# rpng/open_vins

Hardware: NVIDIA H100
Metric: msckf_updates_per_sec (higher is better)
Workload: dtype f64

## Files before the change

open_vins_b200/csrc/chol_tiles.cuh:

```cuda
#pragma once
#include "chol.cuh"
#ifdef CQ_PROBE
#include <cstdio>
#endif

#define CT_XP 12

__device__ __forceinline__ void ct_dmma(double &d0, double &d1, double a, double b) {
  asm volatile("mma.sync.aligned.m8n8k4.row.col.f64.f64.f64.f64 {%0,%1}, {%2}, {%3}, {%0,%1};" : "+d"(d0), "+d"(d1) : "d"(a), "d"(b));
}
__device__ __forceinline__ int ct_tri(int b) { return (b * (b + 1)) >> 1; }
__device__ __forceinline__ void ct_bar_group(int id, int nthreads) { asm volatile("bar.sync %0, %1;" ::"r"(id), "r"(nthreads) : "memory"); }
__device__ __forceinline__ size_t ct_idx(int i, int j) { return (size_t)(ct_tri(i >> 3) + (j >> 3)) * 64 + (i & 7) * 8 + (j & 7); }

struct CtView {
  double *T, *Xp0, *Xp1, *invd, *Linv0, *Linv1, *dummyT, *dummyX;
  int *flag;
};
__host__ __device__ inline size_t ct_view_doubles(int NRB) {
  return (size_t)((NRB * (NRB + 1)) / 2) * 64 + 2 * (size_t)NRB * 8 * CT_XP + (size_t)NRB * 8 + 128 + 64 + 2 * CT_XP;
}
__device__ __forceinline__ CtView ct_view_carve(double *base, int NRB, int *flag_word) {
  CtView v;
  v.T = base;
  v.Xp0 = v.T + (size_t)((NRB * (NRB + 1)) / 2) * 64;
  v.Xp1 = v.Xp0 + (size_t)NRB * 8 * CT_XP;
  v.invd = v.Xp1 + (size_t)NRB * 8 * CT_XP;
  v.Linv0 = v.invd + (size_t)NRB * 8;
  v.Linv1 = v.Linv0 + 64;
  v.dummyT = v.Linv1 + 64;
  v.dummyX = v.dummyT + 64;
  v.flag = flag_word;
  return v;
}

__device__ __forceinline__ void ct_diag8_frag(double &d0, double &d1, int nbk, double *invd, bool strict, double floor_d, int *flag) {
  const unsigned full = 0xffffffffu;
  const int lane = threadIdx.x & 31, g = lane >> 2, q = lane & 3;
  bool bad = false;
  double myinv = 0.0;
  const double inv_floor = (floor_d > 0.0) ? fast_rsqrt(floor_d) : 0.0;
  double pj = __shfl_sync(full, d0, 0);
#pragma unroll
  for (int j = 0; j < 8; j++) {
    const int jq = j >> 1;
    const double cur = (j & 1) ? d1 : d0;
    const double ag = __shfl_sync(full, cur, 4 * g + jq);
    const double ac0 = __shfl_sync(full, cur, 8 * q + jq);
    const double ac1 = __shfl_sync(full, cur, 8 * q + 4 + jq);
    double an = 0.0, dn = 0.0;
    if (j < 7) {
      an = __shfl_sync(full, cur, 4 * (j + 1) + jq);
      dn = __shfl_sync(full, ((j + 1) & 1) ? d1 : d0, 4 * (j + 1) + ((j + 1) >> 1));
    }
    const double y = fast_rsqrt(pj);
    const bool in = j < nbk;
    double d, iv;
    if (strict) {
      const bool pos = pj > 0.0;
      bad = bad || (in && !pos);
      d = pj;
      iv = (in && pos) ? y : 0.0;
    } else {
      const bool above = pj > floor_d;
      d = above ? pj : floor_d;
      iv = in ? (above ? y : inv_floor) : 0.0;
    }
    if (j < 7) {
      const double ln = an * iv;
      pj = fma(-ln, ln, dn);
    }
    if (lane == j)
      myinv = iv;
    if (q == jq) {
      if (j & 1)
        d1 = (g == j) ? d * iv : d1 * iv;
      else
        d0 = (g == j) ? d * iv : d0 * iv;
    }
    const double lg = ag * iv, lc0 = ac0 * iv, lc1 = ac1 * iv;
    if (2 * q > j)
      d0 = fma(-lg, lc0, d0);
    if (2 * q + 1 > j)
      d1 = fma(-lg, lc1, d1);
  }
  if (lane < 8)
    invd[lane] = myinv;
  if (bad && lane == 0)
    *flag = 1;
}

__device__ __forceinline__ void ct_linv8(const double *Lt, const double *invd, double *Linv) {
  const int lane = threadIdx.x & 31, cc = lane & 7;
  double mc[8];
#pragma unroll
  for (int j = 0; j < 8; j++) {
    double s0 = (j == cc) ? 1.0 : 0.0, s1 = 0.0;
#pragma unroll
    for (int t = 0; t < j; t++) {
      if (t & 1)
        s1 = fma(-Lt[j * 8 + t], mc[t], s1);
      else
        s0 = fma(-Lt[j * 8 + t], mc[t], s0);
    }
    mc[j] = (s0 + s1) * invd[j];
  }
  if (lane < 8) {
#pragma unroll
    for (int i = 0; i < 8; i++)
      Linv[i * 8 + cc] = (i >= cc) ? mc[i] : 0.0;
  }
}

__device__ __forceinline__ void ct_panel_tile(const CtView &sm, int i, int k, const double *Linv, double *Xb) {
  const int lane = threadIdx.x & 31, g = lane >> 2, q = lane & 3;
  double *t = sm.T + (size_t)(ct_tri(i) + k) * 64;
  const double a0 = t[g * 8 + q], a1 = t[g * 8 + q + 4];
  const double b0 = Linv[g * 8 + q], b1 = Linv[g * 8 + q + 4];
  double2 d = make_double2(0.0, 0.0);
  ct_dmma(d.x, d.y, a0, b0);
  ct_dmma(d.x, d.y, a1, b1);
  *reinterpret_cast<double2 *>(t + 2 * lane) = d;
  *reinterpret_cast<double2 *>(Xb + (size_t)(8 * i + g) * CT_XP + 2 * q) = d;
}

__device__ __forceinline__ void ct_panel_rows(double *T, double *Xp, const double *invd, int i0, int stride, int nrows, int k, int nbk) {
  if (i0 >= nrows)
    return;
  const double *Lk = T + (size_t)(ct_tri(k) + k) * 64;
  double L[8][8], iv[8];
#pragma unroll
  for (int c = 0; c < 8; c++) {
    iv[c] = (c < nbk) ? invd[8 * k + c] : 0.0;
#pragma unroll
    for (int t2 = 0; t2 < 4; t2++) {
      if (2 * t2 < c) {
        const double2 v = *reinterpret_cast<const double2 *>(Lk + c * 8 + 2 * t2);
        L[c][2 * t2] = v.x;
        L[c][2 * t2 + 1] = v.y;
      }
    }
  }
  for (int i = i0; i < nrows; i += stride) {
    double *src = T + (size_t)(ct_tri(i >> 3) + k) * 64 + (i & 7) * 8;
    double v[8], x[8];
    {
      const double2 v01 = *reinterpret_cast<const double2 *>(src), v23 = *reinterpret_cast<const double2 *>(src + 2);
      const double2 v45 = *reinterpret_cast<const double2 *>(src + 4), v67 = *reinterpret_cast<const double2 *>(src + 6);
      v[0] = v01.x, v[1] = v01.y, v[2] = v23.x, v[3] = v23.y, v[4] = v45.x, v[5] = v45.y, v[6] = v67.x, v[7] = v67.y;
    }
#pragma unroll
    for (int c = 0; c < 8; c++) {
      x[c] = (c < nbk) ? v[c] * iv[c] : 0.0;
#pragma unroll
      for (int t = c + 1; t < 8; t++)
        v[t] = fma(-x[c], L[t][c], v[t]);
    }
    if (nbk == 8) {
      *reinterpret_cast<double2 *>(src) = make_double2(x[0], x[1]);
      *reinterpret_cast<double2 *>(src + 2) = make_double2(x[2], x[3]);
      *reinterpret_cast<double2 *>(src + 4) = make_double2(x[4], x[5]);
      *reinterpret_cast<double2 *>(src + 6) = make_double2(x[6], x[7]);
    } else {
#pragma unroll
      for (int c = 0; c < 8; c++)
        if (c < nbk)
          src[c] = x[c];
    }
    double *xp = Xp + (size_t)i * CT_XP;
    *reinterpret_cast<double2 *>(xp) = make_double2(x[0], x[1]);
    *reinterpret_cast<double2 *>(xp + 2) = make_double2(x[2], x[3]);
    *reinterpret_cast<double2 *>(xp + 4) = make_double2(x[4], x[5]);
    *reinterpret_cast<double2 *>(xp + 6) = make_double2(x[6], x[7]);
  }
}

struct CtTileOps {
  double a0, a1, b0, b1;
  double2 c;
  double2 *cp;
};
__device__ __forceinline__ void ct_tile_load(CtTileOps &o, const CtView &sm, const double *Xp, int bi, int bj, int lane, bool valid) {
  const int g = lane >> 2, q = lane & 3;
  const double *xa = valid ? Xp + (size_t)(8 * bi + g) * CT_XP + q : sm.dummyX + q;
  const double *xb = valid ? Xp + (size_t)(8 * bj + g) * CT_XP + q : sm.dummyX + q;
  o.cp = reinterpret_cast<double2 *>((valid ? sm.T + (size_t)(ct_tri(bi) + bj) * 64 : sm.dummyT) + 2 * lane);
  o.a0 = -xa[0];
  o.a1 = -xa[4];
  o.b0 = xb[0];
  o.b1 = xb[4];
  o.c = *o.cp;
}
__device__ __forceinline__ void ct_tile_mma(CtTileOps &o) {
  ct_dmma(o.c.x, o.c.y, o.a0, o.b0);
  ct_dmma(o.c.x, o.c.y, o.a1, o.b1);
}
__device__ __forceinline__ void ct_tile_mma_store(CtTileOps &o) {
  ct_tile_mma(o);
  *o.cp = o.c;
}

#ifdef CQ_PROBE
#define CT_PROBE_T(v) v = clock64()
#else
#define CT_PROBE_T(v) do { } while (0)
#endif

__device__ __forceinline__ void ct_trail_row(const CtView &sm, const double *Xk, int bi, int j0, int jmax, int lane) {
  const int g = lane >> 2, q = lane & 3;
  const double *xa = Xk + (size_t)(8 * bi + g) * CT_XP + q;
  const double a0 = -xa[0], a1 = -xa[4];
  double *trow = sm.T + (size_t)ct_tri(bi) * 64 + 2 * lane;
  for (int bj = j0; bj <= jmax; bj += 2) {
    const bool two = bj + 1 <= jmax;
    const double *xb0 = Xk + (size_t)(8 * bj + g) * CT_XP + q;
    const double *xb1 = two ? xb0 + 8 * CT_XP : sm.dummyX + q;
    double2 *c0p = reinterpret_cast<double2 *>(trow + (size_t)bj * 64);
    double2 *c1p = two ? c0p + 32 : reinterpret_cast<double2 *>(sm.dummyT + 2 * lane);
    const double b00 = xb0[0], b01 = xb0[4], b10 = xb1[0], b11 = xb1[4];
    double2 c0 = *c0p, c1 = *c1p;
    ct_dmma(c0.x, c0.y, a0, b00);
    ct_dmma(c1.x, c1.y, a0, b10);
    ct_dmma(c0.x, c0.y, a1, b01);
    ct_dmma(c1.x, c1.y, a1, b11);
    *c0p = c0;
    *c1p = c1;
  }
}

template <int THREADS>
__device__ __forceinline__ void ct_chol_tiles(const CtView &sm, int n, int nrows, bool strict, double floor_d) {
  const int tid = threadIdx.x, lane = tid & 31, wid = tid >> 5;
  constexpr int NW = THREADS / 32, NH = NW - (NW + 3) / 4;
  static_assert(NH >= 1, "need at least one helper warp");
  const bool helper = (wid & 3) != 0;
  const int hr = wid - 1 - (wid >> 2);
  constexpr bool LINV = NW >= 8;
#ifdef CQ_PROBE
  long long p0 = 0, p1 = 0, p2 = 0, p3 = 0, p4 = 0, p5 = 0, acc[6] = {0, 0, 0, 0, 0, 0};
#endif
  const int NB = (n + 7) >> 3, NRB = (nrows + 7) >> 3;
  if (wid == 0) {
    double2 c = *reinterpret_cast<const double2 *>(sm.T + 2 * lane);
    ct_diag8_frag(c.x, c.y, min(8, n), sm.invd, strict, floor_d, sm.flag);
    *reinterpret_cast<double2 *>(sm.T + 2 * lane) = c;
    __syncwarp();
    if (LINV)
      asm volatile("bar.arrive 3, 64;" ::: "memory");
    ct_panel_rows(sm.T, sm.Xp0, sm.invd, lane < 8 ? 8 + lane : nrows, 1 << 30, nrows, 0, min(8, n));
  } else if (LINV && wid == 4) {
    asm volatile("bar.sync 3, 64;" ::: "memory");
    ct_linv8(sm.T, sm.invd, sm.Linv0);
  }
  __syncthreads();
  for (int k = 0; k < NB; k++) {
    const int par = k & 1;
    double *Xk = par ? sm.Xp1 : sm.Xp0, *Xn = par ? sm.Xp0 : sm.Xp1;
    const bool more = k + 1 < NB;
    CT_PROBE_T(p0);
#ifdef CQ_PROBE
    p1 = p2 = p3 = p4 = p0;
#endif
    if (wid == 0) {
      if (more) {
        const int k1 = k + 1, nbk1 = min(8, n - 8 * k1);
        CtTileOps o;
        ct_tile_load(o, sm, Xk, k1, k1, lane, true);
        ct_tile_mma(o);
        CT_PROBE_T(p1);
        ct_diag8_frag(o.c.x, o.c.y, nbk1, sm.invd + 8 * k1, strict, floor_d, sm.flag);
        *o.cp = o.c;
        __syncwarp();
        if (LINV)
          asm volatile("bar.arrive 3, 64;" ::: "memory");
        CT_PROBE_T(p2);
        asm volatile("bar.sync 2, %0;" ::"r"((NH + 1) * 32) : "memory");
        CT_PROBE_T(p3);
        ct_panel_rows(sm.T, Xn, sm.invd, lane < 8 ? 8 * (k + 2) + lane : nrows, 1 << 30, nrows, k1, nbk1);
        CT_PROBE_T(p4);
      }
    } else if (LINV && wid == 4) {
      if (more) {
        asm volatile("bar.sync 3, 64;" ::: "memory");
        ct_linv8(sm.T + (size_t)(ct_tri(k + 1) + k + 1) * 64, sm.invd + 8 * (k + 1), par ? sm.Linv0 : sm.Linv1);
      }
    } else if (helper) {
      if (LINV) {
        const double *Lk = par ? sm.Linv1 : sm.Linv0;
        for (int i = k + 2 + hr; i < NRB; i += NH)
          ct_panel_tile(sm, i, k, Lk, Xk);
      } else {
        ct_panel_rows(sm.T, Xk, sm.invd, 8 * (k + 2) + hr * 32 + lane, NH * 32, nrows, k, min(8, n - 8 * k));
      }
      if (NH > 1)
        ct_bar_group(1, NH * 32);
      else
        __syncwarp();
      CT_PROBE_T(p1);
      if (more) {
        for (int i = k + 2 + hr; i < NRB; i += 2 * NH) {
          CtTileOps o0, o1;
          ct_tile_load(o0, sm, Xk, i, k + 1, lane, true);
          ct_tile_load(o1, sm, Xk, i + NH, k + 1, lane, i + NH < NRB);
          ct_tile_mma_store(o0);
          ct_tile_mma_store(o1);
        }
        asm volatile("bar.arrive 2, %0;" ::"r"((NH + 1) * 32) : "memory");
        CT_PROBE_T(p2);
        const int R = NRB - (k + 2), jmaxc = NB - 1;
        for (int pr = hr; 2 * pr < R; pr += NH) {
          const int rb = R - 1 - pr;
          ct_trail_row(sm, Xk, k + 2 + rb, k + 2, min(k + 2 + rb, jmaxc), lane);
          if (rb != pr)
            ct_trail_row(sm, Xk, k + 2 + pr, k + 2, min(k + 2 + pr, jmaxc), lane);
        }
      }
      CT_PROBE_T(p3);
    }
    __syncthreads();
    CT_PROBE_T(p5);
#ifdef CQ_PROBE
    if (wid == 0) {
      acc[0] += p1 - p0, acc[1] += p2 - p1, acc[2] += p3 - p2, acc[3] += p4 - p3, acc[4] += p5 - p4;
    } else {
      acc[0] += p1 - p0, acc[1] += p2 - p1, acc[2] += p3 - p2, acc[3] += p5 - p3;
    }
    acc[5] += p5 - p0;
#endif
  }
#ifdef CQ_PROBE
  if (tid == 0)
    printf("chol n=%d W0 (cycles over %d steps): diag update %lld pivots %lld wait %lld rows below %lld step tail %lld | %lld\n", n, NB, acc[0], acc[1], acc[2], acc[3],
           acc[4], acc[5]);
  if (tid == 32 || tid == THREADS - 32)
    printf("chol n=%d helper warp %d: panel rows %lld column k+1 %lld trailing %lld wait %lld | %lld\n", n, wid, acc[0], acc[1], acc[2], acc[3], acc[5]);
#endif
}
```

open_vins_b200/csrc/k_cholqr.cu:

```cuda
#include "chol.cuh"
#include "chol_tiles.cuh"
#include "ovb_internal.cuh"
#include <math.h>
#include <cstdio>

#define CQ_MAXN 160
#define CQ_MAXB 20
#define CQ_MAXRB 22
#define CQ_GRAM_T 512
#define CQ_KB 32
#ifndef CQ_CHOL_T
#define CQ_CHOL_T 384
#endif
#define CQ_XP CT_XP
#define CQ_TRSM_T 640

namespace {

__device__ __forceinline__ void dmma(double &d0, double &d1, double a, double b) {
  asm volatile("mma.sync.aligned.m8n8k4.row.col.f64.f64.f64.f64 {%0,%1}, {%2}, {%3}, {%0,%1};" : "+d"(d0), "+d"(d1) : "d"(a), "d"(b));
}
__device__ __forceinline__ unsigned s_u32(const void *p) { return (unsigned)__cvta_generic_to_shared(p); }
__device__ __forceinline__ void cpa16(unsigned dst, const void *src, unsigned bytes) {
  asm volatile("cp.async.cg.shared.global [%0], [%1], 16, %2;" ::"r"(dst), "l"(src), "r"(bytes) : "memory");
// ... 79 lines not shown

}

__global__ void __launch_bounds__(CQ_GRAM_T) k_cq_gram(const double *__restrict__ A, int ldA, int m, int nt, int slab_rows, int BW, int nblk_side,
                                                      double *__restrict__ Gpart, int cs) {
  OVB_PDL_ENTER();
  extern __shared__ __align__(16) double gsm[];
  const int tid = threadIdx.x, lane = tid & 31, wid = tid >> 5, g = lane >> 2, q = lane & 3;
  int ci, cj, offI, offJ;
  bool diag;
  const bool active = cq_tile_origin(blockIdx.x, wid, BW, nblk_side, ci, cj, offI, offJ, diag);
  int bI = 0, tt = blockIdx.x;
  while (tt >= nblk_side - bI) {
    tt -= nblk_side - bI;
    bI++;
  }
  const int bJ = bI + tt;
  const int WI = BW * 32;
  const int nrng = (bI == bJ) ? 1 : 2;
  const int pitch = nrng * WI + 4;
  const int cI0 = bI * WI, cJ0 = bJ * WI;
  const int r0 = blockIdx.y * slab_rows, r1 = min(m, r0 + slab_rows);
  const int nchunks = (r1 > r0) ? (r1 - r0 + CQ_KB - 1) / CQ_KB : 0;
  double acc[4][4][2];
#pragma unroll
  for (int a = 0; a < 4; a++)
#pragma unroll
    for (int b = 0; b < 4; b++)
      acc[a][b][0] = acc[a][b][1] = 0.0;

  auto issue = [&](int c) { cq_issue_rows<CQ_GRAM_T>(gsm + (size_t)(c & 1) * CQ_KB * pitch, pitch, A, ldA, r0 + c * CQ_KB, CQ_KB, r1, nt, cI0, cJ0, WI, nrng); };
  if (nchunks > 0)
    issue(0);
  for (int c = 0; c < nchunks; c++) {
    if (c + 1 < nchunks) {
      issue(c + 1);
      cpa_wait<1>();
    } else {
      cpa_wait<0>();
    }
    __syncthreads();
    if (active) {
      const double *buf = gsm + (size_t)(c & 1) * CQ_KB * pitch;
#pragma unroll
      for (int ks = 0; ks < CQ_KB / 4; ks++)
        cq_gram_kstep(acc, buf + (size_t)4 * ks * pitch, pitch, offI, offJ, diag && offI == offJ, g, q);
    }
    __syncthreads();
  }
  if (cs <= 1) {
    if (active) {
      double *dst = Gpart + (((size_t)blockIdx.y * gridDim.x + blockIdx.x) * 16 + wid) * 1024;
#pragma unroll
      for (int a = 0; a < 4; a++)
#pragma unroll
        for (int b = 0; b < 4; b++)
          *reinterpret_cast<double2 *>(dst + (8 * a + g) * 32 + 8 * b + 2 * q) = make_double2(acc[a][b][0], acc[a][b][1]);
    }
    return;
  }
  double *stage = gsm;
  if (active) {
    double *dst = stage + (size_t)wid * 1024;
#pragma unroll
    for (int a = 0; a < 4; a++)
#pragma unroll
      for (int b = 0; b < 4; b++)
        *reinterpret_cast<double2 *>(dst + (8 * a + g) * 32 + 8 * b + 2 * q) = make_double2(acc[a][b][0], acc[a][b][1]);
  }
  asm volatile("barrier.cluster.arrive.release.aligned;" ::: "memory");
  asm volatile("barrier.cluster.wait.acquire.aligned;" ::: "memory");
  unsigned rank;
  asm volatile("mov.u32 %0, %%cluster_ctarank;" : "=r"(rank));
  if (active) {
    const int per = 1024 / cs;
    double *dst = Gpart + ((((size_t)blockIdx.y / cs) * gridDim.x + blockIdx.x) * 16 + wid) * 1024 + (size_t)rank * per;
    const unsigned base = s_u32(stage + (size_t)wid * 1024 + (size_t)rank * per);
    for (int e = lane; e < per; e += 32) {
      double sum = 0.0;
      for (int r = 0; r < cs; r++) {
        unsigned ra;
        double v;
        asm volatile("mapa.shared::cluster.u32 %0, %1, %2;" : "=r"(ra) : "r"(base + 8u * (unsigned)e), "r"((unsigned)r));
        asm volatile("ld.shared::cluster.f64 %0, [%1];" : "=d"(v) : "r"(ra) : "memory");
        sum += v;
      }
      dst[e] = sum;
    }
  }
  asm volatile("barrier.cluster.arrive.release.aligned;" ::: "memory");
  asm volatile("barrier.cluster.wait.acquire.aligned;" ::: "memory");
}

#define CQ_RED_T 1024
#define CQ_RED_CH 8
#define CQ_RED_GX (16 * CQ_RED_CH)
__global__ void __launch_bounds__(CQ_RED_T) k_cq_reduce(const double *__restrict__ Gpart, int nslab, int nblk, int BW, int nblk_side, int nt,
                                                       double *__restrict__ G, int ldG, int tiled) {
  OVB_PDL_ENTER();
  __shared__ double red[8][128];
  int ci, cj, offI, offJ;
  bool diag;
  const int w = blockIdx.x / CQ_RED_CH, ch = blockIdx.x % CQ_RED_CH, blk = blockIdx.y;
  if (!cq_tile_origin(blk, w, BW, nblk_side, ci, cj, offI, offJ, diag))
    return;
  if (ci >= nt || cj >= nt)
    return;
  const int el = threadIdx.x & 127, sg = threadIdx.x >> 7;
  const int e = ch * 128 + el;
  const double *src = Gpart + ((size_t)blk * 16 + w) * 1024 + e;
  const size_t stride = (size_t)nblk * 16 * 1024;
  double s0 = 0.0, s1 = 0.0;
  int sl = sg;
  for (; sl + 8 < nslab; sl += 16) {
    s0 += src[(size_t)sl * stride];
    s1 += src[(size_t)(sl + 8) * stride];
  }
  if (sl < nslab)
    s0 += src[(size_t)sl * stride];
  red[sg][el] = s0 + s1;
  __syncthreads();
  if (sg == 0) {
    const int i = ci + (e >> 5), j = cj + (e & 31);
    if (i < nt && j < nt && i <= j) {
      const double s = ((red[0][el] + red[1][el]) + (red[2][el] + red[3][el])) + ((red[4][el] + red[5][el]) + (red[6][el] + red[7][el]));
      if (tiled) {
        G[ct_idx(j, i)] = s;
        if ((i >> 3) == (j >> 3))
          G[(size_t)(tri(j >> 3) + (j >> 3)) * 64 + (i & 7) * 8 + (j & 7)] = s;
      } else {
        G[(size_t)i * ldG + j] = s;
        G[(size_t)j * ldG + i] = s;
      }
    }
  }
}

struct CqCholSmem {
  double T[(CQ_MAXRB * (CQ_MAXRB + 1) / 2) * 64];
  double Xp[2][CQ_MAXRB * 8 * CQ_XP];
  double invd[CQ_MAXRB * 8];
  double Linv[2][64];
  double red[32];
  double dummyT[64];
  double dummyX[2 * CQ_XP];
  int flag;
};

#define CQ_PK_INV ((CQ_MAXB * (CQ_MAXB + 1) / 2) * 64)
#define CQ_PK_DOUBLES (CQ_PK_INV + CQ_MAXB * 8)

namespace {

__device__ __forceinline__ void cq_chol_tiles(CqCholSmem &sm, int n, int nrows, bool strict, double floor_d) {
  CtView v;
  v.T = sm.T;
  v.Xp0 = sm.Xp[0];
  v.Xp1 = sm.Xp[1];
  v.invd = sm.invd;
  v.Linv0 = sm.Linv[0];
  v.Linv1 = sm.Linv[1];
  v.dummyT = sm.dummyT;
  v.dummyX = sm.dummyX;
  v.flag = &sm.flag;
  ct_chol_tiles<CQ_CHOL_T>(v, n, nrows, strict, floor_d);
}

__device__ void cq_load_tiles(CqCholSmem &sm, const double *__restrict__ G, size_t ldG, int n, int nrows, const double *__restrict__ rhs, int ld_rhs) {
  const int tid = threadIdx.x, lane = tid & 31, wid = tid >> 5;
  const int NB = (n + 7) >> 3, NRB = (nrows + 7) >> 3;
  for (int i = wid; i < 8 * NRB; i += CQ_CHOL_T / 32) {
    const double *row = (i >= n && rhs != nullptr) ? rhs + (size_t)(i - n) * ld_rhs : G + (size_t)i * ldG;
    const int jmax = min(i | 7, 8 * NB - 1);
    double *dst = sm.T + (size_t)tri(i >> 3) * 64 + (i & 7) * 8;
    for (int j = 2 * lane; j <= jmax; j += 64) {
      unsigned bytes = 0;
      if (i < nrows)
        bytes = (j + 1 < n) ? 16u : (j < n ? 8u : 0u);
      cpa16(s_u32(dst + (size_t)(j >> 3) * 64 + (j & 7)), bytes ? (const void *)(row + j) : (const void *)G, bytes);
    }
  }
  cpa_commit();
  for (int e = tid; e < 2 * CQ_MAXRB * 8 * CQ_XP; e += CQ_CHOL_T)
    (&sm.Xp[0][0])[e] = 0.0;
  if (tid < 64)
    sm.dummyT[tid] = 0.0;
  if (tid < 2 * CQ_XP)
    sm.dummyX[tid] = 0.0;
  if (tid == 0)
    sm.flag = 0;
  cpa_wait<0>();
}

__device__ __forceinline__ double cq_el(const double *T, int i, int j) { return T[(size_t)(tri(i >> 3) + (j >> 3)) * 64 + (i & 7) * 8 + (j & 7)]; }

}

__global__ void __launch_bounds__(CQ_CHOL_T) k_cq_chol_gram(const double *__restrict__ G, int ldG, int n, double shift_rel, double *__restrict__ Lpk, int tiled) {
  OVB_PDL_ENTER();
  extern __shared__ __align__(16) unsigned char cq_raw[];
  CqCholSmem &sm = *reinterpret_cast<CqCholSmem *>(cq_raw);
  const int tid = threadIdx.x, lane = tid & 31, wid = tid >> 5;
#ifdef CQ_PROBE
  const long long q0 = clock64();
#endif
  if (tiled) {
    __shared__ __align__(8) unsigned long long g_bar;
    const unsigned bar = s_u32(&g_bar);
    const int NB = (n + 7) >> 3;
    if (tid == 0) {
      asm volatile("mbarrier.init.shared::cta.b64 [%0], 1;" ::"r"(bar) : "memory");
      asm volatile("fence.mbarrier_init.release.cluster;" ::: "memory");
    }
    __syncthreads();
    if (tid == 0) {
      const unsigned bytes = (unsigned)(tri(NB) * 64 * sizeof(double));
      asm volatile("mbarrier.arrive.expect_tx.shared::cta.b64 _, [%0], %1;" ::"r"(bar), "r"(bytes) : "memory");
      asm volatile("cp.async.bulk.shared::cluster.global.mbarrier::complete_tx::bytes [%0], [%1], %2, [%3];" ::"r"(s_u32(sm.T)), "l"(G), "r"(bytes), "r"(bar)
                   : "memory");
    }
    for (int e = tid; e < 2 * CQ_MAXRB * 8 * CQ_XP; e += CQ_CHOL_T)
      (&sm.Xp[0][0])[e] = 0.0;
    if (tid < 64)
      sm.dummyT[tid] = 0.0;
    if (tid < 2 * CQ_XP)
      sm.dummyX[tid] = 0.0;
    if (tid == 0)
      sm.flag = 0;
    asm volatile("{\n\t.reg .pred p;\n\tCQ_GWAIT:\n\tmbarrier.try_wait.parity.shared::cta.b64 p, [%0], 0;\n\t@p bra CQ_GDONE;\n\tbra CQ_GWAIT;\n\tCQ_GDONE:\n\t}" ::"r"(bar)
                 : "memory");
    const int r0 = n - 8 * (NB - 1);
    if (r0 < 8) {
      double *last = sm.T + (size_t)tri(NB - 1) * 64;
      for (int e = tid; e < NB * 64; e += CQ_CHOL_T)
        if (((e >> 3) & 7) >= r0)
          last[e] = 0.0;
    }
  } else {
    cq_load_tiles(sm, G, (size_t)ldG, n, n, nullptr, 0);
  }
  __syncthreads();
  double mx = 0.0;
  for (int i = tid; i < n; i += CQ_CHOL_T) {
    const double d = sm.T[(size_t)(tri(i >> 3) + (i >> 3)) * 64 + (i & 7) * 9];
    mx = (d > mx) ? d : mx;
  }
#pragma unroll
  for (int o = 16; o > 0; o >>= 1) {
    const double y = __shfl_xor_sync(0xffffffffu, mx, o);
    mx = (y > mx) ? y : mx;
  }
  if (lane == 0)
    sm.red[wid] = mx;
  __syncthreads();
  mx = 0.0;
  for (int w = 0; w < CQ_CHOL_T / 32; w++)
    mx = (sm.red[w] > mx) ? sm.red[w] : mx;
  const double shift = shift_rel * mx;
  for (int i = tid; i < n; i += CQ_CHOL_T)
    sm.T[(size_t)(tri(i >> 3) + (i >> 3)) * 64 + (i & 7) * 9] += shift;
  __syncthreads();
#ifdef CQ_PROBE
  const long long q1 = clock64();
#endif
  cq_chol_tiles(sm, n, n, false, 0.25 * shift);
#ifdef CQ_PROBE
  const long long q2 = clock64();
#endif
  const int NB = (n + 7) >> 3;
  for (int e = 2 * tid; e < tri(NB) * 64; e += 2 * CQ_CHOL_T)
    *reinterpret_cast<double2 *>(Lpk + e) = *reinterpret_cast<const double2 *>(sm.T + e);
  for (int e = tid; e < CQ_MAXB * 8; e += CQ_CHOL_T)
    Lpk[CQ_PK_INV + e] = (e < n) ? sm.invd[e] : 1.0;
#ifdef CQ_PROBE
  if (tid == 0)
    printf("chol_gram n=%d: load %lld factor %lld store %lld cycles\n", n, q1 - q0, q2 - q1, clock64() - q2);
#endif
}

__global__ void __launch_bounds__(CQ_CHOL_T) k_cq_chol_ekf(double *__restrict__ S, int ldS, int r, const double *__restrict__ res, double *__restrict__ w,
                                                          double *__restrict__ invdiag, DevUpdateInfo *__restrict__ info, double *__restrict__ Lpk,
                                                          const double *__restrict__ floor_dev) {
  OVB_PDL_ENTER();
  extern __shared__ __align__(16) unsigned char cq_raw[];
  CqCholSmem &sm = *reinterpret_cast<CqCholSmem *>(cq_raw);
  const int tid = threadIdx.x, lane = tid & 31, wid = tid >> 5;
  const int nrows = r + (res != nullptr ? 1 : 0);
  cq_load_tiles(sm, S, (size_t)ldS, r, nrows, res, 0);
  __syncthreads();
  if (floor_dev != nullptr)
    cq_chol_tiles(sm, r, nrows, false, *floor_dev);
  else
    cq_chol_tiles(sm, r, nrows, true, 0.0);
  for (int i = wid; i < r; i += CQ_CHOL_T / 32)
    for (int j = lane; j <= i; j += 32)
      S[(size_t)i * ldS + j] = cq_el(sm.T, i, j);
  if (res != nullptr)
    for (int j = tid; j < r; j += CQ_CHOL_T)
      w[j] = cq_el(sm.T, r, j);
  if (invdiag != nullptr)
    for (int j = tid; j < r; j += CQ_CHOL_T)
      invdiag[j] = sm.invd[j];
  if (Lpk != nullptr) {
    const int NB = (r + 7) >> 3;
    for (int e = 2 * tid; e < tri(NB) * 64; e += 2 * CQ_CHOL_T)
      *reinterpret_cast<double2 *>(Lpk + e) = *reinterpret_cast<const double2 *>(sm.T + e);
    for (int e = tid; e < CQ_MAXB * 8; e += CQ_CHOL_T)
      Lpk[CQ_PK_INV + e] = (e < r) ? sm.invd[e] : 1.0;
  }
  if (tid == 0 && sm.flag && info != nullptr)
    info->not_spd = 1;
}

#define CQ_TRSM_NH 10
#define CQ_TRSM_SMEM (sizeof(double) * ((size_t)CQ_PK_DOUBLES + (size_t)(CQ_TRSM_T / 32) * CQ_TRSM_NH * 2 * 32))
template <int NH>
__device__ __forceinline__ void cq_trsm_half(double (&acc)[NH][2], int b0, const double *Lt, const double *Ri, double *xs, int lane) {
  const int g = lane >> 2, q = lane & 3;
#pragma unroll
  for (int jb = 0; jb < NH; jb++) {
    const int B = b0 + jb;
    const double *Ld = Lt + (size_t)(tri(B) + B) * 64;
    const double *ri = Ri + B * 8;
    double x[8];
#pragma unroll
    for (int qq = 0; qq < 4; qq++) {
      x[2 * qq] = __shfl_sync(0xffffffffu, acc[jb][0], (lane & ~3) | qq);
      x[2 * qq + 1] = __shfl_sync(0xffffffffu, acc[jb][1], (lane & ~3) | qq);
    }
#pragma unroll
    for (int c = 0; c < 8; c++) {
      x[c] *= ri[c];
#pragma unroll
      for (int c2 = c + 1; c2 < 8; c2++)
        x[c2] -= x[c] * Ld[c2 * 8 + c];
    }
    acc[jb][0] = (q == 0) ? x[0] : (q == 1) ? x[2] : (q == 2) ? x[4] : x[6];
    acc[jb][1] = (q == 0) ? x[1] : (q == 1) ? x[3] : (q == 2) ? x[5] : x[7];
    const double af0 = -((q == 0) ? x[0] : (q == 1) ? x[1] : (q == 2) ? x[2] : x[3]);
    const double af1 = -((q == 0) ? x[4] : (q == 1) ? x[5] : (q == 2) ? x[6] : x[7]);
    if (xs != nullptr) {
      xs[(2 * jb) * 32 + lane] = af0;
      xs[(2 * jb + 1) * 32 + lane] = af1;
    }
#pragma unroll
    for (int j = jb + 1; j < NH; j++) {
      const double *lf = Lt + (size_t)(tri(b0 + j) + B) * 64 + g * 8 + q;
      dmma(acc[j][0], acc[j][1], af0, lf[0]);
      dmma(acc[j][0], acc[j][1], af1, lf[4]);
    }
  }
}

template <int NH>
__device__ __forceinline__ void cq_trsm_load(double (&acc)[NH][2], const double *arow, bool row_ok, int b0, int nt, int q) {
#pragma unroll
  for (int jb = 0; jb < NH; jb++) {
    const int col = 8 * (b0 + jb) + 2 * q;
    acc[jb][0] = acc[jb][1] = 0.0;
    if (row_ok) {
      if (col + 1 < nt) {
        const double2 v = *reinterpret_cast<const double2 *>(arow + col);
        acc[jb][0] = v.x;
        acc[jb][1] = v.y;
      } else if (col < nt) {
        acc[jb][0] = arow[col];
      }
    }
  }
}
template <int NH>
__device__ __forceinline__ void cq_trsm_store(const double (&acc)[NH][2], double *arow, bool row_ok, int b0, int nt, int q) {
  if (!row_ok)
    return;
#pragma unroll
  for (int jb = 0; jb < NH; jb++) {
    const int col = 8 * (b0 + jb) + 2 * q;
    if (col + 1 < nt)
      *reinterpret_cast<double2 *>(arow + col) = make_double2(acc[jb][0], acc[jb][1]);
    else if (col < nt)
      arow[col] = acc[jb][0];
  }
}

template <int NBP, int NT>
__device__ __forceinline__ void cq_fetch_factor(double *Lt, double *Ri, const double *__restrict__ Lpk, int NB) {
  const int tid = threadIdx.x;
  __shared__ __align__(8) unsigned long long l_bar;
  const unsigned bar = s_u32(&l_bar);
  if (tid == 0) {
    asm volatile("mbarrier.init.shared::cta.b64 [%0], 1;" ::"r"(bar) : "memory");
    asm volatile("fence.mbarrier_init.release.cluster;" ::: "memory");
  }
  __syncthreads();
  if (tid == 0) {
    const unsigned bytesL = (unsigned)(tri(NB) * 64 * sizeof(double)), bytesR = (unsigned)(NB * 8 * sizeof(double));
    asm volatile("mbarrier.arrive.expect_tx.shared::cta.b64 _, [%0], %1;" ::"r"(bar), "r"(bytesL + bytesR) : "memory");
    asm volatile("cp.async.bulk.shared::cluster.global.mbarrier::complete_tx::bytes [%0], [%1], %2, [%3];" ::"r"(s_u32(Lt)), "l"(Lpk), "r"(bytesL), "r"(bar)
                 : "memory");
    asm volatile("cp.async.bulk.shared::cluster.global.mbarrier::complete_tx::bytes [%0], [%1], %2, [%3];" ::"r"(s_u32(Ri)), "l"(Lpk + CQ_PK_INV), "r"(bytesR),
                 "r"(bar)
                 : "memory");
  }
  for (int e = tri(NB) * 64 + tid; e < tri(NBP) * 64; e += NT)
    Lt[e] = 0.0;
  for (int e = NB * 8 + tid; e < NBP * 8; e += NT)
    Ri[e] = 1.0;
  asm volatile("{\n\t.reg .pred p;\n\tCQ_LWAIT:\n\tmbarrier.try_wait.parity.shared::cta.b64 p, [%0], 0;\n\t@p bra CQ_LDONE;\n\tbra CQ_LWAIT;\n\tCQ_LDONE:\n\t}" ::"r"(bar)
               : "memory");
  __syncthreads();
}

template <int NH1, int NH2>
__global__ void __launch_bounds__(CQ_TRSM_T) k_cq_trsm(double *__restrict__ A, int ldA, int m, int nt, const double *__restrict__ Lpk) {
  OVB_PDL_ENTER();
  extern __shared__ __align__(16) double tsm[];
  double *Lt = tsm;
  double *Ri = tsm + CQ_PK_INV;
  double *Xs = tsm + CQ_PK_DOUBLES;
  const int tid = threadIdx.x, lane = tid & 31, wid = tid >> 5, g = lane >> 2, q = lane & 3;
  cq_fetch_factor<NH1 + NH2, CQ_TRSM_T>(Lt, Ri, Lpk, (nt + 7) >> 3);
  double *xs = Xs + (size_t)wid * (CQ_TRSM_NH * 2 * 32);
  const int ngroups = (m + 7) >> 3;
  for (int rg = blockIdx.x + gridDim.x * wid; rg < ngroups; rg += gridDim.x * (CQ_TRSM_T / 32)) {
    const int row = 8 * rg + g;
    const bool row_ok = row < m;
    double *arow = A + (size_t)row * ldA;
#ifdef CQ_PROBE
    long long t0 = clock64(), t1, t2, t3 = 0, t4 = 0;
#endif
    {
      double acc[NH1][2];
      cq_trsm_load<NH1>(acc, arow, row_ok, 0, nt, q);
#ifdef CQ_PROBE
      t1 = clock64();
#endif
      cq_trsm_half<NH1>(acc, 0, Lt, Ri, NH2 > 0 ? xs : nullptr, lane);
#ifdef CQ_PROBE
      t2 = clock64();
#endif
      cq_trsm_store<NH1>(acc, arow, row_ok, 0, nt, q);
    }
    if constexpr (NH2 > 0) {
      double acc[NH2][2];
      cq_trsm_load<NH2>(acc, arow, row_ok, NH1, nt, q);
      __syncwarp();
#pragma unroll 2
      for (int jb = 0; jb < NH1; jb++) {
        const double af0 = xs[(2 * jb) * 32 + lane], af1 = xs[(2 * jb + 1) * 32 + lane];
#pragma unroll
        for (int j = 0; j < NH2; j++) {
          const double *lf = Lt + (size_t)(tri(NH1 + j) + jb) * 64 + g * 8 + q;
          dmma(acc[j][0], acc[j][1], af0, lf[0]);
          dmma(acc[j][0], acc[j][1], af1, lf[4]);
        }
      }
#ifdef CQ_PROBE
      t3 = clock64();
#endif
      cq_trsm_half<NH2>(acc, NH1, Lt, Ri, nullptr, lane);
#ifdef CQ_PROBE
      t4 = clock64();
#endif
      cq_trsm_store<NH2>(acc, arow, row_ok, NH1, nt, q);
      __syncwarp();
    }
// ... 210 lines not shown
      acc[a][b][0] = acc[a][b][1] = 0.0;
  for (int k0 = 0; k0 < K; k0 += 32) {
    for (int e = tid; e < 64 * 16; e += CQ_GN_T) {
      const int r = e >> 4, u = e & 15, k = k0 + 2 * u;
      unsigned ba = 0, bb = 0;
      if (m0 + r < M)
        ba = (k + 1 < K) ? 16u : (k < K ? 8u : 0u);
      if (n0 + r < N)
        bb = (k + 1 < K) ? 16u : (k < K ? 8u : 0u);
      cpa16(s_u32(&As[r][2 * u]), ba ? (const void *)(A + (size_t)(m0 + r) * lda + k) : (const void *)A, ba);
      cpa16(s_u32(&Bs[r][2 * u]), bb ? (const void *)(B + (size_t)(n0 + r) * ldb + k) : (const void *)B, bb);
    }
    cpa_commit();
    cpa_wait<0>();
    __syncthreads();
#pragma unroll
    for (int ks = 0; ks < 8; ks++) {
      double fa[4], fb[2];
#pragma unroll
      for (int a = 0; a < 4; a++)
        fa[a] = As[wm + 8 * a + g][4 * ks + q];
#pragma unroll
      for (int b = 0; b < 2; b++)
        fb[b] = Bs[wn + 8 * b + g][4 * ks + q];
#pragma unroll
      for (int a = 0; a < 4; a++)
#pragma unroll
        for (int b = 0; b < 2; b++)
          dmma(acc[a][b][0], acc[a][b][1], fa[a], fb[b]);
    }
    __syncthreads();
  }
#pragma unroll
  for (int a = 0; a < 4; a++)
#pragma unroll
    for (int b = 0; b < 2; b++) {
      const int i = m0 + wm + 8 * a + g, j = n0 + wn + 8 * b + 2 * q;
      if (i < M) {
        double *c = C + (size_t)i * ldc + j;
        if (j + 1 < N) {
          double2 v = *reinterpret_cast<double2 *>(c);
          v.x -= acc[a][b][0];
          v.y -= acc[a][b][1];
          *reinterpret_cast<double2 *>(c) = v;
        } else if (j < N) {
          c[0] -= acc[a][b][0];
        }
      }
    }
}

__global__ void __launch_bounds__(256) k_cq_shift(double *__restrict__ G, int ldG, int n, double shift_rel, double *__restrict__ floor_out) {
  OVB_PDL_ENTER();
  __shared__ double red[8];
  double mx = 0.0;
  for (int i = threadIdx.x; i < n; i += 256) {
    const double d = G[(size_t)i * ldG + i];
    mx = (d > mx) ? d : mx;
  }
#pragma unroll
  for (int o = 16; o > 0; o >>= 1) {
    const double y = __shfl_xor_sync(0xffffffffu, mx, o);
    mx = (y > mx) ? y : mx;
  }
  if ((threadIdx.x & 31) == 0)
    red[threadIdx.x >> 5] = mx;
  __syncthreads();
  mx = 0.0;
  for (int w = 0; w < 8; w++)
    mx = (red[w] > mx) ? red[w] : mx;
  const double shift = shift_rel * mx;
  for (int i = threadIdx.x; i < n; i += 256)
    G[(size_t)i * ldG + i] += shift;
  if (threadIdx.x == 0)
    *floor_out = 0.25 * shift;
}

__global__ void __launch_bounds__(256) k_cq_trmm_wide(const double *__restrict__ L2, const double *__restrict__ L1, int ldL, int nt, double *__restrict__ Rout,
                                                     int ldR) {
  OVB_PDL_ENTER();
  __shared__ double As[32][33];
  __shared__ double Bs[32][33];
  const int ti = blockIdx.y, tj = blockIdx.x;
  const int tid = threadIdx.x, tx = tid & 31, ty = tid >> 5;
  const int n = nt - 1;
  double acc[4] = {0, 0, 0, 0};
  if (tj >= ti) {
    for (int tk = ti; tk <= tj; tk++) {
      for (int e = tid; e < 1024; e += 256) {
        const int a = e >> 5, b = e & 31;
        const int k = tk * 32 + a, i = ti * 32 + b;
        As[a][b] = (k < nt && i < nt && k >= i) ? L2[(size_t)k * ldL + i] : 0.0;
        const int j = tj * 32 + a, k2 = tk * 32 + b;
        Bs[a][b] = (j < nt && k2 < nt && j >= k2) ? L1[(size_t)j * ldL + k2] : 0.0;
      }
      __syncthreads();
#pragma unroll 8
      for (int kk = 0; kk < 32; kk++) {
        const double b = Bs[tx][kk];
#pragma unroll
        for (int u = 0; u < 4; u++)
          acc[u] += As[kk][ty + 8 * u] * b;
      }
      __syncthreads();
    }
  }
#pragma unroll
  for (int u = 0; u < 4; u++) {
    const int i = ti * 32 + ty + 8 * u, j = tj * 32 + tx;
    if (i < n && j < nt)
      Rout[(size_t)i * ldR + j] = (j >= i) ? acc[u] : 0.0;
  }
}

#define CQ_GRAM_CS 4
static void cq_launch_gram(ovb_ctx *ctx, int nblk, int nslab_padded, size_t smem, const double *A, int ldA, int m, int nt, int slab_rows, int BW, int nblk_side,
                           double *Gpart, int cs) {
  cudaLaunchConfig_t cfg = {};
  cfg.gridDim = dim3(nblk, nslab_padded);
  cfg.blockDim = dim3(CQ_GRAM_T);
  cfg.dynamicSmemBytes = smem;
  cfg.stream = ctx->stream;
  cudaLaunchAttribute at[2];
  int na = 0;
  if (ctx->tsqr_pdl && !ctx->prof_on) {
    at[na].id = cudaLaunchAttributeProgrammaticStreamSerialization;
    at[na].val.programmaticStreamSerializationAllowed = 1;
    na++;
  }
  if (cs > 1) {
    at[na].id = cudaLaunchAttributeClusterDimension;
    at[na].val.clusterDim.x = 1;
    at[na].val.clusterDim.y = cs;
    at[na].val.clusterDim.z = 1;
    na++;
  }
  cfg.attrs = at;
  cfg.numAttrs = na;
  const bool prof = ctx->prof_on && ctx->prof_n < 96 && ctx->prof_ev[0] != nullptr;
  if (prof)
    cudaEventRecord(ctx->prof_ev[2 * ctx->prof_n], ctx->stream);
  cudaLaunchKernelEx(&cfg, k_cq_gram, A, ldA, m, nt, slab_rows, BW, nblk_side, Gpart, cs);
  if (prof) {
    cudaEventRecord(ctx->prof_ev[2 * ctx->prof_n + 1], ctx->stream);
    ctx->prof_fn[ctx->prof_n++] = (const void *)k_cq_gram;
  }
}

static bool cq_attrs(ovb_ctx *ctx) {
  if (!ctx->attr_done[4]) {
    cudaFuncSetAttribute(k_cq_gram, cudaFuncAttributeMaxDynamicSharedMemorySize, 160 * 1024);
    cudaFuncSetAttribute(k_cq_chol_gram, cudaFuncAttributeMaxDynamicSharedMemorySize, (int)sizeof(CqCholSmem));
    cudaFuncSetAttribute(k_cq_chol_ekf, cudaFuncAttributeMaxDynamicSharedMemorySize, (int)sizeof(CqCholSmem));
    cudaFuncSetAttribute(k_cq_trsm<5, 0>, cudaFuncAttributeMaxDynamicSharedMemorySize, (int)CQ_TRSM_SMEM);
    cudaFuncSetAttribute(k_cq_trsm<10, 0>, cudaFuncAttributeMaxDynamicSharedMemorySize, (int)CQ_TRSM_SMEM);
    cudaFuncSetAttribute(k_cq_trsm<10, 5>, cudaFuncAttributeMaxDynamicSharedMemorySize, (int)CQ_TRSM_SMEM);
    cudaFuncSetAttribute(k_cq_trsm<10, 10>, cudaFuncAttributeMaxDynamicSharedMemorySize, (int)CQ_TRSM_SMEM);
    cudaFuncSetAttribute(k_cq_solve_gram<5, 0>, cudaFuncAttributeMaxDynamicSharedMemorySize, CQ_SG_SMEM);
    cudaFuncSetAttribute(k_cq_solve_gram<10, 0>, cudaFuncAttributeMaxDynamicSharedMemorySize, CQ_SG_SMEM);
    cudaFuncSetAttribute(k_cq_solve_gram<10, 5>, cudaFuncAttributeMaxDynamicSharedMemorySize, CQ_SG_SMEM);
    cudaFuncSetAttribute(k_cq_solve_gram<10, 10>, cudaFuncAttributeMaxDynamicSharedMemorySize, CQ_SG_SMEM);
    ctx->attr_done[4] = 1;
  }
  return true;
}

int ovb_cholqr_max_cols(void) { return CQ_MAXN; }

static bool cq_ensure_G(ovb_ctx *ctx) {
  const int ldW = CQ_MAXN + 8;
  const size_t need_G = (size_t)4 * ldW * ldW;
  if (need_G > ctx->G_cap) {
    if (ctx->d_G)
      cudaFree(ctx->d_G);
    ctx->d_G = nullptr;
    if (cudaMalloc(&ctx->d_G, sizeof(double) * need_G) != cudaSuccess)
      return false;
    cudaMemsetAsync(ctx->d_G, 0, sizeof(double) * need_G, ctx->stream);
    ctx->G_cap = need_G;
  }
  return true;
}

bool launch_chol_ekf_dmma(ovb_ctx *ctx, double *S, int ldS, int r, const double *res, double *w, double *invdiag, double **Lpk_out) {
  if (Lpk_out)
    *Lpk_out = nullptr;
  if (r + 1 > CQ_MAXRB * 8 || r > CQ_MAXN || (ldS & 1))
    return false;
  cq_attrs(ctx);
  double *Lpk = nullptr;
  if (cq_ensure_G(ctx)) {
    const int ldW = CQ_MAXN + 8;
    Lpk = ctx->d_G + (size_t)3 * ldW * ldW;
  }
  ovb_launch(ctx, k_cq_chol_ekf, dim3(1), dim3(CQ_CHOL_T), sizeof(CqCholSmem), S, ldS, r, res, w, invdiag, ctx->d_info, Lpk, (const double *)nullptr);
  if (Lpk_out)
    *Lpk_out = Lpk;
  return true;
}

bool launch_trsm_rows(ovb_ctx *ctx, double *A, int ldA, int m, int nt, const double *Lpk) {
  if (nt > CQ_MAXN || (ldA & 1) || m < 1 || Lpk == nullptr)
    return false;
  cq_attrs(ctx);
  const int ngroups = (m + 7) / 8;
  int ctas = ngroups;
  if (ctas > ctx->sm_count)
    ctas = ctx->sm_count;
  cq_launch_trsm(ctx, ctas, A, ldA, m, nt, Lpk);
  return true;
}

#define CQ_WB 128
#define CQ_WMAX 520
#define CQ_WBLOCKS ((CQ_WMAX + CQ_WB - 1) / CQ_WB)
static bool cq_ensure_wide(ovb_ctx *ctx) {
  const size_t need = (size_t)2 * CQ_WMAX * CQ_WMAX + (size_t)2 * CQ_WBLOCKS * CQ_PK_DOUBLES + 64;
  if (need > ctx->cqw_cap) {
    if (ctx->d_cqw)
      cudaFree(ctx->d_cqw);
    ctx->d_cqw = nullptr;
    if (cudaMalloc(&ctx->d_cqw, sizeof(double) * need) != cudaSuccess)
      return false;
    ctx->cqw_cap = need;
  }
  return true;
}
static void cq_gemm_nt(ovb_ctx *ctx, double *C, int ldc, const double *A, int lda, const double *B, int ldb, int M, int N, int K, int lower_only) {
  if (M <= 0 || N <= 0 || K <= 0)
    return;
  ovb_launch(ctx, k_cq_gemm_nt, dim3((N + 63) / 64, (M + 63) / 64), dim3(CQ_GN_T), (size_t)0, C, ldc, A, lda, B, ldb, M, N, K, lower_only);
}
static void cq_trsm_any(ovb_ctx *ctx, double *A, int ldA, int m, int nt, const double *Lpk) {
  const int ngroups = (m + 7) / 8;
  int ctas = (ngroups + CQ_TRSM_T / 32 - 1) / (CQ_TRSM_T / 32);
  if (ngroups <= ctx->sm_count)
    ctas = ngroups;
  if (ctas > ctx->sm_count)
    ctas = ctx->sm_count;
  cq_launch_trsm(ctx, ctas, A, ldA, m, nt, Lpk);
}
static void cq_chol_blocked(ovb_ctx *ctx, double *S, int ld, int n, int extra, double *Lpk, const double *floor_dev, DevUpdateInfo *info) {
  for (int J = 0, b = 0; J < n; J += CQ_WB, b++) {
    const int nb = (n - J < CQ_WB) ? n - J : CQ_WB;
    double *Lb = Lpk + (size_t)b * CQ_PK_DOUBLES;
    ovb_launch(ctx, k_cq_chol_ekf, dim3(1), dim3(CQ_CHOL_T), sizeof(CqCholSmem), S + (size_t)J * ld + J, ld, nb, (const double *)nullptr, (double *)nullptr,
               (double *)nullptr, info, Lb, floor_dev);
    const int mrem = n + extra - (J + nb);
    if (mrem > 0) {
      double *panel = S + (size_t)(J + nb) * ld + J;
      cq_trsm_any(ctx, panel, ld, mrem, nb, Lb);
      const int ncols = n - (J + nb);
      cq_gemm_nt(ctx, S + (size_t)(J + nb) * ld + (J + nb), ld, panel, ld, panel, ld, mrem, ncols, nb, 1);
    }
  }
}
static void cq_trsm_blocked(ovb_ctx *ctx, double *X, int ldx, int m, int n, const double *S, int ld, const double *Lpk) {
  for (int J = 0, b = 0; J < n; J += CQ_WB, b++) {
    const int nb = (n - J < CQ_WB) ? n - J : CQ_WB;
    if (J > 0)
      cq_gemm_nt(ctx, X + J, ldx, X, ldx, S + (size_t)J * ld, ld, m, nb, J, 0);
    cq_trsm_any(ctx, X + J, ldx, m, nb, Lpk + (size_t)b * CQ_PK_DOUBLES);
  }
}

__global__ void k_cq_copy_row(const double *__restrict__ src, double *__restrict__ dst, int n) {
  OVB_PDL_ENTER();
  const int i = blockIdx.x * blockDim.x + threadIdx.x;
  if (i < n)
    dst[i] = src[i];
}
__global__ void k_cq_inv_diag(const double *__restrict__ S, int ld, int n, double *__restrict__ inv) {
  OVB_PDL_ENTER();
  const int i = blockIdx.x * blockDim.x + threadIdx.x;
  if (i < n) {
    const double d = S[(size_t)i * ld + i];
    inv[i] = d != 0.0 ? 1.0 / d : 0.0;
  }
}

bool launch_chol_solve_wide(ovb_ctx *ctx, double *S, int ldS, int r, double *w, double *invdiag, double *M, int ldM, int N, bool gate_only) {
  if (r > CQ_WMAX - 8 || (ldS & 1) || (ldM & 1) || r + 1 > ctx->cfg.max_state + 1)
    return false;
  cq_attrs(ctx);
  if (!cq_ensure_wide(ctx))
    return false;
  double *Lpk = ctx->d_cqw + (size_t)2 * CQ_WMAX * CQ_WMAX;
  ovb_launch(ctx, k_cq_copy_row, dim3((r + 127) / 128), dim3(128), (size_t)0, (const double *)w, S + (size_t)r * ldS, r);
  cq_chol_blocked(ctx, S, ldS, r, 1, Lpk, nullptr, ctx->d_info);
  ovb_launch(ctx, k_cq_copy_row, dim3((r + 127) / 128), dim3(128), (size_t)0, (const double *)(S + (size_t)r * ldS), w, r);
  ovb_launch(ctx, k_cq_inv_diag, dim3((r + 127) / 128), dim3(128), (size_t)0, (const double *)S, ldS, r, invdiag);
  if (!gate_only)
    cq_trsm_blocked(ctx, M, ldM, N, r, S, ldS, Lpk);
  return true;
}

static int cq_compress_wide(ovb_ctx *ctx, double *A, int m, int n, int ldA, double *Rout, int ldR) {
  const int nt = n + 1;
  if (nt > CQ_WMAX - 7 || !cq_ensure_wide(ctx))
    return -1;
  const int nT = (nt + 31) / 32, BW = 4, nblk_side = (nT + BW - 1) / BW, nblk = nblk_side * (nblk_side + 1) / 2;
  int nslab = ctx->sm_count / nblk;
  if (nslab < 1)
    nslab = 1;
  const int max_slabs = (m + CQ_KB - 1) / CQ_KB;
  if (nslab > max_slabs)
    nslab = max_slabs;
  int slab_rows = (((m + nslab - 1) / nslab) + 3) & ~3;
  nslab = (m + slab_rows - 1) / slab_rows;
  const size_t need_part = (size_t)nslab * nblk * 16 * 1024;
  if (need_part > ctx->Gpart_cap) {
    if (ctx->d_Gpart)
      cudaFree(ctx->d_Gpart);
    ctx->d_Gpart = nullptr;
    if (cudaMalloc(&ctx->d_Gpart, sizeof(double) * need_part) != cudaSuccess)
      return -1;
    ctx->Gpart_cap = need_part;
  }
  double *G1 = ctx->d_cqw, *G2 = G1 + (size_t)CQ_WMAX * CQ_WMAX, *Lpk1 = G2 + (size_t)CQ_WMAX * CQ_WMAX, *Lpk2 = Lpk1 + (size_t)CQ_WBLOCKS * CQ_PK_DOUBLES;
  double *floor_dev = Lpk2 + (size_t)CQ_WBLOCKS * CQ_PK_DOUBLES;
  const size_t gram_smem = sizeof(double) * 2 * CQ_KB * (size_t)(2 * BW * 32 + 4);
  int launches = 0;
  for (int pass = 0; pass < 2; pass++) {
    double *G = pass == 0 ? G1 : G2;
    cq_launch_gram(ctx, nblk, nslab, gram_smem, (const double *)A, ldA, m, nt, slab_rows, BW, nblk_side, ctx->d_Gpart, 1);
    ovb_launch(ctx, k_cq_reduce, dim3(CQ_RED_GX, nblk), dim3(CQ_RED_T), (size_t)0, (const double *)ctx->d_Gpart, nslab, nblk, BW, nblk_side, nt, G, (int)CQ_WMAX, 0);
    ovb_launch(ctx, k_cq_shift, dim3(1), dim3(256), (size_t)0, G, (int)CQ_WMAX, nt, pass == 0 ? 1e-11 : 1e-13, floor_dev + pass);
    cq_chol_blocked(ctx, G, CQ_WMAX, nt, 0, pass == 0 ? Lpk1 : Lpk2, floor_dev + pass, (DevUpdateInfo *)nullptr);
    if (pass == 0)
      cq_trsm_blocked(ctx, A, ldA, m, nt, G1, CQ_WMAX, Lpk1);
    launches += 3 + 3 * ((nt + CQ_WB - 1) / CQ_WB);
  }
  const int nT32 = (nt + 31) / 32;
  ovb_launch(ctx, k_cq_trmm_wide, dim3(nT32, nT32), dim3(256), (size_t)0, (const double *)G2, (const double *)G1, (int)CQ_WMAX, nt, Rout, ldR);
  ctx->n_launch += launches + 1;
  return launches + 1;
}

int launch_compress_cholqr2(ovb_ctx *ctx, double *A, int m, int n, int ldA, double *Rout, int ldR) {
  const int nt = n + 1;
  if ((ldA & 1) || m < 1)
    return -1;
  cq_attrs(ctx);
  if (nt > CQ_MAXN)
    return cq_compress_wide(ctx, A, m, n, ldA, Rout, ldR);
  const int nT = (nt + 31) / 32;
  const int BW = nT, nblk_side = 1, nblk = 1;
  int nslab = ctx->sm_count;
  const int max_slabs = (m + CQ_KB - 1) / CQ_KB;
  if (nslab > max_slabs)
    nslab = max_slabs;
  int slab_rows = (m + nslab - 1) / nslab;
  slab_rows = (slab_rows + 3) & ~3;
  nslab = (m + slab_rows - 1) / slab_rows;
  const int cs = (ctx->gram_cluster && nslab >= 2 * CQ_GRAM_CS) ? CQ_GRAM_CS : 1;
  const int nslab_pad = (nslab + cs - 1) / cs * cs, npart = nslab_pad / cs;
  const size_t part_doubles = (size_t)nslab_pad * nblk * 16 * 1024;
  const size_t need_part = part_doubles + cq_solve_gram_scratch(nslab, nt, BW, slab_rows);
  const int ldW = CQ_MAXN + 8;
  if (!cq_ensure_G(ctx))
    return -1;
  if (need_part > ctx->Gpart_cap) {
    if (ctx->d_Gpart)
// ... 23 lines not shown
```

open_vins_b200/csrc/k_ekf.cu:

```cuda
#include "chol.cuh"
#include "ovb_internal.cuh"

#define EK_T 32

__global__ void __launch_bounds__(256) k_ekf_gemm(int mode, const double *__restrict__ P, int ldP, const double *__restrict__ H, int ldH,
                                                  const double *__restrict__ Min, int ldM, const DevUpdateInfo *__restrict__ info, int X, int Y,
                                                  int K, double *__restrict__ Cout, int ldC, double sigma2, const double *__restrict__ Rdiag) {
  OVB_PDL_ENTER();
  __shared__ double As[EK_T][EK_T + 1];
  __shared__ double Bs[EK_T][EK_T + 1];
  const int x0 = blockIdx.x * EK_T, y0 = blockIdx.y * EK_T;
  if (mode == 1 && y0 > x0 + EK_T - 1)
    return;
  const int tid = threadIdx.x, tx = tid & 31, ty = tid >> 5;
  double acc[4] = {0, 0, 0, 0};
  const int *cs = info->col_state;
  for (int j0 = 0; j0 < K; j0 += EK_T) {
    for (int e = tid; e < EK_T * EK_T; e += 256) {
      int jj = e >> 5, q = e & 31;
      int j = j0 + jj;
      double av = 0.0, bv = 0.0;
      if (j < K) {
        if (mode == 0) {
          int a = x0 + q;
// ... 58 lines not shown
    ld = r | 1;
    W = chol_sm;
    stage_lower_async<EKC_THREADS>(W, ld, S, (size_t)ldS, r + 1, r);
  }
  chol_lower_block<EKC_THREADS, 4>(W, ld, r, 1, &flag, invd_sh, nullptr, 0.0, invdiag);
  __syncthreads();
  if (use_smem) {
    for (int i = wid; i < r; i += EKC_THREADS / 32) {
      for (int j = lane; j <= i; j += 32)
        S[(size_t)i * ldS + j] = W[i * ld + j];
    }
  }
  for (int j = tid; j < r; j += EKC_THREADS)
    w[j] = W[(size_t)r * ld + j];
  if (tid == 0 && flag)
    info->not_spd = 1;
}

#define TR_ROWS 8
__global__ void __launch_bounds__(32 * TR_ROWS) k_ekf_trsm(const double *__restrict__ M, int ldM, const double *__restrict__ L, int ldL,
                                                           const double *__restrict__ invdiag, int N, int r, double *__restrict__ Yout, int ldY,
                                                           int L_in_smem, const DevUpdateInfo *__restrict__ info) {
  OVB_PDL_ENTER();
  extern __shared__ __align__(16) double tsm[];
  const int lane = threadIdx.x & 31, wid = threadIdx.x >> 5;
  if (info->not_spd)
    return;
  const int ldl = r | 1;
  double *inv_s = tsm + (size_t)TR_ROWS * r;
  double *Ls = inv_s + r;
  for (int e = threadIdx.x; e < r; e += 32 * TR_ROWS)
    inv_s[e] = invdiag[e];
  if (L_in_smem)
    stage_lower_async<32 * TR_ROWS>(Ls, ldl, L, (size_t)ldL, r, r);
  else
    __syncthreads();
  const double *Lp = L_in_smem ? Ls : L;
  const int lp = L_in_smem ? ldl : ldL;
  const int a = blockIdx.x * TR_ROWS + wid;
  if (a >= N)
    return;
  double *y = tsm + (size_t)wid * r;
  for (int t = lane; t < r; t += 32)
    y[t] = M[(size_t)a * ldM + t];
  __syncwarp();
  for (int kb = 0; kb < r; kb += 8) {
    const int nbk = min(8, r - kb);
    double s[8];
#pragma unroll
    for (int c = 0; c < 8; c++)
      s[c] = 0.0;
    for (int t = lane; t < kb; t += 32) {
      const double yt = y[t];
#pragma unroll
      for (int c = 0; c < 8; c++)
        if (c < nbk)
          s[c] += Lp[(size_t)(kb + c) * lp + t] * yt;
    }
#pragma unroll
    for (int o = 16; o > 0; o >>= 1) {
#pragma unroll
      for (int c = 0; c < 8; c++)
        s[c] += __shfl_xor_sync(0xffffffffu, s[c], o);
    }
    double yn[8];
#pragma unroll
    for (int c = 0; c < 8; c++) {
      if (c < nbk) {
        const double *Lr = Lp + (size_t)(kb + c) * lp + kb;
        double v = y[kb + c] - s[c];
#pragma unroll
        for (int t = 0; t < 8; t++)
          if (t + 1 < c)
            v -= Lr[t] * yn[t];
        if (c > 0)
          v -= Lr[c - 1] * yn[c - 1];
        yn[c] = v * inv_s[kb + c];
      }
    }
    __syncwarp();
    if (lane < nbk) {
      double v = yn[0];
#pragma unroll
      for (int c = 1; c < 8; c++)
        v = (lane == c) ? yn[c] : v;
      y[kb + lane] = v;
    }
    __syncwarp();
  }
  for (int t = lane; t < r; t += 32)
    Yout[(size_t)a * ldY + t] = y[t];
}

__global__ void __launch_bounds__(256) k_ekf_downdate(double *__restrict__ P, int ldP, const double *__restrict__ Yin, int ldY, int N, int r,
                                                      const double *__restrict__ w, double *__restrict__ dx, DevUpdateInfo *__restrict__ info) {
  OVB_PDL_ENTER();
  __shared__ double As[EK_T][EK_T + 1];
  __shared__ double Bs[EK_T][EK_T + 1];
  const int a0 = blockIdx.x * EK_T, b0 = blockIdx.y * EK_T;
  if (b0 < a0)
    return;
  const int tid = threadIdx.x, tx = tid & 31, ty = tid >> 5;
  if (info->not_spd) {
    if (a0 == b0 && tid < EK_T && a0 + tid < N)
      dx[a0 + tid] = 0.0;
    return;
  }
  double acc[4] = {0, 0, 0, 0};
  double dxa = 0.0;
  for (int k0 = 0; k0 < r; k0 += EK_T) {
    for (int e = tid; e < EK_T * EK_T; e += 256) {
      int q = e >> 5, kk = e & 31;
      int k = k0 + kk;
      As[kk][q] = (k < r && a0 + q < N) ? Yin[(size_t)(a0 + q) * ldY + k] : 0.0;
      Bs[kk][q] = (k < r && b0 + q < N) ? Yin[(size_t)(b0 + q) * ldY + k] : 0.0;
    }
    __syncthreads();
#pragma unroll 8
    for (int kk = 0; kk < EK_T; kk++) {
      double b = Bs[kk][tx];
#pragma unroll
      for (int u = 0; u < 4; u++)
        acc[u] += As[kk][ty + 8 * u] * b;
    }
    if (a0 == b0 && tid < EK_T) {
      for (int kk = 0; kk < EK_T; kk++)
        if (k0 + kk < r)
          dxa += As[kk][tid] * w[k0 + kk];
    }
    __syncthreads();
  }
#pragma unroll
  for (int u = 0; u < 4; u++) {
    int a = a0 + ty + 8 * u, b = b0 + tx;
    if (a < N && b < N && b >= a) {
      double v = P[(size_t)a * ldP + b] - acc[u];
      P[(size_t)a * ldP + b] = v;
      P[(size_t)b * ldP + a] = v;
      if (a == b && v < 0.0)
        atomicMin(&info->neg_diag_index, a);
      if (!isfinite(v))
        info->nonfinite = 1;
    }
  }
  if (a0 == b0 && tid < EK_T && a0 + tid < N)
    dx[a0 + tid] = dxa;
}

#define EK1_KMAX 160
__device__ __forceinline__ void ek_cpa8(double *dst_smem, const double *src) {
  asm volatile("cp.async.ca.shared.global [%0], [%1], 8;" ::"r"((unsigned)__cvta_generic_to_shared(dst_smem)), "l"(src) : "memory");
}
__global__ void __launch_bounds__(256) k_ekf_gemm1(int mode, const double *__restrict__ P, int ldP, const double *__restrict__ H, int ldH,
                                                   const double *__restrict__ Min, int ldM, const DevUpdateInfo *__restrict__ info, int X, int Y,
                                                   int K, double *__restrict__ Cout, int ldC, double sigma2, const double *__restrict__ Rdiag) {
  OVB_PDL_ENTER();
  extern __shared__ __align__(16) double g1[];
  const int x0 = blockIdx.x * EK_T, y0 = blockIdx.y * EK_T;
  if (mode == 1 && y0 > x0 + EK_T - 1)
    return;
  const int tid = threadIdx.x, tx = tid & 31, ty = tid >> 5;
  const int *cs = info->col_state;
  const int pk = K | 1;
  double *Gs = g1, *Hs = g1 + (size_t)K * 33;
  const double *Gsrc = (mode == 0) ? P : Min;
  const int ldG = (mode == 0) ? ldP : ldM;
  const int g0 = (mode == 0) ? x0 : y0, gmax = (mode == 0) ? X : Y;
  const int h0 = (mode == 0) ? y0 : x0, hmax = (mode == 0) ? Y : X;
  __shared__ int cs_s[EK1_KMAX];
  for (int j = tid; j < K; j += 256)
    cs_s[j] = cs[j];
  __syncthreads();
  for (int e = tid; e < K * 32; e += 256) {
    const int j = e >> 5, a = e & 31;
    if (g0 + a < gmax)
      ek_cpa8(&Gs[j * 33 + a], &Gsrc[(size_t)cs_s[j] * ldG + g0 + a]);
    else
      Gs[j * 33 + a] = 0.0;
  }
  for (int i = ty; i < 32; i += 8)
    for (int j = tx; j < K; j += 32) {
      if (h0 + i < hmax)
        ek_cpa8(&Hs[i * pk + j], &H[(size_t)(h0 + i) * ldH + j]);
      else
        Hs[i * pk + j] = 0.0;
    }
  asm volatile("cp.async.commit_group;" ::: "memory");
  asm volatile("cp.async.wait_group 0;" ::: "memory");
  __syncthreads();
  double acc[4] = {0, 0, 0, 0};
  if (mode == 0) {
    for (int j = 0; j < K; j++) {
      const double gv = Gs[j * 33 + tx];
#pragma unroll
      for (int u = 0; u < 4; u++)
        acc[u] += gv * Hs[(ty + 8 * u) * pk + j];
    }
#pragma unroll
    for (int u = 0; u < 4; u++) {
      const int a = x0 + tx, i = y0 + ty + 8 * u;
      if (a < X && i < Y)
        Cout[(size_t)a * ldC + i] = acc[u];
    }
  } else {
    for (int j = 0; j < K; j++) {
      const double gv = Gs[j * 33 + tx];
#pragma unroll
      for (int u = 0; u < 4; u++)
        acc[u] += Hs[(ty + 8 * u) * pk + j] * gv;
    }
#pragma unroll
    for (int u = 0; u < 4; u++) {
      const int i = x0 + ty + 8 * u, k = y0 + tx;
      if (i < X && k < Y) {
        double v = acc[u];
        if (i == k)
          v += Rdiag ? Rdiag[i] : sigma2;
        Cout[(size_t)i * ldC + k] = v;
      }
    }
  }
}

__global__ void __launch_bounds__(256) k_ekf_downdate1(double *__restrict__ P, int ldP, const double *__restrict__ Yin, int ldY, int N, int r,
                                                       const double *__restrict__ w, double *__restrict__ dx, DevUpdateInfo *__restrict__ info) {
  OVB_PDL_ENTER();
  extern __shared__ __align__(16) double d1[];
  const int a0 = blockIdx.x * EK_T, b0 = blockIdx.y * EK_T;
  if (b0 < a0)
    return;
  const int tid = threadIdx.x, tx = tid & 31, ty = tid >> 5;
  if (info->not_spd) {
    if (a0 == b0 && tid < EK_T && a0 + tid < N)
      dx[a0 + tid] = 0.0;
    return;
  }
  const int pk = r | 1;
  double *As = d1, *Bs = d1 + (size_t)32 * pk, *ws = Bs + (size_t)32 * pk;
  for (int i = ty; i < 32; i += 8)
    for (int k = tx; k < r; k += 32) {
      if (a0 + i < N)
        ek_cpa8(&As[i * pk + k], &Yin[(size_t)(a0 + i) * ldY + k]);
      else
        As[i * pk + k] = 0.0;
      if (b0 + i < N)
        ek_cpa8(&Bs[i * pk + k], &Yin[(size_t)(b0 + i) * ldY + k]);
      else
        Bs[i * pk + k] = 0.0;
    }
  for (int k = tid; k < r; k += 256)
    ek_cpa8(&ws[k], &w[k]);
  asm volatile("cp.async.commit_group;" ::: "memory");
  asm volatile("cp.async.wait_group 0;" ::: "memory");
  __syncthreads();
  double acc[4] = {0, 0, 0, 0};
  for (int k = 0; k < r; k++) {
    const double bv = Bs[tx * pk + k];
#pragma unroll
    for (int u = 0; u < 4; u++)
      acc[u] += As[(ty + 8 * u) * pk + k] * bv;
  }
#pragma unroll
  for (int u = 0; u < 4; u++) {
    const int a = a0 + ty + 8 * u, b = b0 + tx;
    if (a < N && b < N && b >= a) {
      const double v = P[(size_t)a * ldP + b] - acc[u];
      P[(size_t)a * ldP + b] = v;
      P[(size_t)b * ldP + a] = v;
      if (a == b && v < 0.0)
        atomicMin(&info->neg_diag_index, a);
      if (!isfinite(v))
        info->nonfinite = 1;
    }
  }
  if (a0 == b0 && tid < EK_T && a0 + tid < N) {
    double s0 = 0.0, s1 = 0.0;
    int k = 0;
    for (; k + 1 < r; k += 2) {
      s0 += As[tid * pk + k] * ws[k];
      s1 += As[tid * pk + k + 1] * ws[k + 1];
    }
    if (k < r)
      s0 += As[tid * pk + k] * ws[k];
    dx[a0 + tid] = s0 + s1;
  }
}

__global__ void k_ekf_prep(DevUpdateInfo *info) {
  OVB_PDL_ENTER();
  info->neg_diag_index = 0x7fffffff;
  info->not_spd = 0;
  info->nonfinite = 0;
}

void launch_ekf_update(ovb_ctx *ctx, const double *H, int ldHm, int r, int n, bool gate_only, double sigma2, const double *Rdiag_dev) {
  const int N = ctx->N;
  const int ld = ctx->ldP;
  double *P = ctx->P[ctx->cur];
  ovb_launch(ctx, k_ekf_prep, dim3(1), dim3(1), (size_t)(0), ctx->d_info);
  if (r <= 0 || n <= 0)
    return;
  if (!ctx->attr_done[2]) {
    cudaFuncSetAttribute(k_ekf_chol, cudaFuncAttributeMaxDynamicSharedMemorySize, 200 * 1024);
    cudaFuncSetAttribute(k_ekf_trsm, cudaFuncAttributeMaxDynamicSharedMemorySize, 200 * 1024);
    cudaFuncSetAttribute(k_ekf_gemm1, cudaFuncAttributeMaxDynamicSharedMemorySize, 100 * 1024);
    cudaFuncSetAttribute(k_ekf_downdate1, cudaFuncAttributeMaxDynamicSharedMemorySize, 100 * 1024);
    ctx->attr_done[2] = 1;
  }
  const bool one_shot = ctx->ekf_chol_dmma && n <= EK1_KMAX && r <= EK1_KMAX;
  dim3 g0((N + EK_T - 1) / EK_T, (r + EK_T - 1) / EK_T);
  dim3 g1((r + EK_T - 1) / EK_T, (r + EK_T - 1) / EK_T);
  if (one_shot) {
    const size_t sm01 = sizeof(double) * ((size_t)n * 33 + (size_t)32 * (n | 1));
    ovb_launch(ctx, k_ekf_gemm1, dim3(g0), dim3(256), sm01, 0, P, ld, H, ldHm, nullptr, 0, ctx->d_info, N, r, n, ctx->d_M, ld, 0.0, nullptr);
    ovb_launch(ctx, k_ekf_gemm1, dim3(g1), dim3(256), sm01, 1, P, ld, H, ldHm, ctx->d_M, ld, ctx->d_info, r, r, n, ctx->d_S, ld, sigma2, Rdiag_dev);
  } else {
    ovb_launch(ctx, k_ekf_gemm, dim3(g0), dim3(256), (size_t)(0), 0, P, ld, H, ldHm, nullptr, 0, ctx->d_info, N, r, n, ctx->d_M, ld, 0.0, nullptr);
    ovb_launch(ctx, k_ekf_gemm, dim3(g1), dim3(256), (size_t)(0), 1, P, ld, H, ldHm, ctx->d_M, ld, ctx->d_info, r, r, n, ctx->d_S, ld, sigma2, Rdiag_dev);
  }
  size_t chol_bytes = sizeof(double) * (size_t)(r + 1) * (size_t)(r | 1);
  int use_smem = chol_bytes <= 200 * 1024;
  double *invdiag = ctx->d_w + ctx->cfg.max_state;
  double *Lpk = nullptr;
  const bool dmma_chol = ctx->ekf_chol_dmma && launch_chol_ekf_dmma(ctx, ctx->d_S, ld, r, ctx->d_w, ctx->d_w, invdiag, &Lpk);
  const bool wide = !dmma_chol && ctx->ekf_chol_dmma && r < ld && launch_chol_solve_wide(ctx, ctx->d_S, ld, r, ctx->d_w, invdiag, ctx->d_M, ld, N, gate_only);
  if (wide) {
    if (gate_only)
      return;
    dim3 g2w((N + EK_T - 1) / EK_T, (N + EK_T - 1) / EK_T);
    ovb_launch(ctx, k_ekf_downdate, dim3(g2w), dim3(256), (size_t)(0), P, ld, (const double *)ctx->d_M, ld, N, r, ctx->d_w, ctx->d_dx, ctx->d_info);
    return;
  }
  if (!dmma_chol)
    ovb_launch(ctx, k_ekf_chol, dim3(1), dim3(EKC_THREADS), (size_t)(use_smem ? chol_bytes : 0), ctx->d_S, ld, r, ctx->d_w, ctx->d_w, invdiag, ctx->d_info, use_smem);
  if (gate_only)
    return;
  const double *Yd = ctx->d_Y;
  if (dmma_chol && Lpk != nullptr && launch_trsm_rows(ctx, ctx->d_M, ld, N, r, Lpk)) {
    Yd = ctx->d_M;
  } else {
    size_t trsm_small = sizeof(double) * ((size_t)TR_ROWS * r + r);
    size_t trsm_full = trsm_small + sizeof(double) * (size_t)r * (size_t)(r | 1);
    int L_in_smem = trsm_full <= 200 * 1024;
    ovb_launch(ctx, k_ekf_trsm, dim3((N + TR_ROWS - 1) / TR_ROWS), dim3(32 * TR_ROWS), (size_t)(L_in_smem ? trsm_full : trsm_small), ctx->d_M, ld, ctx->d_S, ld, invdiag, N,
               r, ctx->d_Y, ld, L_in_smem, ctx->d_info);
  }
  dim3 g2((N + EK_T - 1) / EK_T, (N + EK_T - 1) / EK_T);
  if (one_shot) {
    const size_t smd = sizeof(double) * ((size_t)64 * (r | 1) + r);
    ovb_launch(ctx, k_ekf_downdate1, dim3(g2), dim3(256), smd, P, ld, Yd, ld, N, r, ctx->d_w, ctx->d_dx, ctx->d_info);
  } else {
    ovb_launch(ctx, k_ekf_downdate, dim3(g2), dim3(256), (size_t)(0), P, ld, Yd, ld, N, r, ctx->d_w, ctx->d_dx, ctx->d_info);
  }
}


__global__ void k_cov_init_augment(double *__restrict__ P, int ld, int N, int k, int n, const DevUpdateInfo *__restrict__ info,
                                   const double *__restrict__ Hx, const double *__restrict__ Hinv, double sigma2) {
  extern __shared__ double ism[];
  double *m = ism, *M = ism + (size_t)N * k;
  const int tid = threadIdx.x;
  for (int a = tid; a < N; a += blockDim.x) {
    for (int i = 0; i < k; i++) {
      double acc = 0.0;
      for (int j = 0; j < n; j++)
        acc += P[(size_t)a * ld + info->col_state[j]] * Hx[i * n + j];
      m[a * k + i] = acc;
    }
  }
  __syncthreads();
  if (tid < k * k) {
    const int i = tid / k, i2 = tid % k;
    double acc = 0.0;
    for (int j = 0; j < n; j++)
      acc += Hx[i * n + j] * m[info->col_state[j] * k + i2];
    M[i * k + i2] = acc + (i == i2 ? sigma2 : 0.0);
  }
  __syncthreads();
  if (tid < k * k) {
    const int i = tid / k, i2 = tid % k;
    if (i2 < i)
      M[i * k + i2] = M[i2 * k + i];
  }
  __syncthreads();
  for (int a = tid; a < N; a += blockDim.x) {
    for (int q = 0; q < k; q++) {
      double acc = 0.0;
      for (int i = 0; i < k; i++)
        acc += m[a * k + i] * Hinv[q * k + i];
      P[(size_t)a * ld + N + q] = -acc;
      P[(size_t)(N + q) * ld + a] = -acc;
    }
  }
  if (tid < k * k) {
    const int q = tid / k, q2 = tid % k;
    double acc = 0.0;
    for (int i = 0; i < k; i++)
      for (int i2 = 0; i2 < k; i2++)
        acc += Hinv[q * k + i] * M[i * k + i2] * Hinv[q2 * k + i2];
    if (q <= q2) {
      P[(size_t)(N + q) * ld + N + q2] = acc;
      P[(size_t)(N + q2) * ld + N + q] = acc;
    }
  }
}

bool launch_cov_init_augment(ovb_ctx *ctx, int k, int n, const double *Hx_dev, const double *Hinv_dev, double sigma2) {
  const int N = ctx->N;
  size_t smem = sizeof(double) * ((size_t)N * k + (size_t)k * k);
  if (smem > 200 * 1024)
    return false;
  if (!ctx->attr_done[5]) {
    cudaFuncSetAttribute(k_cov_init_augment, cudaFuncAttributeMaxDynamicSharedMemorySize, 200 * 1024);
    ctx->attr_done[5] = 1;
  }
  k_cov_init_augment<<<1, 256, smem, ctx->stream>>>(ctx->P[ctx->cur], ctx->ldP, N, k, n, ctx->d_info, Hx_dev, Hinv_dev, sigma2);
  return cudaGetLastError() == cudaSuccess;
}

__global__ void k_cov_clone(double *P, int ld, int N, int old_off, int size) {
  int idx = blockIdx.x * blockDim.x + threadIdx.x;
  int N2 = N + size;
  if (idx >= N2 * size)
    return;
  int i = idx / size, j = idx % size;
  double v;
  if (i < N)
    v = P[(size_t)i * ld + old_off + j];
  else
    v = P[(size_t)(old_off + (i - N)) * ld + old_off + j];
  double vr = (i < N) ? P[(size_t)(old_off + j) * ld + i] : v;
  P[(size_t)i * ld + N + j] = v;
  if (i < N)
    P[(size_t)(N + j) * ld + i] = vr;
}
__global__ void k_cov_dt_cols(double *P, int ld, int N2, int new_off, int size, int dt_off, const double *dnc) {
  int idx = blockIdx.x * blockDim.x + threadIdx.x;
  if (idx >= N2 * size)
    return;
  int i = idx / size, j = idx % size;
  P[(size_t)i * ld + new_off + j] += P[(size_t)i * ld + dt_off] * dnc[j];
}
__global__ void k_cov_dt_rows(double *P, int ld, int N2, int new_off, int size, int dt_off, const double *dnc) {
  int idx = blockIdx.x * blockDim.x + threadIdx.x;
  if (idx >= N2 * size)
    return;
  int i = idx / N2, j = idx % N2;
  P[(size_t)(new_off + i) * ld + j] += dnc[i] * P[(size_t)dt_off * ld + j];
}

void launch_cov_clone(ovb_ctx *ctx, int old_off, int size, const double *dnc_dt_dev, int dt_off) {
  double *P = ctx->P[ctx->cur];
  int N = ctx->N, N2 = N + size;
  int tot = N2 * size;
  k_cov_clone<<<(tot + 255) / 256, 256, 0, ctx->stream>>>(P, ctx->ldP, N, old_off, size);
  if (dnc_dt_dev) {
    k_cov_dt_cols<<<(tot + 255) / 256, 256, 0, ctx->stream>>>(P, ctx->ldP, N2, N, size, dt_off, dnc_dt_dev);
    k_cov_dt_rows<<<(tot + 255) / 256, 256, 0, ctx->stream>>>(P, ctx->ldP, N2, N, size, dt_off, dnc_dt_dev);
  }
}

__global__ void k_cov_marg(const double *Pin, double *Pout, int ld, int N, int off, int size) {
  int N2 = N - size;
  int i = blockIdx.y * blockDim.y + threadIdx.y, j = blockIdx.x * blockDim.x + threadIdx.x;
  if (i >= N2 || j >= N2)
    return;
  int si = i < off ? i : i + size, sj = j < off ? j : j + size;
  double v = (i >= off && j < off) ? Pin[(size_t)sj * ld + si] : Pin[(size_t)si * ld + sj];
  Pout[(size_t)i * ld + j] = v;
}

void launch_cov_marginalize(ovb_ctx *ctx, int off, int size) {
  int N2 = ctx->N - size;
  dim3 b(32, 8), g((N2 + 31) / 32, (N2 + 7) / 8);
  k_cov_marg<<<g, b, 0, ctx->stream>>>(ctx->P[ctx->cur], ctx->P[ctx->cur ^ 1], ctx->ldP, ctx->N, off, size);
}

__global__ void k_prop_C(const double *P, int ld, int N, int p, int q, const int *old_idx, const double *Phi, double *Cbuf, int ldC) {
  int idx = blockIdx.x * blockDim.x + threadIdx.x;
  if (idx >= N * p)
    return;
  int a = idx / p, j = idx % p;
  double acc = 0.0;
  for (int k = 0; k < q; k++)
    acc += P[(size_t)a * ld + old_idx[k]] * Phi[(size_t)j * q + k];
  Cbuf[(size_t)a * ldC + j] = acc;
}
__global__ void k_prop_PCP(const double *Cbuf, int ldC, int p, int q, const int *old_idx, const double *Phi, const double *Q, double *Sbuf,
                           int ldS) {
  int idx = blockIdx.x * blockDim.x + threadIdx.x;
  if (idx >= p * p)
    return;
  int i = idx / p, j = idx % p;
  double acc = (i <= j) ? Q[(size_t)i * p + j] : Q[(size_t)j * p + i];
  for (int k = 0; k < q; k++)
    acc += Phi[(size_t)i * q + k] * Cbuf[(size_t)old_idx[k] * ldC + j];
  Sbuf[(size_t)i * ldS + j] = acc;
}
__global__ void k_prop_write(double *P, int ld, int N, int new_off, int p, const double *Cbuf, int ldC, const double *Sbuf, int ldS,
                             DevUpdateInfo *info) {
  int idx = blockIdx.x * blockDim.x + threadIdx.x;
  if (idx >= N * p)
    return;
  int a = idx / p, j = idx % p;
  if (a >= new_off && a < new_off + p) {
    double v = Sbuf[(size_t)(a - new_off) * ldS + j];
// ... 19 lines not shown
```

open_vins_b200/csrc/ovb_api.cu:

```cuda
#include "ovb_internal.cuh"
#include <chrono>
#include <algorithm>
#include <cmath>
#include <cstdio>
#include <cstdlib>
#include <cstring>
#include <new>
#include <vector>

static const double g_chi2_table[OVB_CHI2_TABLE_LEN] = {
#include "chi2_table.inc"
};

unsigned char *ovb_feat_order_ptr(ovb_ctx *ctx) { return ctx->d_feat_order; }

static size_t align_up(size_t v, size_t a) { return (v + a - 1) / a * a; }

extern "C" {

static ovb_status ensure_stage(ovb_ctx *ctx, size_t doubles);

int ovb_abi_version(void) { return OVB_ABI_VERSION; }

double ovb_chi2_quantile95(int dof) {
  if (dof < 1)
    return 0.0;
  if (dof >= OVB_CHI2_TABLE_LEN)
    dof = OVB_CHI2_TABLE_LEN - 1;
  return g_chi2_table[dof];
}

void ovb_opts_default(ovb_opts *o) {
  memset(o, 0, sizeof(*o));
  o->triangulate_1d = 0;
  o->refine_features = 1;
  o->max_runs = 5;
  o->init_lamda = 1e-3;
  o->max_lamda = 1e10;
  o->min_dx = 1e-6;
  o->min_dcost = 1e-6;
  o->lam_mult = 10;
  o->min_dist = 0.10;
  o->max_dist = 60;
  o->max_baseline = 40;
  o->max_cond_number = 10000;
  o->sigma_pix = 1;
  o->chi2_multipler = 5;
  o->do_fej = 1;
  o->feat_rep = OVB_REP_GLOBAL_3D;
  o->do_calib_camera_pose = 0;
  o->do_calib_camera_intrinsics = 0;
  o->col_order = OVB_COLS_CANONICAL;
  o->compress = OVB_COMPRESS_CHOLQR2;
}

const char *ovb_last_error(const ovb_ctx *ctx) { return ctx ? ctx->err : "null context"; }

ovb_status ovb_create(const ovb_config *cfg, ovb_ctx **out) {
  if (!cfg || !out)
    return OVB_ERR_ARG;
  *out = nullptr;
  ovb_ctx *ctx = new (std::nothrow) ovb_ctx();
  if (!ctx)
    return OVB_ERR_CAPACITY;
  memset(ctx, 0, sizeof(*ctx));
  ctx->cfg = *cfg;
  if (ctx->cfg.max_state < 32)
    ctx->cfg.max_state = 32;
  if (ctx->cfg.max_feats < 1)
    ctx->cfg.max_feats = 1;
  if (ctx->cfg.max_meas < 2)
    ctx->cfg.max_meas = 2;
  ctx->device = cfg->device;
  int ndev = 0;
  if (cudaGetDeviceCount(&ndev) != cudaSuccess || ndev <= 0 || cfg->device >= ndev) {
    delete ctx;
    return OVB_ERR_CUDA;
  }
#define CK(call)                                                                                                      \
  do {                                                                                                                \
    cudaError_t e_ = (call);                                                                                          \
    if (e_ != cudaSuccess) {                                                                                          \
      fprintf(stderr, "ovb_create: %s failed: %s\n", #call, cudaGetErrorString(e_));                                  \
      ovb_destroy(ctx);                                                                                               \
      return OVB_ERR_CUDA;                                                                                            \
    }                                                                                                                 \
  } while (0)
  CK(cudaSetDevice(ctx->device));
  cudaDeviceProp prop;
  CK(cudaGetDeviceProperties(&prop, ctx->device));
  ctx->sm_count = prop.multiProcessorCount;
  {
    const char *e = getenv("OVB_TSQR_CLUSTER");
    ctx->tsqr_cluster = e ? atoi(e) : 1;
    const char *e2 = getenv("OVB_TSQR_PDL");
    ctx->tsqr_pdl = e2 ? atoi(e2) : 1;
    const char *e3 = getenv("OVB_FEAT_CLASSES");
    ctx->feat_classes = e3 ? atoi(e3) : 1;
    const char *e4 = getenv("OVB_EKF_CHOL_DMMA");
    ctx->ekf_chol_dmma = e4 ? atoi(e4) : 1;
    const char *e5 = getenv("OVB_GRAM_CLUSTER");
    ctx->gram_cluster = e5 ? atoi(e5) : 0;
  }
  CK(cudaStreamCreateWithFlags(&ctx->stream, cudaStreamNonBlocking));
  ctx->own_stream = 1;
  CK(cudaStreamCreateWithFlags(&ctx->side_stream, cudaStreamNonBlocking));
  CK(cudaStreamCreateWithFlags(&ctx->side_stream2, cudaStreamNonBlocking));
  CK(cudaEventCreateWithFlags(&ctx->ev_join2, cudaEventDisableTiming));
  CK(cudaEventCreateWithFlags(&ctx->ev_fork, cudaEventDisableTiming));
  CK(cudaEventCreateWithFlags(&ctx->ev_join, cudaEventDisableTiming));
  for (int i = 0; i < 8; i++)
    CK(cudaEventCreate(&ctx->ev[i]));
  const int ms = ctx->cfg.max_state;
  ctx->ldP = ms;
  ctx->N = 0;
  ctx->cur = 0;
  CK(cudaMalloc(&ctx->P[0], sizeof(double) * (size_t)ms * ms));
  CK(cudaMalloc(&ctx->P[1], sizeof(double) * (size_t)ms * ms));
  CK(cudaMemset(ctx->P[0], 0, sizeof(double) * (size_t)ms * ms));
  CK(cudaMemset(ctx->P[1], 0, sizeof(double) * (size_t)ms * ms));
  ctx->off_opts = align_up(sizeof(DevFrame), 256);
  ctx->off_feat = ctx->off_opts + align_up(sizeof(DevOpts), 256);
  ctx->off_blob = ctx->off_feat + align_up(sizeof(DevFeat) * (size_t)ctx->cfg.max_feats, 256);
  ctx->blob_cap = align_up((size_t)ctx->cfg.max_meas * (1 + 2 + 8 + 8) + (size_t)ctx->cfg.max_feats * OVB_MAX_CAMS + 64, 256);
  ctx->arena_bytes = ctx->off_blob + ctx->blob_cap;
  CK(cudaMalloc(&ctx->d_arena, ctx->arena_bytes));
  CK(cudaMallocHost(&ctx->h_arena, ctx->arena_bytes));
  ctx->d_frame = (DevFrame *)ctx->d_arena;
  ctx->d_opts = (DevOpts *)(ctx->d_arena + ctx->off_opts);
  ctx->d_feat = (DevFeat *)(ctx->d_arena + ctx->off_feat);
  ctx->d_blob = ctx->d_arena + ctx->off_blob;
  ctx->h_frame = (DevFrame *)ctx->h_arena;
  ctx->h_opts = (DevOpts *)(ctx->h_arena + ctx->off_opts);
  ctx->h_feat = (DevFeat *)(ctx->h_arena + ctx->off_feat);
  ctx->h_blob = ctx->h_arena + ctx->off_blob;
  CK(cudaMalloc(&ctx->d_cc, sizeof(DevCamPoses)));
  CK(cudaMalloc(&ctx->d_feat_order, (size_t)ctx->cfg.max_feats * (OVB_MAX_VARS + 1)));
  ctx->info_bytes = align_up(sizeof(DevUpdateInfo), 256);
  CK(cudaMalloc(&ctx->d_info, ctx->info_bytes + sizeof(double) * (size_t)ms));
  ctx->d_dx = (double *)((char *)ctx->d_info + ctx->info_bytes);
  CK(cudaMallocHost(&ctx->h_info, ctx->info_bytes + sizeof(double) * (size_t)ms));
  ctx->h_dx = (double *)((char *)ctx->h_info + ctx->info_bytes);
  CK(cudaMalloc(&ctx->d_chi2_table, sizeof(g_chi2_table)));
  CK(cudaMemcpy(ctx->d_chi2_table, g_chi2_table, sizeof(g_chi2_table), cudaMemcpyHostToDevice));
  ctx->max_rows = ctx->cfg.max_rows > 0 ? ctx->cfg.max_rows : 2 * ctx->cfg.max_meas;
  if (ctx->max_rows < 2 * ctx->cfg.max_meas)
    ctx->max_rows = 2 * ctx->cfg.max_meas;
  int ldcap = std::min(OVB_MAX_COLS, ms) + 8;
  ctx->Hs_cap = (size_t)ctx->max_rows * ldcap;
  CK(cudaMalloc(&ctx->d_Hs, sizeof(double) * ctx->Hs_cap));
  ctx->h_stage = nullptr;
  ctx->stage_cap = 0;
  ctx->W_cap = ((size_t)ctx->max_rows / OVB_CR + 2 + (size_t)ctx->sm_count) * OVB_NB * OVB_NB + 4096;
  CK(cudaMalloc(&ctx->d_W[0], sizeof(double) * ctx->W_cap));
  CK(cudaMalloc(&ctx->d_W[1], sizeof(double) * ctx->W_cap));
  size_t rsz = (size_t)(ms + 8) * (ms + 8);
  CK(cudaMalloc(&ctx->d_R, sizeof(double) * rsz));
  CK(cudaMalloc(&ctx->d_R2, sizeof(double) * rsz));
  CK(cudaMalloc(&ctx->d_M, sizeof(double) * (size_t)ms * ms));
  CK(cudaMalloc(&ctx->d_S, sizeof(double) * (size_t)(ms + 1) * ms));
  CK(cudaMalloc(&ctx->d_Y, sizeof(double) * (size_t)ms * ms));
  CK(cudaMalloc(&ctx->d_w, sizeof(double) * (size_t)ms * 4));
  ctx->scratch_per_cta = (size_t)(2 * OVB_BIG_MAX_MEAS + 1) * (2 * OVB_BIG_MAX_MEAS + 1);
  ctx->scratch_ctas = 2 * ctx->sm_count;
  CK(cudaMalloc(&ctx->d_scratch, sizeof(double) * ctx->scratch_per_cta * ctx->scratch_ctas));
  ctx->dump_cap = 0;
  ctx->d_dump = nullptr;
#undef CK
  *out = ctx;
  return OVB_OK;
}

void ovb_destroy(ovb_ctx *ctx) {
  if (ctx)
    for (int i = 0; i < 2 * 96; i++)
      if (ctx->prof_ev[i])
        cudaEventDestroy(ctx->prof_ev[i]);
  if (!ctx)
    return;
  cudaSetDevice(ctx->device);
  if (ctx->stream)
    cudaStreamSynchronize(ctx->stream);
  void *dev[] = {ctx->P[0],   ctx->P[1], ctx->d_arena, ctx->d_cc, ctx->d_feat_order, ctx->d_info, ctx->d_chi2_table, ctx->d_Hs, ctx->d_W[0],
                 ctx->d_W[1], ctx->d_R,  ctx->d_R2,    ctx->d_M,  ctx->d_S,          ctx->d_Y,    ctx->d_w,          ctx->d_scratch,
                 ctx->d_long, ctx->d_dump, ctx->P_snap, ctx->d_flush, ctx->d_Gpart, ctx->d_G, ctx->d_cqw, ctx->d_grp, ctx->d_grp_acc};
  for (void *p : dev)
    if (p)
      cudaFree(p);
  void *host[] = {ctx->h_arena, ctx->h_info, ctx->h_stage, ctx->h_grp};
  for (void *p : host)
    if (p)
      cudaFreeHost(p);
  for (int i = 0; i < 8; i++)
    if (ctx->ev[i])
      cudaEventDestroy(ctx->ev[i]);
  if (ctx->ev_fork)
    cudaEventDestroy(ctx->ev_fork);
  if (ctx->ev_join)
    cudaEventDestroy(ctx->ev_join);
  if (ctx->ev_join2)
    cudaEventDestroy(ctx->ev_join2);
  if (ctx->side_stream2)
    cudaStreamDestroy(ctx->side_stream2);
  if (ctx->side_stream)
    cudaStreamDestroy(ctx->side_stream);
  if (ctx->stream && ctx->own_stream)
    cudaStreamDestroy(ctx->stream);
  delete ctx;
}

int ovb_cov_dim(const ovb_ctx *ctx) { return ctx ? ctx->N : 0; }

ovb_status ovb_cov_set(ovb_ctx *ctx, const double *P, int N) {
  if (!ctx || !P || N < 1)
    return OVB_ERR_ARG;
  if (N > ctx->cfg.max_state) {
    snprintf(ctx->err, sizeof(ctx->err), "ovb_cov_set: N=%d exceeds max_state=%d", N, ctx->cfg.max_state);
    return OVB_ERR_CAPACITY;
  }
  OVB_CUDA_CHECK(ctx, cudaSetDevice(ctx->device));
  OVB_CUDA_CHECK(ctx, cudaMemcpy2DAsync(ctx->P[ctx->cur], sizeof(double) * ctx->ldP, P, sizeof(double) * N, sizeof(double) * N, N,
                                        cudaMemcpyHostToDevice, ctx->stream));
  OVB_CUDA_CHECK(ctx, cudaStreamSynchronize(ctx->stream));
  ctx->N = N;
  return OVB_OK;
}

ovb_status ovb_cov_get(ovb_ctx *ctx, double *P, int N) {
  if (!ctx || !P || N != ctx->N)
    return OVB_ERR_ARG;
  OVB_CUDA_CHECK(ctx, cudaSetDevice(ctx->device));
  OVB_CUDA_CHECK(ctx, cudaMemcpy2DAsync(P, sizeof(double) * N, ctx->P[ctx->cur], sizeof(double) * ctx->ldP, sizeof(double) * N, N,
                                        cudaMemcpyDeviceToHost, ctx->stream));
  OVB_CUDA_CHECK(ctx, cudaStreamSynchronize(ctx->stream));
  return OVB_OK;
}

ovb_status ovb_cov_get_marginal(ovb_ctx *ctx, const int *off, const int *sz, int nvar, double *out) {
  if (!ctx || !off || !sz || !out || nvar < 1)
    return OVB_ERR_ARG;
  int n = 0;
  for (int i = 0; i < nvar; i++) {
    if (off[i] < 0 || sz[i] < 1 || off[i] + sz[i] > ctx->N)
      return OVB_ERR_ARG;
    n += sz[i];
  }
  OVB_CUDA_CHECK(ctx, cudaSetDevice(ctx->device));
  int ii = 0;
  for (int i = 0; i < nvar; i++) {
    int kk = 0;
    for (int k = 0; k < nvar; k++) {
      OVB_CUDA_CHECK(ctx, cudaMemcpy2DAsync(out + (size_t)ii * n + kk, sizeof(double) * n,
                                            ctx->P[ctx->cur] + (size_t)off[i] * ctx->ldP + off[k], sizeof(double) * ctx->ldP,
// ... 610 lines not shown
}

static void nullspace_project_host(double *Hf, int nf, double *X, int w, int rows) {
  for (int n = 0; n < nf; ++n)
    for (int m = rows - 1; m > n; m--) {
      double gc, gs;
      make_givens(Hf[(size_t)(m - 1) * nf + n], Hf[(size_t)m * nf + n], gc, gs);
      auto rot = [&](double &x, double &y) {
        const double x0 = x, y0 = y;
        x = gc * x0 - gs * y0;
        y = gs * x0 + gc * y0;
      };
      for (int k = n; k < nf; k++)
        rot(Hf[(size_t)(m - 1) * nf + k], Hf[(size_t)m * nf + k]);
      for (int k = 0; k < w; k++)
        rot(X[(size_t)(m - 1) * w + k], X[(size_t)m * w + k]);
    }
}

ovb_status ovb_slam_delayed_init(ovb_ctx *ctx, const ovb_frame *frame, const ovb_feat_batch *feats, const ovb_opts *opts, const double *sigma_pix,
                                 const double *chi2_multipler, ovb_init_callback on_init, void *user, ovb_feat_out *out, int32_t *lm_off_out) {
  return ovb_slam_delayed_init_reps(ctx, frame, feats, opts, nullptr, sigma_pix, chi2_multipler, on_init, user, out, lm_off_out);
}

ovb_status ovb_slam_delayed_init_reps(ovb_ctx *ctx, const ovb_frame *frame, const ovb_feat_batch *feats, const ovb_opts *opts,
                                      const int32_t *feat_rep, const double *sigma_pix, const double *chi2_multipler, ovb_init_callback on_init,
                                      void *user, ovb_feat_out *out, int32_t *lm_off_out) {
  if (!ctx || !frame || !feats || !opts || !out || !out->status || !out->p_FinA || !out->p_FinG || !out->anchor_cam || !out->anchor_clone || !lm_off_out)
    return OVB_ERR_ARG;
  const int F = feats->n_feats;
  auto rep_of = [&](int f) { return feat_rep ? feat_rep[f] : opts->feat_rep; };
  int n_single = 0;
  for (int f = 0; f < F; f++) {
    if (rep_of(f) < OVB_REP_GLOBAL_3D || rep_of(f) > OVB_REP_ANCHORED_INVERSE_DEPTH_SINGLE) {
      snprintf(ctx->err, sizeof(ctx->err), "feature %d: representation %d is not an ovb_feat_rep", f, rep_of(f));
      return OVB_ERR_ARG;
    }
    n_single += rep_of(f) == OVB_REP_ANCHORED_INVERSE_DEPTH_SINGLE ? 1 : 0;
  }
  if (n_single > 0 && n_single < F) {
    snprintf(ctx->err, sizeof(ctx->err), "ovb_slam_delayed_init: ANCHORED_INVERSE_DEPTH_SINGLE mixed with a 3-wide representation in one call");
    return OVB_ERR_ARG;
  }
  for (int f = 0; f < F; f++)
    lm_off_out[f] = -1;
  if (F <= 0)
    return OVB_OK;
  ovb_status st = ovb_triangulate(ctx, frame, feats, opts, out);
  if (st != OVB_OK)
    return st;
  std::vector<double> Hf, Hx, res, HR, dx;
  std::vector<int32_t> colidx(OVB_MAX_COLS);
  for (int f = 0; f < F; f++) {
    if (out->status[f] != OVB_FEAT_OK)
      continue;
    const int m0 = feats->meas_off[f], m1 = feats->meas_off[f + 1], rows = 2 * (m1 - m0);
    int32_t moff[2] = {0, m1 - m0}, koff[2] = {0, 0};
    ovb_feat_batch v = *feats;
    v.n_feats = 1;
    v.n_meas = m1 - m0;
    v.meas_off = moff;
    v.cam = feats->cam + m0;
    v.clone = feats->clone + m0;
    v.uv = feats->uv + 2 * (size_t)m0;
    v.uvn = feats->uvn + 2 * (size_t)m0;
    if (feats->cam_keys_off && feats->cam_keys) {
      koff[1] = feats->cam_keys_off[f + 1] - feats->cam_keys_off[f];
      v.cam_keys_off = koff;
      v.cam_keys = feats->cam_keys + feats->cam_keys_off[f];
    }
    int32_t st1 = OVB_FEAT_OK, ac = out->anchor_cam[f], acl = out->anchor_clone[f];
    double pA[3] = {out->p_FinA[3 * f], out->p_FinA[3 * f + 1], out->p_FinA[3 * f + 2]};
    double pG[3] = {out->p_FinG[3 * f], out->p_FinG[3 * f + 1], out->p_FinG[3 * f + 2]}, c2 = 0;
    ovb_feat_out o1{&st1, pA, pG, &ac, &acl, &c2};
    Hf.assign((size_t)rows * 3, 0.0);
    Hx.assign((size_t)rows * OVB_MAX_COLS, 0.0);
    res.assign((size_t)rows, 0.0);
    int32_t row_off[2], ncols = 0;
    ovb_opts o_f = *opts;
    o_f.feat_rep = rep_of(f);
    const bool single = o_f.feat_rep == OVB_REP_ANCHORED_INVERSE_DEPTH_SINGLE;
    const int lm_size = single ? 1 : 3;
    st = ovb_feature_jacobians(ctx, frame, &v, &o_f, &o1, 0, Hf.data(), Hx.data(), res.data(), row_off, &ncols, colidx.data(), OVB_MAX_COLS);
    if (st != OVB_OK)
      return st;
    std::vector<int> used;
    for (int j = 0; j < ncols; j++) {
      bool nz = false;
      for (int i = 0; i < rows && !nz; i++)
        nz = Hx[(size_t)i * OVB_MAX_COLS + j] != 0.0;
      if (nz)
        used.push_back(j);
    }
    std::vector<int> off, sz;
    for (size_t a = 0; a < used.size();) {
      size_t b = a + 1;
      while (b < used.size() && colidx[(size_t)used[b]] == colidx[(size_t)used[b - 1]] + 1)
        b++;
      off.push_back(colidx[(size_t)used[a]]);
      sz.push_back((int)(b - a));
      a = b;
    }
    const int n = (int)used.size();
    HR.assign((size_t)rows * n, 0.0);
    for (int i = 0; i < rows; i++)
      for (int j = 0; j < n; j++)
        HR[(size_t)i * n + j] = Hx[(size_t)i * OVB_MAX_COLS + used[(size_t)j]];
    const double *HL = Hf.data(), *rs = res.data();
    int r = rows;
    if (single) {
      std::vector<double> Hb((size_t)rows * 2), X((size_t)rows * (n + 2));
      for (int i = 0; i < rows; i++) {
        Hb[(size_t)i * 2] = Hf[(size_t)i * 3];
        Hb[(size_t)i * 2 + 1] = Hf[(size_t)i * 3 + 1];
        for (int j = 0; j < n; j++)
          X[(size_t)i * (n + 2) + j] = HR[(size_t)i * n + j];
        X[(size_t)i * (n + 2) + n] = Hf[(size_t)i * 3 + 2];
        X[(size_t)i * (n + 2) + n + 1] = res[i];
      }
      nullspace_project_host(Hb.data(), 2, X.data(), n + 2, rows);
      r = rows - 2;
      HR.assign((size_t)r * n, 0.0);
      Hf.assign((size_t)r, 0.0);
      res.assign((size_t)r, 0.0);
      for (int i = 0; i < r; i++) {
        const double *xi = X.data() + (size_t)(i + 2) * (n + 2);
        for (int j = 0; j < n; j++)
          HR[(size_t)i * n + j] = xi[j];
        Hf[i] = xi[n];
        res[i] = xi[n + 1];
      }
      HL = Hf.data();
      rs = res.data();
    }
    const double sp = sigma_pix ? sigma_pix[f] : opts->sigma_pix, cm = chi2_multipler ? chi2_multipler[f] : opts->chi2_multipler;
    const int N0 = ctx->N;
    int accepted = 0;
    double dx_new[3] = {0, 0, 0};
    dx.assign((size_t)N0 + lm_size, 0.0);
    st = ovb_cov_initialize(ctx, off.data(), sz.data(), (int)off.size(), HR.data(), HL, rs, r, lm_size, sp * sp, cm, &accepted, dx_new, dx.data());
    if (st != OVB_OK)
      return st;
    if (!accepted) {
      out->status[f] = OVB_FEAT_CHI2;
      continue;
    }
    lm_off_out[f] = N0;
    if (on_init)
      on_init(user, f, N0, lm_size, dx_new, dx.data(), N0 + lm_size);
  }
  return OVB_OK;
}

__global__ void k_take_z(const double *R, int ldR, int rows, int col, double *w) {
  OVB_PDL_ENTER();
  int i = blockIdx.x * blockDim.x + threadIdx.x;
  if (i < rows)
    w[i] = R[(size_t)i * ldR + col];
}
__global__ void k_fill_zero_dx(double *dx, int N) {
  int i = blockIdx.x * blockDim.x + threadIdx.x;
  if (i < N)
    dx[i] = 0.0;
}

__global__ void k_group_take_z(const double *__restrict__ R, int ldR, int rows, int n, const int *__restrict__ col_state,
                               const double *__restrict__ dx_acc, double *__restrict__ w, DevUpdateInfo *__restrict__ info) {
  OVB_PDL_ENTER();
  const int i = blockIdx.x * blockDim.x + threadIdx.x;
  if (i < n)
    info->col_state[i] = col_state[i];
  if (i < rows) {
    const double *Ri = R + (size_t)i * ldR;
    double z = Ri[n];
    for (int j = 0; j < n; j++)
      z -= Ri[j] * dx_acc[col_state[j]];
    w[i] = z;
  }
}
__global__ void k_group_accumulate(const double *__restrict__ dx, double *__restrict__ dx_acc, int N, const DevUpdateInfo *__restrict__ info,
                                   int *__restrict__ flags) {
  OVB_PDL_ENTER();
  const int i = blockIdx.x * blockDim.x + threadIdx.x;
  if (i < N)
    dx_acc[i] += dx[i];
  if (i == 0) {
    if (info->not_spd)
      flags[0] = 1;
    if (info->nonfinite)
      flags[1] = 1;
  }
}
__global__ void k_group_finish(double *__restrict__ P, int ldP, int N, const double *__restrict__ P_prior, const double *__restrict__ dx_acc,
                               double *__restrict__ dx, DevUpdateInfo *__restrict__ info, const int *__restrict__ flags) {
  OVB_PDL_ENTER();
  const bool failed = flags[0] || flags[1] || info->neg_diag_index != 0x7fffffff;
  const int j = blockIdx.x * blockDim.x + threadIdx.x, i = blockIdx.y * blockDim.y + threadIdx.y;
  if (i == 0 && j < N)
    dx[j] = failed ? 0.0 : dx_acc[j];
  if (i == 0 && j == 0) {
    info->not_spd = flags[0];
    info->nonfinite = flags[1];
  }
  if (failed && i < N && j < N)
    P[(size_t)i * ldP + j] = P_prior[(size_t)i * ldP + j];
}

static int compress_system(ovb_ctx *ctx, int mode, double *A, int m, int n, int ldA, double *Rout, int ldR) {
  if (mode == OVB_COMPRESS_CHOLQR2 && launch_compress_cholqr2(ctx, A, m, n, ldA, Rout, ldR) >= 0)
    return n;
  if (mode == OVB_COMPRESS_NORMAL_EQUATIONS && launch_compress_gram(ctx, A, m, n, ldA, Rout, ldR) >= 0)
    return n;
  launch_tsqr(ctx, A, m, n, ldA, Rout, ldR);
  return std::min(m, n);
}

static int enqueue_slam_groups(ovb_ctx *ctx, int n_groups, int ldH);
static int enqueue_update(ovb_ctx *ctx, int F, BlobView bv, int ldH, int m_total, int n_all, int col_order, cudaEvent_t *ev,
                          bool slam = false, int n_groups = 1) {
  const int N = ctx->N;
  ctx->n_launch = 0;
  ctx->n_launch_tsqr_level = 0;
  ctx->prof_n = 0;
  if (!slam) {
    launch_cam_poses(ctx);
    launch_triangulate(ctx, F, bv);
    ctx->n_launch += 2;
  }
  ctx->n_launch += 1;
  if (ev)
    cudaEventRecord(ev[1], ctx->stream);
  launch_feature_system(ctx, F, bv, ldH, slam ? 2 : 0);
  if (ev)
    cudaEventRecord(ev[2], ctx->stream);
  {
    cudaEventRecord(ctx->ev_fork, ctx->stream);
    cudaStreamWaitEvent(ctx->side_stream, ctx->ev_fork, 0);
    cudaStream_t main_stream = ctx->stream;
    ctx->stream = ctx->side_stream;
    if (slam) {
      launch_column_map_slam(ctx, F, n_groups == 1);
    } else {
      launch_column_map(ctx, F, bv, 3);
    }
    ctx->stream = main_stream;
    cudaEventRecord(ctx->ev_join, ctx->side_stream);
  }
  if (ev)
    cudaEventRecord(ev[3], ctx->stream);
  if (slam && n_groups > 1) {
    cudaStreamWaitEvent(ctx->stream, ctx->ev_join, 0);
    if (ev)
      cudaEventRecord(ev[4], ctx->stream);
    const int r = enqueue_slam_groups(ctx, n_groups, ldH);
    if (ev)
      cudaEventRecord(ev[5], ctx->stream);
    return r;
  }
  const int ldR = ldH;
  const double *Rfinal = ctx->d_R;
  int r = 0;
  if (m_total > 0) {
    r = compress_system(ctx, ctx->h_opts->o.compress, ctx->d_Hs, m_total, n_all, ldH, ctx->d_R, ldR);
    cudaStreamWaitEvent(ctx->stream, ctx->ev_join, 0);
    if (col_order == OVB_COLS_REFERENCE_FIRST_SEEN) {
      launch_reorder_R(ctx, ctx->d_R, n_all, ldR, ctx->d_R2, ldR);
      Rfinal = ctx->d_R2;
    }
  }
  else
    cudaStreamWaitEvent(ctx->stream, ctx->ev_join, 0);
  if (ev)
    cudaEventRecord(ev[4], ctx->stream);
  if (r > 0) {
    ovb_launch(ctx, k_take_z, dim3((r + 127) / 128), dim3(128), (size_t)(0), Rfinal, ldR, r, n_all, ctx->d_w);
    launch_ekf_update(ctx, Rfinal, ldR, r, n_all, false, slam ? 1.0 : ctx->h_opts->sigma_pix_sq, nullptr);
    ctx->n_launch += 7;
  } else {
    k_fill_zero_dx<<<(N + 127) / 128, 128, 0, ctx->stream>>>(ctx->d_dx, N);
    ctx->n_launch += 1;
  }
  if (ev)
    cudaEventRecord(ev[5], ctx->stream);
  return r;
}

static int enqueue_slam_groups(ovb_ctx *ctx, int n_groups, int ldH) {
  const int N = ctx->N, ld = ctx->ldP;
  double *P = ctx->P[ctx->cur];
  double *acc = ctx->d_grp_acc;
  int *flags = (int *)(acc + ctx->cfg.max_state);
  cudaMemcpyAsync(ctx->P_snap, P, sizeof(double) * (size_t)ld * N, cudaMemcpyDeviceToDevice, ctx->stream);
  cudaMemsetAsync(acc, 0, sizeof(double) * ((size_t)ctx->cfg.max_state + 4), ctx->stream);
  int r_total = 0;
  for (int g = 0; g < n_groups; g++) {
    const DevGroup &G = ctx->h_grp[g];
    if (G.rows == 0)
      continue;
    const int n = G.n_cols;
    const int r = compress_system(ctx, ctx->h_opts->o.compress, ctx->d_Hs + (size_t)G.row0 * ldH, G.rows, n, ldH, ctx->d_R, ldH);
    ovb_launch(ctx, k_group_take_z, dim3((n + 127) / 128), dim3(128), (size_t)0, (const double *)ctx->d_R, ldH, r, n,
               (const int *)ctx->d_grp[g].col_state, (const double *)acc, ctx->d_w, ctx->d_info);
    launch_ekf_update(ctx, ctx->d_R, ldH, r, n, false, 1.0, nullptr);
    ovb_launch(ctx, k_group_accumulate, dim3((N + 255) / 256), dim3(256), (size_t)0, (const double *)ctx->d_dx, acc, N,
               (const DevUpdateInfo *)ctx->d_info, flags);
    ctx->n_launch += 8;
    r_total += r;
  }
  if (r_total > 0) {
    ovb_launch(ctx, k_group_finish, dim3((N + 31) / 32, (N + 7) / 8), dim3(32, 8), (size_t)0, P, ld, N, (const double *)ctx->P_snap,
               (const double *)acc, ctx->d_dx, ctx->d_info, (const int *)flags);
  } else {
    k_fill_zero_dx<<<(N + 127) / 128, 128, 0, ctx->stream>>>(ctx->d_dx, N);
  }
  ctx->n_launch += 1;
  return r_total;
}

ovb_status ovb_set_profile(ovb_ctx *ctx, int enabled) {
  if (!ctx)
    return OVB_ERR_ARG;
  OVB_CUDA_CHECK(ctx, cudaSetDevice(ctx->device));
  if (enabled && ctx->prof_ev[0] == nullptr)
    for (int i = 0; i < 2 * 96; i++)
      OVB_CUDA_CHECK(ctx, cudaEventCreate(&ctx->prof_ev[i]));
  ctx->prof_on = enabled ? 1 : 0;
  ctx->prof_n = 0;
  return OVB_OK;
}

ovb_status ovb_profile_read(ovb_ctx *ctx, char *names, int name_cap, float *us, int cap, int *n) {
  if (!ctx || !names || !us || !n || name_cap < 1)
    return OVB_ERR_ARG;
  OVB_CUDA_CHECK(ctx, cudaSetDevice(ctx->device));
  int w = 0, k = 0;
  for (; k < ctx->prof_n && k < cap; k++) {
    float ms = 0.f;
    if (cudaEventElapsedTime(&ms, ctx->prof_ev[2 * k], ctx->prof_ev[2 * k + 1]) != cudaSuccess)
      cudaGetLastError();
    us[k] = 1e3f * ms;
    const char *nm = nullptr;
    if (cudaFuncGetName(&nm, ctx->prof_fn[k]) != cudaSuccess || !nm) {
      cudaGetLastError();
      nm = "?";
    }
    for (const char *c = nm; *c && w < name_cap - 2; c++)
      names[w++] = *c;
    names[w++] = 0;
  }
  if (w < name_cap)
    names[w] = 0;
  *n = k;
  return OVB_OK;
}

ovb_status ovb_last_host_us(const ovb_ctx *ctx, double out[4]) {
  if (!ctx || !out)
    return OVB_ERR_ARG;
  for (int i = 0; i < 4; i++)
    out[i] = ctx->host_us[i];
  return OVB_OK;
}

ovb_status ovb_last_counters(const ovb_ctx *ctx, int64_t out[4]) {
  if (!ctx || !out)
    return OVB_ERR_ARG;
  out[0] = ctx->n_launch;
  out[1] = ctx->n_launch_tsqr_level;
  out[2] = (int64_t)ctx->last_h2d_bytes;
  out[3] = (int64_t)ctx->last_d2h_bytes;
  return OVB_OK;
}

ovb_status ovb_set_slam_unbounded(ovb_ctx *ctx, int enabled) {
  if (!ctx)
    return OVB_ERR_ARG;
  ctx->slam_unbounded = enabled ? 1 : 0;
  return OVB_OK;
}

ovb_status ovb_set_replay(ovb_ctx *ctx, int enabled) {
  if (!ctx)
    return OVB_ERR_ARG;
  OVB_CUDA_CHECK(ctx, cudaSetDevice(ctx->device));
  if (enabled && !ctx->P_snap)
    OVB_CUDA_CHECK(ctx, cudaMalloc(&ctx->P_snap, sizeof(double) * (size_t)ctx->ldP * ctx->ldP));
  ctx->replay_enabled = enabled ? 1 : 0;
  ctx->last_pk_valid = 0;
  return OVB_OK;
}

ovb_status ovb_msckf_replay(ovb_ctx *ctx, int steps, int flush_l2, float *ms_per_step, float stage_ms_sum[5]) {
  if (!ctx || steps < 1 || !ms_per_step)
    return OVB_ERR_ARG;
  if (!ctx->replay_enabled || !ctx->last_pk_valid) {
    snprintf(ctx->err, sizeof(ctx->err), "ovb_msckf_replay: call ovb_set_replay(ctx,1) and ovb_msckf_update first");
    return OVB_ERR_ARG;
  }
  OVB_CUDA_CHECK(ctx, cudaSetDevice(ctx->device));
  const size_t flush_bytes = (size_t)256 << 20;
  if (flush_l2 && !ctx->d_flush)
    OVB_CUDA_CHECK(ctx, cudaMalloc(&ctx->d_flush, flush_bytes));
  std::vector<cudaEvent_t> evs((size_t)steps * 6);
  for (auto &e : evs)
    OVB_CUDA_CHECK(ctx, cudaEventCreate(&e));
  const size_t Pbytes = sizeof(double) * (size_t)ctx->ldP * ctx->N;
  for (int s = 0; s < steps; s++) {
    if (flush_l2)
      cudaMemsetAsync(ctx->d_flush, s & 0xff, flush_bytes, ctx->stream);
    cudaMemcpyAsync(ctx->P[ctx->cur], ctx->P_snap, Pbytes, cudaMemcpyDeviceToDevice, ctx->stream);
    cudaEvent_t *ev = &evs[(size_t)s * 6];
    cudaEventRecord(ev[0], ctx->stream);
    enqueue_update(ctx, ctx->last_n_feats, ctx->last_bv, ctx->last_ldH, ctx->last_m_total, ctx->last_n_all, ctx->last_col_order,
                   ev);
  }
  OVB_CUDA_CHECK(ctx, cudaGetLastError());
  OVB_CUDA_CHECK(ctx, cudaStreamSynchronize(ctx->stream));
  if (stage_ms_sum)
    for (int k = 0; k < 5; k++)
      stage_ms_sum[k] = 0.f;
  for (int s = 0; s < steps; s++) {
    cudaEvent_t *ev = &evs[(size_t)s * 6];
    cudaEventElapsedTime(&ms_per_step[s], ev[0], ev[5]);
    if (stage_ms_sum)
      for (int k = 0; k < 5; k++) {
        float t;
        cudaEventElapsedTime(&t, ev[k], ev[k + 1]);
        stage_ms_sum[k] += t;
      }
  }
  for (auto &e : evs)
    cudaEventDestroy(e);
  return OVB_OK;
}

ovb_status ovb_msckf_update(ovb_ctx *ctx, const ovb_frame *frame, const ovb_feat_batch *feats, const ovb_opts *opts, ovb_feat_out *out,
                            double *dx, ovb_stats *stats) {
  if (!ctx || !dx)
    return OVB_ERR_ARG;
  if (ctx->N < 1) {
    snprintf(ctx->err, sizeof(ctx->err), "ovb_msckf_update: no covariance loaded (ovb_cov_set)");
    return OVB_ERR_ARG;
  }
  OVB_CUDA_CHECK(ctx, cudaSetDevice(ctx->device));
  const int N = ctx->N;
  if (stats) {
    memset(stats, 0, sizeof(*stats));
    stats->neg_diag_index = -1;
  }
  for (int i = 0; i < N; i++)
    dx[i] = 0.0;
  if (!feats || feats->n_feats <= 0)
    return OVB_OK;
  cudaEventRecord(ctx->ev[0], ctx->stream);
  const auto h0 = std::chrono::steady_clock::now();
  Packed pk;
  ovb_status st = pack_inputs(ctx, frame, feats, opts, nullptr, &pk);
  if (st != OVB_OK)
    return st;
// ... 109 lines not shown
    dx[i] = ctx->h_dx[i];
  ctx->stage_pending = 1;
  cudaEventElapsedTime(&ctx->stage_ms[5], ctx->ev[0], ctx->ev[6]);
  const DevUpdateInfo *inf = ctx->h_info;
  if (stats) {
    stats->n_feats_in = F;
    stats->n_feats_used = inf->n_feats_used;
    stats->rows_stacked = inf->rows_stacked;
    stats->cols_stacked = inf->n_used;
    stats->rows_update = inf->rows_stacked;
    stats->neg_diag_index = (r > 0 && inf->neg_diag_index != 0x7fffffff) ? inf->neg_diag_index : -1;
    stats->ms_total = ctx->stage_ms[5];
  }
  if (r > 0) {
    if (inf->not_spd) {
      snprintf(ctx->err, sizeof(ctx->err), "EKFUpdate: innovation covariance not positive definite");
      return OVB_ERR_NOT_SPD;
    }
    if (inf->nonfinite) {
      snprintf(ctx->err, sizeof(ctx->err), "EKFUpdate: non-finite covariance entry");
      return OVB_ERR_NONFINITE;
    }
    if (inf->neg_diag_index != 0x7fffffff) {
      snprintf(ctx->err, sizeof(ctx->err), "EKFUpdate: diagonal at %d is negative", inf->neg_diag_index);
      return OVB_ERR_NEG_DIAG;
    }
  }
  return OVB_OK;
}

ovb_status ovb_last_stage_ms(const ovb_ctx *ctx, float ms[6]) {
  if (!ctx || !ms)
    return OVB_ERR_ARG;
  if (ctx->stage_pending) {
    for (int s = 0; s < 5; s++)
      cudaEventElapsedTime(&ctx->stage_ms[s], ctx->ev[s], ctx->ev[s + 1]);
    ctx->stage_pending = 0;
  }
  for (int i = 0; i < 6; i++)
    ms[i] = ctx->stage_ms[i];
  return OVB_OK;
}

ovb_status ovb_set_stream(ovb_ctx *ctx, void *cuda_stream) {
  if (!ctx)
    return OVB_ERR_ARG;
  if (!cuda_stream) {
    snprintf(ctx->err, sizeof(ctx->err), "ovb_set_stream: pass an explicit (non-default) CUDA stream handle");
    return OVB_ERR_ARG;
  }
  OVB_CUDA_CHECK(ctx, cudaSetDevice(ctx->device));
  OVB_CUDA_CHECK(ctx, cudaStreamSynchronize(ctx->stream));
  if (ctx->own_stream && ctx->stream)
    cudaStreamDestroy(ctx->stream);
  ctx->stream = (cudaStream_t)cuda_stream;
  ctx->own_stream = 0;
  return OVB_OK;
}

ovb_status ovb_shard_partition(const int32_t *meas_off, int n_feats, int world, int32_t *bounds) {
  if (!meas_off || !bounds || n_feats < 0 || world < 1)
    return OVB_ERR_ARG;
  long long total = 0;
  for (int f = 0; f < n_feats; f++)
    total += std::max(2 * (meas_off[f + 1] - meas_off[f]) - 3, 0);
  bounds[0] = 0;
  long long cum = 0;
  int f = 0;
  for (int r = 1; r < world; r++) {
    const double target = (double)total * r / world;
    while (f < n_feats && (double)cum < target) {
      cum += std::max(2 * (meas_off[f + 1] - meas_off[f]) - 3, 0);
      f++;
    }
    bounds[r] = f;
  }
  bounds[world] = n_feats;
  return OVB_OK;
}

ovb_status ovb_msckf_shard_compress_range(ovb_ctx *ctx, const ovb_frame *frame, const ovb_feat_batch *feats, int f0, int f1, const ovb_opts *opts,
                                          double *R_dev, int R_cap_doubles, int *n_cols, int *ld) {
  if (!ctx || !feats || f0 < 0 || f1 < f0 || f1 > feats->n_feats)
    return OVB_ERR_ARG;
  const int F = f1 - f0, m0 = feats->meas_off[f0], m1 = feats->meas_off[f1];
  std::vector<int32_t> moff((size_t)F + 1), koff;
  for (int f = 0; f <= F; f++)
    moff[(size_t)f] = feats->meas_off[f0 + f] - m0;
  ovb_feat_batch v = *feats;
  v.n_feats = F;
  v.n_meas = m1 - m0;
  v.meas_off = moff.data();
  v.cam = feats->cam + m0;
  v.clone = feats->clone + m0;
  v.uv = feats->uv + 2 * (size_t)m0;
  v.uvn = feats->uvn + 2 * (size_t)m0;
  if (feats->cam_keys_off && feats->cam_keys) {
    const int k0 = feats->cam_keys_off[f0];
    koff.resize((size_t)F + 1);
    for (int f = 0; f <= F; f++)
      koff[(size_t)f] = feats->cam_keys_off[f0 + f] - k0;
    v.cam_keys_off = koff.data();
    v.cam_keys = feats->cam_keys + k0;
  }
  return ovb_msckf_shard_compress(ctx, frame, &v, opts, R_dev, R_cap_doubles, n_cols, ld);
}

ovb_status ovb_msckf_shard_compress(ovb_ctx *ctx, const ovb_frame *frame, const ovb_feat_batch *feats, const ovb_opts *opts, double *R_dev,
                                    int R_cap_doubles, int *n_cols, int *ld) {
  if (!ctx || !frame || !feats || !opts || !R_dev || !n_cols || !ld || ctx->N < 1)
    return OVB_ERR_ARG;
  OVB_CUDA_CHECK(ctx, cudaSetDevice(ctx->device));
  cudaEventRecord(ctx->ev[0], ctx->stream);
  Packed pk;
  ovb_opts o2 = *opts;
  o2.col_order = OVB_COLS_CANONICAL;
  ovb_status st = pack_inputs(ctx, frame, feats, &o2, nullptr, &pk);
  if (st != OVB_OK)
    return st;
  cudaEventRecord(ctx->ev[1], ctx->stream);
  *n_cols = pk.n_all;
  *ld = pk.ldH;
  if ((size_t)pk.n_all * pk.ldH > (size_t)R_cap_doubles)
    return OVB_ERR_CAPACITY;
  ctx->last_n_feats = pk.n_feats;
  ctx->last_n_all = pk.n_all;
  ctx->last_ldH = pk.ldH;
  ctx->n_launch = 0;
  ctx->n_launch_tsqr_level = 0;
  launch_cam_poses(ctx);
  launch_triangulate(ctx, pk.n_feats, pk.bv);
  launch_feature_system(ctx, pk.n_feats, pk.bv, pk.ldH, 0);
  launch_column_map(ctx, pk.n_feats, pk.bv);
  ctx->n_launch += 3;
  if (pk.m_total > 0)
    compress_system(ctx, o2.compress, ctx->d_Hs, pk.m_total, pk.n_all, pk.ldH, R_dev, pk.ldH);
  else
    OVB_CUDA_CHECK(ctx, cudaMemsetAsync(R_dev, 0, sizeof(double) * (size_t)pk.n_all * pk.ldH, ctx->stream));
  cudaEventRecord(ctx->ev[4], ctx->stream);
  OVB_CUDA_CHECK(ctx, cudaGetLastError());
  return OVB_OK;
}

ovb_status ovb_msckf_shard_finish(ovb_ctx *ctx, double *stacked_dev, int n_blocks, ovb_feat_out *out, double *dx, ovb_stats *stats) {
  if (!ctx || !stacked_dev || n_blocks < 1 || !dx || ctx->N < 1)
    return OVB_ERR_ARG;
  OVB_CUDA_CHECK(ctx, cudaSetDevice(ctx->device));
  const int N = ctx->N, n_all = ctx->last_n_all, ld = ctx->last_ldH, F = ctx->last_n_feats;
  const double *Rfinal = stacked_dev;
  if (n_blocks > 1) {
    compress_system(ctx, ctx->h_opts->o.compress, stacked_dev, n_blocks * n_all, n_all, ld, ctx->d_R, ld);
    Rfinal = ctx->d_R;
  }
  ovb_launch(ctx, k_take_z, dim3((n_all + 127) / 128), dim3(128), (size_t)(0), Rfinal, ld, n_all, n_all, ctx->d_w);
  launch_ekf_update(ctx, Rfinal, ld, n_all, n_all, false, ctx->h_opts->sigma_pix_sq, nullptr);
  ctx->n_launch += 7;
  cudaEventRecord(ctx->ev[5], ctx->stream);
  OVB_CUDA_CHECK(ctx, cudaGetLastError());
  OVB_CUDA_CHECK(ctx, cudaMemcpyAsync(ctx->h_feat, ctx->d_feat, sizeof(DevFeat) * (size_t)F, cudaMemcpyDeviceToHost, ctx->stream));
  OVB_CUDA_CHECK(ctx, cudaMemcpyAsync(ctx->h_info, ctx->d_info, ctx->info_bytes + sizeof(double) * (size_t)N, cudaMemcpyDeviceToHost,
                                      ctx->stream));
  ctx->last_d2h_bytes = sizeof(DevFeat) * (size_t)F + ctx->info_bytes + sizeof(double) * (size_t)N;
  cudaEventRecord(ctx->ev[6], ctx->stream);
  OVB_CUDA_CHECK(ctx, cudaStreamSynchronize(ctx->stream));
  unpack_feats(ctx, F, out);
  for (int i = 0; i < N; i++)
    dx[i] = ctx->h_dx[i];
  ctx->stage_pending = 0;
  cudaEventElapsedTime(&ctx->stage_ms[5], ctx->ev[0], ctx->ev[6]);
  cudaEventElapsedTime(&ctx->stage_ms[3], ctx->ev[0], ctx->ev[4]);
  cudaEventElapsedTime(&ctx->stage_ms[4], ctx->ev[4], ctx->ev[5]);
  cudaEventElapsedTime(&ctx->stage_ms[0], ctx->ev[1], ctx->ev[5]);
  const DevUpdateInfo *inf = ctx->h_info;
  if (stats) {
    memset(stats, 0, sizeof(*stats));
    stats->n_feats_in = F;
    int used = 0, rows = 0;
    for (int f = 0; f < F; f++)
      if (ctx->h_feat[f].status == OVB_FEAT_OK) {
        used++;
        rows += 2 * (ctx->h_feat[f].m1 - ctx->h_feat[f].m0) - 3;
      }
    stats->n_feats_used = used;
    stats->rows_stacked = rows;
    stats->cols_stacked = n_all;
    stats->rows_update = n_all;
    stats->neg_diag_index = inf->neg_diag_index != 0x7fffffff ? inf->neg_diag_index : -1;
    stats->ms_total = ctx->stage_ms[5];
  }
  if (inf->not_spd)
    return OVB_ERR_NOT_SPD;
  if (inf->nonfinite)
    return OVB_ERR_NONFINITE;
  if (inf->neg_diag_index != 0x7fffffff)
    return OVB_ERR_NEG_DIAG;
  return OVB_OK;
}

__global__ void k_whiten_rows(double *A, int ld, int m, int ncols) {
  int i = blockIdx.x;
  double s = 1.0 / sqrt(A[(size_t)i * ld + ncols]);
  __syncthreads();
  for (int j = threadIdx.x; j < ncols; j += blockDim.x)
    A[(size_t)i * ld + j] *= s;
}

static ovb_status ensure_stage(ovb_ctx *ctx, size_t doubles) {
  if (doubles <= ctx->stage_cap && ctx->h_stage)
    return OVB_OK;
  if (ctx->h_stage)
    cudaFreeHost(ctx->h_stage);
  ctx->h_stage = nullptr;
  ctx->stage_cap = 0;
  OVB_CUDA_CHECK(ctx, cudaMallocHost(&ctx->h_stage, sizeof(double) * doubles));
  ctx->stage_cap = doubles;
  return OVB_OK;
}

static ovb_status stage_dense(ovb_ctx *ctx, const double *H, int m, int n, const double *res, const double *extra, int *ld_out) {
  int ld = (int)align_up((size_t)n + 2, 4);
  if ((size_t)std::max(m, n) * ld > ctx->Hs_cap) {
    snprintf(ctx->err, sizeof(ctx->err), "dense system %d x %d exceeds the reserved staging matrix (max_rows/max_state)", m, n);
    return OVB_ERR_CAPACITY;
  }
  ovb_status st = ensure_stage(ctx, (size_t)std::max(m, n) * ld);
  if (st != OVB_OK)
    return st;
  double *hs = ctx->h_stage;
  for (int i = 0; i < m; i++) {
    memcpy(hs + (size_t)i * ld, H + (size_t)i * n, sizeof(double) * n);
    hs[(size_t)i * ld + n] = res[i];
    for (int j = n + 1; j < ld; j++)
      hs[(size_t)i * ld + j] = 0.0;
    if (extra)
      hs[(size_t)i * ld + n + 1] = extra[i];
  }
  OVB_CUDA_CHECK(ctx, cudaMemcpyAsync(ctx->d_Hs, hs, sizeof(double) * (size_t)m * ld, cudaMemcpyHostToDevice, ctx->stream));
  *ld_out = ld;
  return OVB_OK;
}

ovb_status ovb_compress(ovb_ctx *ctx, const double *H, int m, int n, const double *res, double *R_out, double *z_out) {
  if (!ctx || !H || !res || !R_out || !z_out || m < 1 || n < 1)
    return OVB_ERR_ARG;
  if (n + 8 > ctx->cfg.max_state + 8)
    return OVB_ERR_CAPACITY;
  OVB_CUDA_CHECK(ctx, cudaSetDevice(ctx->device));
  int ld;
  ovb_status st = stage_dense(ctx, H, m, n, res, nullptr, &ld);
  if (st != OVB_OK)
    return st;
  launch_tsqr(ctx, ctx->d_Hs, m, n, ld, ctx->d_R, ld);
  OVB_CUDA_CHECK(ctx, cudaGetLastError());
  double *hs = ctx->h_stage;
  OVB_CUDA_CHECK(ctx, cudaMemcpyAsync(hs, ctx->d_R, sizeof(double) * (size_t)n * ld, cudaMemcpyDeviceToHost, ctx->stream));
  OVB_CUDA_CHECK(ctx, cudaStreamSynchronize(ctx->stream));
  for (int i = 0; i < n; i++) {
    for (int j = 0; j < n; j++)
      R_out[(size_t)i * n + j] = hs[(size_t)i * ld + j];
    z_out[i] = hs[(size_t)i * ld + n];
  }
  return OVB_OK;
}

ovb_status ovb_compress_gram(ovb_ctx *ctx, const double *H, int m, int n, const double *res, double *R_out, double *z_out) {
  if (!ctx || !H || !res || !R_out || !z_out || m < 1 || n < 1)
    return OVB_ERR_ARG;
  if (n > ctx->cfg.max_state)
    return OVB_ERR_CAPACITY;
  OVB_CUDA_CHECK(ctx, cudaSetDevice(ctx->device));
  int ld;
  ovb_status st = stage_dense(ctx, H, m, n, res, nullptr, &ld);
  if (st != OVB_OK)
    return st;
  if (launch_compress_gram(ctx, ctx->d_Hs, m, n, ld, ctx->d_R, ld) < 0)
    return OVB_ERR_CUDA;
  OVB_CUDA_CHECK(ctx, cudaGetLastError());
  double *hs = ctx->h_stage;
  OVB_CUDA_CHECK(ctx, cudaMemcpyAsync(hs, ctx->d_R, sizeof(double) * (size_t)n * ld, cudaMemcpyDeviceToHost, ctx->stream));
  OVB_CUDA_CHECK(ctx, cudaStreamSynchronize(ctx->stream));
  for (int i = 0; i < n; i++) {
    for (int j = 0; j < n; j++)
      R_out[(size_t)i * n + j] = hs[(size_t)i * ld + j];
    z_out[i] = hs[(size_t)i * ld + n];
  }
  return OVB_OK;
}

ovb_status ovb_compress_cholqr2(ovb_ctx *ctx, const double *H, int m, int n, const double *res, double *R_out, double *z_out) {
  if (!ctx || !H || !res || !R_out || !z_out || m < 1 || n < 1)
    return OVB_ERR_ARG;
  if (n > ctx->cfg.max_state)
    return OVB_ERR_CAPACITY;
  OVB_CUDA_CHECK(ctx, cudaSetDevice(ctx->device));
  int ld;
  ovb_status st = stage_dense(ctx, H, m, n, res, nullptr, &ld);
  if (st != OVB_OK)
    return st;
  if (launch_compress_cholqr2(ctx, ctx->d_Hs, m, n, ld, ctx->d_R, ld) < 0) {
    snprintf(ctx->err, sizeof(ctx->err), "ovb_compress_cholqr2: %d columns exceed what this path takes", n);
    return OVB_ERR_CAPACITY;
  }
  OVB_CUDA_CHECK(ctx, cudaGetLastError());
  double *hs = ctx->h_stage;
  OVB_CUDA_CHECK(ctx, cudaMemcpyAsync(hs, ctx->d_R, sizeof(double) * (size_t)n * ld, cudaMemcpyDeviceToHost, ctx->stream));
  OVB_CUDA_CHECK(ctx, cudaStreamSynchronize(ctx->stream));
  for (int i = 0; i < n; i++) {
    for (int j = 0; j < n; j++)
      R_out[(size_t)i * n + j] = hs[(size_t)i * ld + j];
    z_out[i] = hs[(size_t)i * ld + n];
  }
  return OVB_OK;
}

ovb_status ovb_ekf_update(ovb_ctx *ctx, const int *off, const int *sz, int nvar, const double *H, int r, const double *res, double sigma2,
                          const double *Rdiag, double *dx) {
  if (!ctx || !off || !sz || !H || !res || !dx || nvar < 1 || r < 1)
    return OVB_ERR_ARG;
  if (ctx->N < 1)
    return OVB_ERR_ARG;
  const int N = ctx->N;
  int n = 0;
  for (int i = 0; i < nvar; i++) {
    if (off[i] < 0 || sz[i] < 1 || off[i] + sz[i] > N)
      return OVB_ERR_ARG;
    n += sz[i];
  }
  if (n > OVB_MAX_COLS || n > ctx->cfg.max_state)
    return OVB_ERR_CAPACITY;
  OVB_CUDA_CHECK(ctx, cudaSetDevice(ctx->device));
  if (Rdiag)
    for (int i = 0; i < r; i++)
      if (!(Rdiag[i] > 0.0))
        return OVB_ERR_ARG;
  int ld;
  ovb_status st = stage_dense(ctx, H, r, n, res, Rdiag, &ld);
  if (st != OVB_OK)
    return st;
  DevUpdateInfo *hi = ctx->h_info;
  memset(hi, 0, sizeof(*hi));
  int c = 0;
  for (int i = 0; i < nvar; i++)
    for (int k = 0; k < sz[i]; k++)
      hi->col_state[c++] = off[i] + k;
  OVB_CUDA_CHECK(ctx, cudaMemcpyAsync(ctx->d_info, hi, sizeof(DevUpdateInfo), cudaMemcpyHostToDevice, ctx->stream));
  const double *Hdev = ctx->d_Hs;
  int rr = r;
  double s2 = sigma2;
  if (Rdiag) {
    k_whiten_rows<<<r, 128, 0, ctx->stream>>>(ctx->d_Hs, ld, r, n + 1);
    s2 = 1.0;
  }
  if (r > n) {
    rr = compress_system(ctx, OVB_COMPRESS_CHOLQR2, ctx->d_Hs, r, n, ld, ctx->d_R, ld);
    Hdev = ctx->d_R;
  }
  ovb_launch(ctx, k_take_z, dim3((rr + 127) / 128), dim3(128), (size_t)(0), Hdev, ld, rr, n, ctx->d_w);
  launch_ekf_update(ctx, Hdev, ld, rr, n, false, s2, nullptr);
  OVB_CUDA_CHECK(ctx, cudaGetLastError());
  OVB_CUDA_CHECK(ctx, cudaMemcpyAsync(ctx->h_info, ctx->d_info, sizeof(DevUpdateInfo), cudaMemcpyDeviceToHost, ctx->stream));
  OVB_CUDA_CHECK(ctx, cudaMemcpyAsync(ctx->h_dx, ctx->d_dx, sizeof(double) * (size_t)N, cudaMemcpyDeviceToHost, ctx->stream));
  OVB_CUDA_CHECK(ctx, cudaStreamSynchronize(ctx->stream));
  for (int i = 0; i < N; i++)
    dx[i] = ctx->h_dx[i];
  if (ctx->h_info->not_spd) {
    snprintf(ctx->err, sizeof(ctx->err), "EKFUpdate: innovation covariance not positive definite");
    return OVB_ERR_NOT_SPD;
  }
  if (ctx->h_info->nonfinite)
    return OVB_ERR_NONFINITE;
  if (ctx->h_info->neg_diag_index != 0x7fffffff) {
    snprintf(ctx->err, sizeof(ctx->err), "EKFUpdate: diagonal at %d is negative", ctx->h_info->neg_diag_index);
    return OVB_ERR_NEG_DIAG;
  }
  return OVB_OK;
}

ovb_status ovb_cov_initialize(ovb_ctx *ctx, const int *off, const int *sz, int nvar, const double *H_R_in, const double *H_L_in,
                              const double *res_in, int r, int k, double sigma2, double chi2_mult, int *accepted, double *dx_new, double *dx) {
  if (!ctx || !off || !sz || !H_R_in || !H_L_in || !res_in || !accepted || !dx_new || !dx || nvar < 1 || k < 1 || k > 3 || r < k)
    return OVB_ERR_ARG;
  if (ctx->N < 1 || !(sigma2 > 0.0))
    return OVB_ERR_ARG;
  const int N = ctx->N;
  int n = 0;
  for (int i = 0; i < nvar; i++) {
    if (off[i] < 0 || sz[i] < 1 || off[i] + sz[i] > N)
      return OVB_ERR_ARG;
    n += sz[i];
  }
  if (n > OVB_MAX_COLS || n > ctx->cfg.max_state)
    return OVB_ERR_CAPACITY;
  if (N + k > ctx->ldP) {
    snprintf(ctx->err, sizeof(ctx->err), "initialize: covariance would grow to %d (max_state %d)", N + k, ctx->ldP);
    return OVB_ERR_CAPACITY;
  }
  OVB_CUDA_CHECK(ctx, cudaSetDevice(ctx->device));
  *accepted = 0;
  std::vector<double> HR(H_R_in, H_R_in + (size_t)r * n), HL(H_L_in, H_L_in + (size_t)r * k), res(res_in, res_in + r);
  auto rot = [](double c, double s, double &x, double &y) {
    const double x0 = x, y0 = y;
    x = c * x0 - s * y0;
    y = s * x0 + c * y0;
  };
  for (int c0 = 0; c0 < k; ++c0) {
    for (int m = r - 1; m > c0; m--) {
      double gc, gs;
      make_givens(HL[(size_t)(m - 1) * k + c0], HL[(size_t)m * k + c0], gc, gs);
      for (int j = c0; j < k; j++)
        rot(gc, gs, HL[(size_t)(m - 1) * k + j], HL[(size_t)m * k + j]);
      rot(gc, gs, res[m - 1], res[m]);
      for (int j = 0; j < n; j++)
        rot(gc, gs, HR[(size_t)(m - 1) * n + j], HR[(size_t)m * n + j]);
    }
  }
  double A[9], Inv[9];
  for (int i = 0; i < k; i++)
    for (int j = 0; j < k; j++) {
      A[i * k + j] = HL[(size_t)i * k + j];
      Inv[i * k + j] = (i == j) ? 1.0 : 0.0;
    }
  for (int c0 = 0; c0 < k; c0++) {
    int piv = c0;
    for (int i = c0 + 1; i < k; i++)
      if (std::fabs(A[i * k + c0]) > std::fabs(A[piv * k + c0]))
        piv = i;
    if (!(std::fabs(A[piv * k + c0]) > 0.0)) {
      snprintf(ctx->err, sizeof(ctx->err), "initialize: H_L is rank deficient");
      return OVB_ERR_ARG;
    }
    if (piv != c0)
      for (int j = 0; j < k; j++) {
        std::swap(A[c0 * k + j], A[piv * k + j]);
        std::swap(Inv[c0 * k + j], Inv[piv * k + j]);
      }
    const double d = A[c0 * k + c0];
    for (int j = 0; j < k; j++) {
      A[c0 * k + j] /= d;
      Inv[c0 * k + j] /= d;
    }
    for (int i = 0; i < k; i++) {
      if (i == c0)
        continue;
      const double f = A[i * k + c0];
      for (int j = 0; j < k; j++) {
        A[i * k + j] -= f * A[c0 * k + j];
        Inv[i * k + j] -= f * Inv[c0 * k + j];
      }
    }
  }
  DevUpdateInfo *hi = ctx->h_info;
  memset(hi, 0, sizeof(*hi));
  {
    int c = 0;
    for (int i = 0; i < nvar; i++)
      for (int q = 0; q < sz[i]; q++)
        hi->col_state[c++] = off[i] + q;
  }
  const int rup = r - k;
  const double *Hdev = nullptr;
  int ld = 0, rr = 0;
  if (rup > 0) {
    ovb_status st = stage_dense(ctx, HR.data() + (size_t)k * n, rup, n, res.data() + k, nullptr, &ld);
    if (st != OVB_OK)
      return st;
    OVB_CUDA_CHECK(ctx, cudaMemcpyAsync(ctx->d_info, hi, sizeof(DevUpdateInfo), cudaMemcpyHostToDevice, ctx->stream));
    Hdev = ctx->d_Hs;
    rr = rup;
    double res2 = 0.0;
    for (int i = k; i < r; i++)
      res2 += res[i] * res[i];
    const bool compressed = rup > n;
    if (compressed) {
      launch_tsqr(ctx, ctx->d_Hs, rup, n, ld, ctx->d_R, ld);
      Hdev = ctx->d_R;
      rr = n;
    }
    ovb_launch(ctx, k_take_z, dim3((rr + 127) / 128), dim3(128), (size_t)(0), Hdev, ld, rr, n, ctx->d_w);
    std::vector<double> zh((size_t)rr), wh((size_t)rr);
    OVB_CUDA_CHECK(ctx, cudaMemcpyAsync(zh.data(), ctx->d_w, sizeof(double) * (size_t)rr, cudaMemcpyDeviceToHost, ctx->stream));
    launch_ekf_update(ctx, Hdev, ld, rr, n, true, sigma2, nullptr);
    OVB_CUDA_CHECK(ctx, cudaGetLastError());
    OVB_CUDA_CHECK(ctx, cudaMemcpyAsync(wh.data(), ctx->d_w, sizeof(double) * (size_t)rr, cudaMemcpyDeviceToHost, ctx->stream));
    OVB_CUDA_CHECK(ctx, cudaMemcpyAsync(ctx->h_info, ctx->d_info, sizeof(DevUpdateInfo), cudaMemcpyDeviceToHost, ctx->stream));
    OVB_CUDA_CHECK(ctx, cudaStreamSynchronize(ctx->stream));
    double chi2 = 0.0, z2 = 0.0;
    for (int i = 0; i < rr; i++) {
      chi2 += wh[(size_t)i] * wh[(size_t)i];
      z2 += zh[(size_t)i] * zh[(size_t)i];
    }
    if (compressed)
      chi2 += std::max(0.0, res2 - z2) / sigma2;
    if (ctx->h_info->not_spd)
      chi2 = NAN;
    const double chi2_check = g_chi2_table[std::min(r, OVB_CHI2_TABLE_LEN - 1)];
    if (!(chi2 <= chi2_mult * chi2_check))
      return OVB_OK;
  } else {
    OVB_CUDA_CHECK(ctx, cudaMemcpyAsync(ctx->d_info, hi, sizeof(DevUpdateInfo), cudaMemcpyHostToDevice, ctx->stream));
  }
  {
    std::vector<double> stage((size_t)k * n + (size_t)k * k);
    for (int i = 0; i < k; i++)
      for (int j = 0; j < n; j++)
        stage[(size_t)i * n + j] = HR[(size_t)i * n + j];
    for (int i = 0; i < k * k; i++)
      stage[(size_t)k * n + i] = Inv[i];
    OVB_CUDA_CHECK(ctx, cudaMemcpyAsync(ctx->d_Y, stage.data(), sizeof(double) * stage.size(), cudaMemcpyHostToDevice, ctx->stream));
    const bool launched = launch_cov_init_augment(ctx, k, n, ctx->d_Y, ctx->d_Y + (size_t)k * n, sigma2);
    OVB_CUDA_CHECK(ctx, cudaStreamSynchronize(ctx->stream));
    if (!launched) {
      snprintf(ctx->err, sizeof(ctx->err), "ovb_cov_initialize: covariance augmentation kernel could not be launched (N=%d, k=%d)", N, k);
      return OVB_ERR_CAPACITY;
    }
  }
  ctx->N = N + k;
  for (int q = 0; q < k; q++) {
    double acc = 0.0;
    for (int i = 0; i < k; i++)
      acc += Inv[q * k + i] * res[i];
    dx_new[q] = acc;
  }
  *accepted = 1;
  for (int i = 0; i < N + k; i++)
    dx[i] = 0.0;
  if (rup > 0) {
    ovb_launch(ctx, k_take_z, dim3((rr + 127) / 128), dim3(128), (size_t)(0), Hdev, ld, rr, n, ctx->d_w);
    launch_ekf_update(ctx, Hdev, ld, rr, n, false, sigma2, nullptr);
    OVB_CUDA_CHECK(ctx, cudaGetLastError());
    OVB_CUDA_CHECK(ctx, cudaMemcpyAsync(ctx->h_info, ctx->d_info, sizeof(DevUpdateInfo), cudaMemcpyDeviceToHost, ctx->stream));
    OVB_CUDA_CHECK(ctx, cudaMemcpyAsync(ctx->h_dx, ctx->d_dx, sizeof(double) * (size_t)(N + k), cudaMemcpyDeviceToHost, ctx->stream));
    OVB_CUDA_CHECK(ctx, cudaStreamSynchronize(ctx->stream));
    for (int i = 0; i < N + k; i++)
      dx[i] = ctx->h_dx[i];
    if (ctx->h_info->not_spd) {
      snprintf(ctx->err, sizeof(ctx->err), "EKFUpdate: innovation covariance not positive definite");
      return OVB_ERR_NOT_SPD;
    }
    if (ctx->h_info->nonfinite)
      return OVB_ERR_NONFINITE;
    if (ctx->h_info->neg_diag_index != 0x7fffffff) {
      snprintf(ctx->err, sizeof(ctx->err), "EKFUpdate: diagonal at %d is negative", ctx->h_info->neg_diag_index);
      return OVB_ERR_NEG_DIAG;
    }
  }
  return OVB_OK;
}

}
```

open_vins_b200/csrc/ovb_internal.cuh:

```cuda
#pragma once
#include "../../include/ovb200.h"
#include <cuda_runtime.h>
#include <stdint.h>

#define OVB_BIG_MAX_MEAS 128
#define OVB_MAX_COLS 512
#define OVB_NB 16
#define OVB_CR 256

struct DevFrame {
  int n_clones, n_cams;
  int n_slots;
  int n_all;
  double clone_R[OVB_MAX_CLONES][9];
  double clone_p[OVB_MAX_CLONES][3];
  double clone_R_fej[OVB_MAX_CLONES][9];
  double clone_p_fej[OVB_MAX_CLONES][3];
  double cam_R[OVB_MAX_CAMS][9];
  double cam_p[OVB_MAX_CAMS][3];
  double cam_intr[OVB_MAX_CAMS][8];
  int cam_model[OVB_MAX_CAMS];
  int slot_off[OVB_MAX_VARS];
  int slot_size[OVB_MAX_VARS];
  int slot_col[OVB_MAX_VARS];
  int clone_slot[OVB_MAX_CLONES];
  int cam_ext_slot[OVB_MAX_CAMS];
  int cam_intr_slot[OVB_MAX_CAMS];
  const struct DevGroup *groups;
  int lm_w;
};

struct DevGroup {
  int f0, f1;
  int row0, rows;
  int n_cols;
  int n_ent;
  int ent[OVB_MAX_VARS + OVB_MAX_COLS];
  int col_state[OVB_MAX_COLS];
  short col_frame[OVB_MAX_COLS];
};

struct DevCamPoses {
  double cc_R[OVB_MAX_CAMS][OVB_MAX_CLONES][9];
  double cc_p[OVB_MAX_CAMS][OVB_MAX_CLONES][3];
};

struct DevOpts {
  ovb_opts o;
  double sigma_pix_sq;
  int rep;
};

struct DevFeat {
  int m0, m1;
  int row0;
  int key0, key1;
  int status;
  int anchor_cam, anchor_clone;
  int sched;
  int rep;
  double p_FinA[3], p_FinG[3];
  double chi2;
  double p_FinG_fej[3];
  double sigma_sq;
  double chi2_mult;
  int lm_off;
  unsigned short lm_col, grp;
};

struct DevUpdateInfo {
  int n_used;
  int n_feats_used;
  int rows_stacked;
  int n_order;
  int order_slot[OVB_MAX_VARS];
  int col_state[OVB_MAX_COLS];
  int col_canon[OVB_MAX_COLS];
  int neg_diag_index;
  int not_spd;
  int nonfinite;
};

struct BlobView {
  const uint8_t *cam;
  const uint16_t *clone;
  const float *uv;
  const float *uvn;
  const uint8_t *keys;
};

struct ovb_ctx {
  ovb_config cfg;
  int device;
  cudaStream_t stream;
  int own_stream;
  cudaStream_t side_stream;
  cudaStream_t side_stream2;
  cudaEvent_t ev_fork, ev_join, ev_join2;
  int feat_classes;
  cudaEvent_t ev[8];
  char err[256];
  int N, ldP;
  double *P[2];
  int cur;
  unsigned char *d_arena, *h_arena;
  size_t arena_bytes, off_opts, off_feat, off_blob;
  DevFrame *d_frame;
  DevOpts *d_opts;
  DevFeat *d_feat;
  unsigned char *d_blob;
  DevFrame *h_frame;
  DevOpts *h_opts;
  DevFeat *h_feat;
  unsigned char *h_blob;
  size_t blob_cap;
  DevCamPoses *d_cc;
  unsigned char *d_feat_order;
  DevUpdateInfo *d_info;
  DevUpdateInfo *h_info;
  double *h_dx;
  double *h_stage;
  size_t stage_cap;
  double *d_chi2_table;
  double *d_Hs;
  size_t Hs_cap;
  double *d_W[2];
  size_t W_cap;
  double *d_R;
  double *d_R2;
  double *d_M;
  double *d_S;
  double *d_Y;
  double *d_w;
  double *d_dx;
  double *d_scratch;
  size_t scratch_per_cta;
  int scratch_ctas;
  double *d_long;
  size_t long_cap;
  double *d_dump;
  size_t dump_cap;
  int dump_rows;
  int max_rows;
  int sm_count;
  size_t info_bytes;
  int attr_done[8];
  int tsqr_pdl;
  int tsqr_cluster;
  int gram_cluster;
  int ekf_chol_dmma;
  mutable float stage_ms[6];
  mutable int stage_pending;
  double host_us[4];
  int replay_enabled, last_pk_valid;
  int last_n_feats, last_m_total, last_ldH, last_n_all, last_col_order;
  BlobView last_bv;
  double *P_snap;
  void *d_flush;
  DevGroup *d_grp, *h_grp;
  int grp_cap;
  double *d_grp_acc;
  int slam_unbounded;
  int n_launch, n_launch_tsqr_level;
  double *d_Gpart, *d_G;
  size_t Gpart_cap, G_cap;
  double *d_cqw;
  size_t cqw_cap;
  size_t last_h2d_bytes, last_d2h_bytes;
  int prof_on, prof_n;
  cudaEvent_t prof_ev[2 * 96];
  const void *prof_fn[96];
};

#define OVB_CUDA_CHECK(ctx, call)                                                                                     \
  do {                                                                                                                \
    cudaError_t e_ = (call);                                                                                          \
    if (e_ != cudaSuccess) {                                                                                          \
      snprintf((ctx)->err, sizeof((ctx)->err), "%s:%d %s: %s", __FILE__, __LINE__, #call, cudaGetErrorString(e_));    \
      return OVB_ERR_CUDA;                                                                                            \
    }                                                                                                                 \
  } while (0)

void launch_cam_poses(ovb_ctx *ctx);
void launch_triangulate(ovb_ctx *ctx, int n_feats, BlobView bv);
void launch_feature_system(ovb_ctx *ctx, int n_feats, BlobView bv, int ldH, int mode);
ovb_status feature_scratch_reserve(ovb_ctx *ctx, int n_feats, bool slam);
void launch_column_map(ovb_ctx *ctx, int n_feats, BlobView bv, int rows_drop = 3);
void launch_column_map_slam(ovb_ctx *ctx, int n_feats, bool full_map);
void launch_tsqr(ovb_ctx *ctx, double *A, int m, int n, int ldA, double *Rout, int ldR);
int launch_compress_gram(ovb_ctx *ctx, const double *A, int m, int n, int ldA, double *Rout, int ldR);
int launch_compress_cholqr2(ovb_ctx *ctx, double *A, int m, int n, int ldA, double *Rout, int ldR);
bool launch_chol_ekf_dmma(ovb_ctx *ctx, double *S, int ldS, int r, const double *res, double *w, double *invdiag, double **Lpk_out);
bool launch_trsm_rows(ovb_ctx *ctx, double *A, int ldA, int m, int nt, const double *Lpk);
bool launch_chol_solve_wide(ovb_ctx *ctx, double *S, int ldS, int r, double *w, double *invdiag, double *M, int ldM, int N, bool gate_only);
void launch_reorder_R(ovb_ctx *ctx, const double *Rin, int n_all, int ldRin, double *Rout, int ldRout);
void launch_ekf_update(ovb_ctx *ctx, const double *H, int ldHm, int r_max, int n_max, bool sizes_from_info, double sigma2,
                       const double *Rdiag_dev);
bool launch_cov_init_augment(ovb_ctx *ctx, int k, int n, const double *Hx_dev, const double *Hinv_dev, double sigma2);
void launch_cov_clone(ovb_ctx *ctx, int old_off, int size, const double *dnc_dt_dev, int dt_off);
void launch_cov_marginalize(ovb_ctx *ctx, int off, int size);
void launch_cov_propagate(ovb_ctx *ctx, int new_off, int p, int q, const int *old_idx_dev, const double *Phi_dev, const double *Q_dev);

#define OVB_PDL_ENTER()                                                     \
  do {                                                                      \
    asm volatile("griddepcontrol.launch_dependents;" ::: "memory");         \
    asm volatile("griddepcontrol.wait;" ::: "memory");                      \
  } while (0)

#ifdef __CUDACC__
template <typename... KArgs, typename... Args>
static inline void ovb_launch(ovb_ctx *ctx, void (*kern)(KArgs...), dim3 grid, dim3 block, size_t smem, Args &&...args) {
  cudaLaunchConfig_t cfg = {};
  cfg.gridDim = grid;
  cfg.blockDim = block;
  cfg.dynamicSmemBytes = smem;
  cfg.stream = ctx->stream;
  cudaLaunchAttribute at[1];
  at[0].id = cudaLaunchAttributeProgrammaticStreamSerialization;
  at[0].val.programmaticStreamSerializationAllowed = 1;
  cfg.attrs = at;
  cfg.numAttrs = (ctx->tsqr_pdl && !ctx->prof_on) ? 1 : 0;
  const bool prof = ctx->prof_on && ctx->prof_n < 96 && ctx->prof_ev[0] != nullptr;
  if (prof)
    cudaEventRecord(ctx->prof_ev[2 * ctx->prof_n], ctx->stream);
  cudaLaunchKernelEx(&cfg, kern, static_cast<KArgs>(args)...);
  if (prof) {
    cudaEventRecord(ctx->prof_ev[2 * ctx->prof_n + 1], ctx->stream);
    ctx->prof_fn[ctx->prof_n++] = (const void *)kern;
  }
}
#endif
```

Measured before the change: 2309.

## Fuse EKF Cholesky and gain TRSM into a cluster kernel with DSMEM panel broadcast

Adds a thread-block-cluster kernel in which CTA 0 runs the tiled DMMA Cholesky of the innovation covariance. After each panel step it pushes the panel block and the 8x8 inverse to peer CTAs with bulk copies into distributed shared memory, synchronised by mbarriers. The peer CTAs keep their slice of the gain matrix in shared memory and do the triangular solve in lockstep. Separately, the k_take_z launch is dropped by reading the residual column straight into the factorization. This removes separate kernel launches and the global round trips between Cholesky and TRSM, at the cost of a complex cluster handshake, an occupancy probe, and reliance on cluster size limits.

```diff
diff --git a/open_vins_b200/csrc/chol_tiles.cuh b/open_vins_b200/csrc/chol_tiles.cuh
--- a/open_vins_b200/csrc/chol_tiles.cuh
+++ b/open_vins_b200/csrc/chol_tiles.cuh
@@ -112,16 +112,18 @@
   }
 }
 
-__device__ __forceinline__ void ct_panel_tile(const CtView &sm, int i, int k, const double *Linv, double *Xb) {
+__device__ __forceinline__ void ct_panel_at(double *t, const double *Linv, double *xrow) {
   const int lane = threadIdx.x & 31, g = lane >> 2, q = lane & 3;
-  double *t = sm.T + (size_t)(ct_tri(i) + k) * 64;
   const double a0 = t[g * 8 + q], a1 = t[g * 8 + q + 4];
   const double b0 = Linv[g * 8 + q], b1 = Linv[g * 8 + q + 4];
   double2 d = make_double2(0.0, 0.0);
   ct_dmma(d.x, d.y, a0, b0);
   ct_dmma(d.x, d.y, a1, b1);
   *reinterpret_cast<double2 *>(t + 2 * lane) = d;
-  *reinterpret_cast<double2 *>(Xb + (size_t)(8 * i + g) * CT_XP + 2 * q) = d;
+  *reinterpret_cast<double2 *>(xrow + (size_t)g * CT_XP + 2 * q) = d;
+}
+__device__ __forceinline__ void ct_panel_tile(const CtView &sm, int i, int k, const double *Linv, double *Xb) {
+  ct_panel_at(sm.T + (size_t)(ct_tri(i) + k) * 64, Linv, Xb + (size_t)(8 * i) * CT_XP);
 }
 
 __device__ __forceinline__ void ct_panel_rows(double *T, double *Xp, const double *invd, int i0, int stride, int nrows, int k, int nbk) {
@@ -206,17 +208,18 @@
 #define CT_PROBE_T(v) do { } while (0)
 #endif
 
-__device__ __forceinline__ void ct_trail_row(const CtView &sm, const double *Xk, int bi, int j0, int jmax, int lane) {
+__device__ __forceinline__ void ct_trail_span(double *trow, const double *xrow, const double *Xk, int j0, int jmax, int lane, const double *dummyX,
+                                              double *dummyT) {
   const int g = lane >> 2, q = lane & 3;
-  const double *xa = Xk + (size_t)(8 * bi + g) * CT_XP + q;
+  const double *xa = xrow + (size_t)g * CT_XP + q;
   const double a0 = -xa[0], a1 = -xa[4];
-  double *trow = sm.T + (size_t)ct_tri(bi) * 64 + 2 * lane;
+  trow += 2 * lane;
   for (int bj = j0; bj <= jmax; bj += 2) {
     const bool two = bj + 1 <= jmax;
     const double *xb0 = Xk + (size_t)(8 * bj + g) * CT_XP + q;
-    const double *xb1 = two ? xb0 + 8 * CT_XP : sm.dummyX + q;
+    const double *xb1 = two ? xb0 + 8 * CT_XP : dummyX + q;
     double2 *c0p = reinterpret_cast<double2 *>(trow + (size_t)bj * 64);
-    double2 *c1p = two ? c0p + 32 : reinterpret_cast<double2 *>(sm.dummyT + 2 * lane);
+    double2 *c1p = two ? c0p + 32 : reinterpret_cast<double2 *>(dummyT + 2 * lane);
     const double b00 = xb0[0], b01 = xb0[4], b10 = xb1[0], b11 = xb1[4];
     double2 c0 = *c0p, c1 = *c1p;
     ct_dmma(c0.x, c0.y, a0, b00);
@@ -227,9 +230,18 @@
     *c1p = c1;
   }
 }
-
-template <int THREADS>
-__device__ __forceinline__ void ct_chol_tiles(const CtView &sm, int n, int nrows, bool strict, double floor_d) {
+__device__ __forceinline__ void ct_trail_row(const CtView &sm, const double *Xk, int bi, int j0, int jmax, int lane) {
+  ct_trail_span(sm.T + (size_t)ct_tri(bi) * 64, Xk + (size_t)(8 * bi) * CT_XP, Xk, j0, jmax, lane, sm.dummyX, sm.dummyT);
+}
+
+struct CtNoPeers {
+  __device__ __forceinline__ void written() const {}
+  __device__ __forceinline__ void push(int, int, const double *, const double *) const {}
+  __device__ __forceinline__ void reuse(int) const {}
+};
+
+template <int THREADS, class Peers = CtNoPeers>
+__device__ __forceinline__ void ct_chol_tiles(const CtView &sm, int n, int nrows, bool strict, double floor_d, const Peers &peers = Peers()) {
   const int tid = threadIdx.x, lane = tid & 31, wid = tid >> 5;
   constexpr int NW = THREADS / 32, NH = NW - (NW + 3) / 4;
   static_assert(NH >= 1, "need at least one helper warp");
@@ -248,9 +260,11 @@
     if (LINV)
       asm volatile("bar.arrive 3, 64;" ::: "memory");
     ct_panel_rows(sm.T, sm.Xp0, sm.invd, lane < 8 ? 8 + lane : nrows, 1 << 30, nrows, 0, min(8, n));
+    peers.written();
   } else if (LINV && wid == 4) {
     asm volatile("bar.sync 3, 64;" ::: "memory");
     ct_linv8(sm.T, sm.invd, sm.Linv0);
+    peers.written();
   }
   __syncthreads();
   for (int k = 0; k < NB; k++) {
@@ -276,13 +290,19 @@
         CT_PROBE_T(p2);
         asm volatile("bar.sync 2, %0;" ::"r"((NH + 1) * 32) : "memory");
         CT_PROBE_T(p3);
+        if (k > 0)
+          peers.reuse(k - 1);
         ct_panel_rows(sm.T, Xn, sm.invd, lane < 8 ? 8 * (k + 2) + lane : nrows, 1 << 30, nrows, k1, nbk1);
+        peers.written();
         CT_PROBE_T(p4);
       }
     } else if (LINV && wid == 4) {
       if (more) {
         asm volatile("bar.sync 3, 64;" ::: "memory");
+        if (k > 0)
+          peers.reuse(k - 1);
         ct_linv8(sm.T + (size_t)(ct_tri(k + 1) + k + 1) * 64, sm.invd + 8 * (k + 1), par ? sm.Linv0 : sm.Linv1);
+        peers.written();
       }
     } else if (helper) {
       if (LINV) {
@@ -292,10 +312,13 @@
       } else {
         ct_panel_rows(sm.T, Xk, sm.invd, 8 * (k + 2) + hr * 32 + lane, NH * 32, nrows, k, min(8, n - 8 * k));
       }
+      peers.written();
       if (NH > 1)
         ct_bar_group(1, NH * 32);
       else
         __syncwarp();
+      if (hr == 0)
+        peers.push(k, NRB, Xk, LINV ? (par ? sm.Linv1 : sm.Linv0) : nullptr);
       CT_PROBE_T(p1);
       if (more) {
         for (int i = k + 2 + hr; i < NRB; i += 2 * NH) {
diff --git a/open_vins_b200/csrc/k_cholqr.cu b/open_vins_b200/csrc/k_cholqr.cu
--- a/open_vins_b200/csrc/k_cholqr.cu
+++ b/open_vins_b200/csrc/k_cholqr.cu
@@ -255,7 +255,8 @@
 
 namespace {
 
-__device__ __forceinline__ void cq_chol_tiles(CqCholSmem &sm, int n, int nrows, bool strict, double floor_d) {
+template <class Peers = CtNoPeers>
+__device__ __forceinline__ void cq_chol_tiles(CqCholSmem &sm, int n, int nrows, bool strict, double floor_d, const Peers &peers = Peers()) {
   CtView v;
   v.T = sm.T;
   v.Xp0 = sm.Xp[0];
@@ -266,7 +267,7 @@
   v.dummyT = sm.dummyT;
   v.dummyX = sm.dummyX;
   v.flag = &sm.flag;
-  ct_chol_tiles<CQ_CHOL_T>(v, n, nrows, strict, floor_d);
+  ct_chol_tiles<CQ_CHOL_T>(v, n, nrows, strict, floor_d, peers);
 }
 
 __device__ void cq_load_tiles(CqCholSmem &sm, const double *__restrict__ G, size_t ldG, int n, int nrows, const double *__restrict__ rhs, int ld_rhs) {
@@ -415,6 +416,192 @@
     info->not_spd = 1;
 }
 
+#define CQ_GAIN_RB 13
+#define CQ_GAIN_MAXP 7
+struct CqGainSmem {
+  double Mt[CQ_GAIN_RB * CQ_MAXB * 64];
+  double Yb[CQ_GAIN_RB * 8 * CQ_XP];
+  double Rx[2][CQ_MAXRB * 8 * CQ_XP];
+  double RL[2][64];
+  double dummyT[64];
+  double dummyX[2 * CQ_XP];
+};
+#define CQ_GAIN_SMEM (sizeof(CqGainSmem) > sizeof(CqCholSmem) ? sizeof(CqGainSmem) : sizeof(CqCholSmem))
+static_assert(CQ_GAIN_SMEM + 64 <= 227 * 1024, "k_cq_chol_gain's shared memory (dynamic + mbarriers) must fit one SM");
+
+namespace {
+__device__ __forceinline__ unsigned cq_mapa(unsigned a, unsigned rank) {
+  unsigned r;
+  asm volatile("mapa.shared::cluster.u32 %0, %1, %2;" : "=r"(r) : "r"(a), "r"(rank));
+  return r;
+}
+__device__ __forceinline__ void cq_mbar_wait(unsigned bar, unsigned parity) {
+  unsigned ok = 0;
+  do {
+    asm volatile("{\n\t.reg .pred p;\n\tmbarrier.try_wait.parity.acquire.cluster.shared::cta.b64 p, [%1], %2;\n\tselp.u32 %0, 1, 0, p;\n\t}"
+                 : "=r"(ok)
+                 : "r"(bar), "r"(parity)
+                 : "memory");
+  } while (!ok);
+}
+__device__ __forceinline__ void cq_mbar_arrive_remote(unsigned bar_cluster) {
+  asm volatile("mbarrier.arrive.release.cluster.shared::cluster.b64 _, [%0];" ::"r"(bar_cluster) : "memory");
+}
+__device__ __forceinline__ void cq_cluster_sync() {
+  asm volatile("barrier.cluster.arrive.release.aligned;\n\tbarrier.cluster.wait.acquire.aligned;" ::: "memory");
+}
+
+struct CqGainLink {
+  unsigned src_bar, free_bar;
+  unsigned full_bar;
+  unsigned rx, rl;
+  int npeer;
+  __device__ __forceinline__ void written() const { asm volatile("fence.proxy.async.shared::cta;" ::: "memory"); }
+  __device__ __forceinline__ void reuse(int k) const { cq_mbar_wait(src_bar + 8 * (k & 1), (k >> 1) & 1); }
+  __device__ __forceinline__ void push(int k, int NRB, const double *Xk, const double *Linv) const {
+    if ((threadIdx.x & 31) == 0) {
+      const int s = k & 1;
+      if (k >= 2)
+        cq_mbar_wait(free_bar + 8 * s, ((k - 2) >> 1) & 1);
+      const unsigned off = (unsigned)(8 * (k + 1) * CQ_XP * sizeof(double));
+      const unsigned bx = (unsigned)(8 * (NRB - k - 1) * CQ_XP * sizeof(double)), bl = 64 * sizeof(double);
+      const unsigned slot = rx + (unsigned)(s * CQ_MAXRB * 8 * CQ_XP * sizeof(double)) + off, lslot = rl + (unsigned)(s * bl);
+      for (int p = 1; p <= npeer; p++) {
+        const unsigned bar = cq_mapa(full_bar + 8 * s, p);
+        asm volatile("mbarrier.arrive.expect_tx.release.cluster.shared::cluster.b64 _, [%0], %1;" ::"r"(bar), "r"(bx + bl) : "memory");
+        if (bx)
+          asm volatile("cp.async.bulk.shared::cluster.shared::cta.mbarrier::complete_tx::bytes [%0], [%1], %2, [%3];" ::"r"(cq_mapa(slot, p)),
+                       "r"(s_u32(Xk) + off), "r"(bx), "r"(bar)
+                       : "memory");
+        asm volatile("cp.async.bulk.shared::cluster.shared::cta.mbarrier::complete_tx::bytes [%0], [%1], %2, [%3];" ::"r"(cq_mapa(lslot, p)),
+                     "r"(s_u32(Linv)), "r"(bl), "r"(bar)
+                     : "memory");
+      }
+    }
+    __syncwarp();
+  }
+};
+}
+
+__global__ void __launch_bounds__(CQ_CHOL_T) k_cq_chol_gain(const double *__restrict__ Spk, int r, const double *__restrict__ z, int ldz, double *__restrict__ M,
+                                                           int ldM, int N, double *__restrict__ w, DevUpdateInfo *__restrict__ info) {
+  extern __shared__ __align__(16) unsigned char cq_raw[];
+  __shared__ __align__(8) unsigned long long gbar[5];
+  const int tid = threadIdx.x, lane = tid & 31, wid = tid >> 5;
+  unsigned rank, nct;
+  asm volatile("mov.u32 %0, %%cluster_ctarank;" : "=r"(rank));
+  asm volatile("mov.u32 %0, %%cluster_nctarank;" : "=r"(nct));
+  const int npeer = (int)nct - 1;
+  const int NB = (r + 7) >> 3, NRB = (r + 8) >> 3;
+  CqGainSmem &ps = *reinterpret_cast<CqGainSmem *>(cq_raw);
+  if (tid == 0) {
+    for (int b = 0; b < 5; b++)
+      if (rank == 0 || b == 1 || b == 2)
+        asm volatile("mbarrier.init.shared::cta.b64 [%0], %1;" ::"r"(s_u32(&gbar[b])), "r"((rank == 0 && b > 0) ? npeer : 1) : "memory");
+    asm volatile("fence.mbarrier_init.release.cluster;" ::: "memory");
+  }
+  cq_cluster_sync();
+  OVB_PDL_ENTER();
+  if (rank == 0) {
+    CqCholSmem &sm = *reinterpret_cast<CqCholSmem *>(cq_raw);
+    const unsigned bar = s_u32(&gbar[0]);
+    if (tid == 0) {
+      const unsigned bytes = (unsigned)(tri(NB) * 64 * sizeof(double));
+      asm volatile("mbarrier.arrive.expect_tx.shared::cta.b64 _, [%0], %1;" ::"r"(bar), "r"(bytes) : "memory");
+      asm volatile("cp.async.bulk.shared::cluster.global.mbarrier::complete_tx::bytes [%0], [%1], %2, [%3];" ::"r"(s_u32(sm.T)), "l"(Spk), "r"(bytes), "r"(bar)
+                   : "memory");
+    }
+    for (int e = tid; e < 2 * CQ_MAXRB * 8 * CQ_XP; e += CQ_CHOL_T)
+      (&sm.Xp[0][0])[e] = 0.0;
+    if (tid < 64)
+      sm.dummyT[tid] = 0.0;
+    if (tid < 2 * CQ_XP)
+      sm.dummyX[tid] = 0.0;
+    if (tid == 0)
+      sm.flag = 0;
+    cq_mbar_wait(bar, 0);
+    for (int e = tid; e < (tri(NRB) - tri(NB - 1)) * 64; e += CQ_CHOL_T) {
+      const int t = tri(NB - 1) + (e >> 6);
+      int bi = NB - 1;
+      while (tri(bi + 1) <= t)
+        bi++;
+      const int row = 8 * bi + ((e >> 3) & 7), col = 8 * (t - tri(bi)) + (e & 7);
+      if (row >= r || col >= r)
+        sm.T[(size_t)t * 64 + (e & 63)] = 0.0;
+    }
+    __syncthreads();
+    for (int j = tid; j < r; j += CQ_CHOL_T)
+      sm.T[ct_idx(r, j)] = z[(size_t)j * ldz];
+    __syncthreads();
+    CqGainLink link;
+    link.src_bar = s_u32(&gbar[1]);
+    link.free_bar = s_u32(&gbar[3]);
+    link.full_bar = s_u32(&gbar[1]);
+    link.rx = s_u32(ps.Rx[0]);
+    link.rl = s_u32(ps.RL[0]);
+    link.npeer = npeer;
+    cq_chol_tiles(sm, r, r + 1, true, 0.0, link);
+    for (int j = tid; j < r; j += CQ_CHOL_T)
+      w[j] = cq_el(sm.T, r, j);
+    if (tid == 0 && sm.flag)
+      info->not_spd = 1;
+  } else {
+    const int NBM = (N + 7) >> 3, p = (int)rank - 1;
+    const int b0 = p * NBM / npeer, nib = (p + 1) * NBM / npeer - b0;
+    const int units = NB * 4;
+    for (int e = tid; e < nib * 8 * units; e += CQ_CHOL_T) {
+      const int a = e / units, col = 2 * (e - a * units), row = 8 * b0 + a;
+      const unsigned bytes = row < N ? ((col + 1 < r) ? 16u : (col < r ? 8u : 0u)) : 0u;
+      double *dst = ps.Mt + (size_t)((a >> 3) * CQ_MAXB + (col >> 3)) * 64 + (a & 7) * 8 + (col & 7);
+      cpa16(s_u32(dst), bytes ? (const void *)(M + (size_t)row * ldM + col) : (const void *)M, bytes);
+    }
+    cpa_commit();
+    if (tid < 64)
+      ps.dummyT[tid] = 0.0;
+    if (tid < 2 * CQ_XP)
+      ps.dummyX[tid] = 0.0;
+    cpa_wait<0>();
+    __syncthreads();
+    constexpr int CW = CQ_CHOL_T / 32 - 1;
+    const unsigned full = s_u32(&gbar[1]);
+    if (wid == CW) {
+      for (int k = 0; k < NB; k++) {
+        cq_mbar_wait(full + 8 * (k & 1), (k >> 1) & 1);
+        if (lane == 0)
+          cq_mbar_arrive_remote(cq_mapa(s_u32(&gbar[1 + (k & 1)]), 0));
+      }
+    } else {
+      for (int k = 0; k < NB; k++) {
+        const int s = k & 1;
+        cq_mbar_wait(full + 8 * s, (k >> 1) & 1);
+        for (int ib = wid; ib < nib; ib += CW)
+          ct_panel_at(ps.Mt + (size_t)(ib * CQ_MAXB + k) * 64, ps.RL[s], ps.Yb + (size_t)ib * 8 * CQ_XP);
+        bar_group(1, CW * 32);
+        const int ppr = (NB - k) >> 1;
+        for (int e = wid; e < nib * ppr; e += CW) {
+          const int ib = e / ppr, j = k + 1 + 2 * (e - ib * ppr);
+          ct_trail_span(ps.Mt + (size_t)ib * CQ_MAXB * 64, ps.Yb + (size_t)ib * 8 * CQ_XP, ps.Rx[s], j, min(j + 1, NB - 1), lane, ps.dummyX, ps.dummyT);
+        }
+        bar_group(1, CW * 32);
+        if (tid == 0)
+          cq_mbar_arrive_remote(cq_mapa(s_u32(&gbar[3 + s]), 0));
+      }
+    }
+    __syncthreads();
+    for (int e = tid; e < nib * 8 * units; e += CQ_CHOL_T) {
+      const int a = e / units, col = 2 * (e - a * units), row = 8 * b0 + a;
+      if (row >= N || col >= r)
+        continue;
+      const double *src = ps.Mt + (size_t)((a >> 3) * CQ_MAXB + (col >> 3)) * 64 + (a & 7) * 8 + (col & 7);
+      if (col + 1 < r)
+        *reinterpret_cast<double2 *>(M + (size_t)row * ldM + col) = *reinterpret_cast<const double2 *>(src);
+      else
+        M[(size_t)row * ldM + col] = src[0];
+    }
+  }
+  cq_cluster_sync();
+}
+
 #define CQ_TRSM_NH 10
 #define CQ_TRSM_SMEM (sizeof(double) * ((size_t)CQ_PK_DOUBLES + (size_t)(CQ_TRSM_T / 32) * CQ_TRSM_NH * 2 * 32))
 template <int NH>
@@ -931,6 +1118,7 @@
     cudaFuncSetAttribute(k_cq_gram, cudaFuncAttributeMaxDynamicSharedMemorySize, 160 * 1024);
     cudaFuncSetAttribute(k_cq_chol_gram, cudaFuncAttributeMaxDynamicSharedMemorySize, (int)sizeof(CqCholSmem));
     cudaFuncSetAttribute(k_cq_chol_ekf, cudaFuncAttributeMaxDynamicSharedMemorySize, (int)sizeof(CqCholSmem));
+    cudaFuncSetAttribute(k_cq_chol_gain, cudaFuncAttributeMaxDynamicSharedMemorySize, (int)CQ_GAIN_SMEM);
     cudaFuncSetAttribute(k_cq_trsm<5, 0>, cudaFuncAttributeMaxDynamicSharedMemorySize, (int)CQ_TRSM_SMEM);
     cudaFuncSetAttribute(k_cq_trsm<10, 0>, cudaFuncAttributeMaxDynamicSharedMemorySize, (int)CQ_TRSM_SMEM);
     cudaFuncSetAttribute(k_cq_trsm<10, 5>, cudaFuncAttributeMaxDynamicSharedMemorySize, (int)CQ_TRSM_SMEM);
@@ -988,6 +1176,70 @@
     ctas = ctx->sm_count;
   cq_launch_trsm(ctx, ctas, A, ldA, m, nt, Lpk);
   return true;
+}
+
+static int cq_gain_peers(int N) {
+  const int p = ((N + 7) / 8 + CQ_GAIN_RB - 1) / CQ_GAIN_RB;
+  return (p >= 1 && p <= CQ_GAIN_MAXP) ? p : 0;
+}
+
+bool chol_gain_fits(ovb_ctx *ctx, int r, int N, int ldM) {
+  const int P = cq_gain_peers(N);
+  if (r < 1 || r > CQ_MAXN || (ldM & 1) || P == 0)
+    return false;
+  const size_t NB = (size_t)(r + 7) / 8;
+  if (NB * (NB + 1) / 2 * 64 > (size_t)(ctx->cfg.max_state + 1) * ctx->cfg.max_state)
+    return false;
+  cq_attrs(ctx);
+  if (ctx->gain_cluster_ok[P] == 0) {
+    cudaLaunchConfig_t cfg = {};
+    cfg.gridDim = dim3(1 + P);
+    cfg.blockDim = dim3(CQ_CHOL_T);
+    cfg.dynamicSmemBytes = CQ_GAIN_SMEM;
+    cudaLaunchAttribute at;
+    at.id = cudaLaunchAttributeClusterDimension;
+    at.val.clusterDim.x = 1 + P;
+    at.val.clusterDim.y = 1;
+    at.val.clusterDim.z = 1;
+    cfg.attrs = &at;
+    cfg.numAttrs = 1;
+    int nclusters = 0;
+    const bool ok = cudaOccupancyMaxActiveClusters(&nclusters, k_cq_chol_gain, &cfg) == cudaSuccess && nclusters >= 1;
+    cudaGetLastError();
+    ctx->gain_cluster_ok[P] = ok ? 1 : -1;
+  }
+  return ctx->gain_cluster_ok[P] > 0;
+}
+
+void launch_chol_gain(ovb_ctx *ctx, const double *Spk, int r, const double *z, int ldz, double *M, int ldM, int N, double *w) {
+  const int P = cq_gain_peers(N);
+  cudaLaunchConfig_t cfg = {};
+  cfg.gridDim = dim3(1 + P);
+  cfg.blockDim = dim3(CQ_CHOL_T);
+  cfg.dynamicSmemBytes = CQ_GAIN_SMEM;
+  cfg.stream = ctx->stream;
+  cudaLaunchAttribute at[2];
+  int na = 0;
+  at[na].id = cudaLaunchAttributeClusterDimension;
+  at[na].val.clusterDim.x = 1 + P;
+  at[na].val.clusterDim.y = 1;
+  at[na].val.clusterDim.z = 1;
+  na++;
+  if (ctx->tsqr_pdl && !ctx->prof_on) {
+    at[na].id = cudaLaunchAttributeProgrammaticStreamSerialization;
+    at[na].val.programmaticStreamSerializationAllowed = 1;
+    na++;
+  }
+  cfg.attrs = at;
+  cfg.numAttrs = na;
+  const bool prof = ctx->prof_on && ctx->prof_n < 96 && ctx->prof_ev[0] != nullptr;
+  if (prof)
+    cudaEventRecord(ctx->prof_ev[2 * ctx->prof_n], ctx->stream);
+  cudaLaunchKernelEx(&cfg, k_cq_chol_gain, Spk, r, z, ldz, M, ldM, N, w, ctx->d_info);
+  if (prof) {
+    cudaEventRecord(ctx->prof_ev[2 * ctx->prof_n + 1], ctx->stream);
+    ctx->prof_fn[ctx->prof_n++] = (const void *)k_cq_chol_gain;
+  }
 }
 
 #define CQ_WB 128
diff --git a/open_vins_b200/csrc/k_ekf.cu b/open_vins_b200/csrc/k_ekf.cu
--- a/open_vins_b200/csrc/k_ekf.cu
+++ b/open_vins_b200/csrc/k_ekf.cu
@@ -234,14 +234,19 @@
   asm volatile("cp.async.ca.shared.global [%0], [%1], 8;" ::"r"((unsigned)__cvta_generic_to_shared(dst_smem)), "l"(src) : "memory");
 }
 __global__ void __launch_bounds__(256) k_ekf_gemm1(int mode, const double *__restrict__ P, int ldP, const double *__restrict__ H, int ldH,
-                                                   const double *__restrict__ Min, int ldM, const DevUpdateInfo *__restrict__ info, int X, int Y,
+                                                   const double *__restrict__ Min, int ldM, DevUpdateInfo *__restrict__ info, int X, int Y,
                                                    int K, double *__restrict__ Cout, int ldC, double sigma2, const double *__restrict__ Rdiag) {
   OVB_PDL_ENTER();
   extern __shared__ __align__(16) double g1[];
   const int x0 = blockIdx.x * EK_T, y0 = blockIdx.y * EK_T;
-  if (mode == 1 && y0 > x0 + EK_T - 1)
+  if (mode != 0 && y0 > x0 + EK_T - 1)
     return;
   const int tid = threadIdx.x, tx = tid & 31, ty = tid >> 5;
+  if (mode == 0 && x0 == 0 && y0 == 0 && tid == 0) {
+    info->neg_diag_index = 0x7fffffff;
+    info->not_spd = 0;
+    info->nonfinite = 0;
+  }
   const int *cs = info->col_state;
   const int pk = K | 1;
   double *Gs = g1, *Hs = g1 + (size_t)K * 33;
@@ -298,7 +303,10 @@
         double v = acc[u];
         if (i == k)
           v += Rdiag ? Rdiag[i] : sigma2;
-        Cout[(size_t)i * ldC + k] = v;
+        if (mode == 1)
+          Cout[(size_t)i * ldC + k] = v;
+        else if ((k >> 3) <= (i >> 3))
+          Cout[(size_t)((((i >> 3) * ((i >> 3) + 1)) >> 1) + (k >> 3)) * 64 + (i & 7) * 8 + (k & 7)] = v;
       }
     }
   }
@@ -368,6 +376,13 @@
   }
 }
 
+__global__ void k_take_z(const double *z, int ldz, int rows, double *w) {
+  OVB_PDL_ENTER();
+  int i = blockIdx.x * blockDim.x + threadIdx.x;
+  if (i < rows)
+    w[i] = z[(size_t)i * ldz];
+}
+
 __global__ void k_ekf_prep(DevUpdateInfo *info) {
   OVB_PDL_ENTER();
   info->neg_diag_index = 0x7fffffff;
@@ -375,13 +390,18 @@
   info->nonfinite = 0;
 }
 
-void launch_ekf_update(ovb_ctx *ctx, const double *H, int ldHm, int r, int n, bool gate_only, double sigma2, const double *Rdiag_dev) {
+int launch_ekf_update(ovb_ctx *ctx, const double *H, int ldHm, int r, int n, bool gate_only, double sigma2, const double *Rdiag_dev, const double *z, int ldz) {
   const int N = ctx->N;
   const int ld = ctx->ldP;
   double *P = ctx->P[ctx->cur];
-  ovb_launch(ctx, k_ekf_prep, dim3(1), dim3(1), (size_t)(0), ctx->d_info);
+  const bool one_shot = ctx->ekf_chol_dmma && n <= EK1_KMAX && r <= EK1_KMAX && r > 0 && n > 0;
+  int launches = 0;
+  if (!one_shot) {
+    ovb_launch(ctx, k_ekf_prep, dim3(1), dim3(1), (size_t)(0), ctx->d_info);
+    launches++;
+  }
   if (r <= 0 || n <= 0)
-    return;
+    return launches;
   if (!ctx->attr_done[2]) {
     cudaFuncSetAttribute(k_ekf_chol, cudaFuncAttributeMaxDynamicSharedMemorySize, 200 * 1024);
     cudaFuncSetAttribute(k_ekf_trsm, cudaFuncAttributeMaxDynamicSharedMemorySize, 200 * 1024);
@@ -389,16 +409,28 @@
     cudaFuncSetAttribute(k_ekf_downdate1, cudaFuncAttributeMaxDynamicSharedMemorySize, 100 * 1024);
     ctx->attr_done[2] = 1;
   }
-  const bool one_shot = ctx->ekf_chol_dmma && n <= EK1_KMAX && r <= EK1_KMAX;
+  const bool fused = one_shot && !gate_only && ctx->ekf_fused && chol_gain_fits(ctx, r, N, ld);
+  if (!fused && z != nullptr) {
+    ovb_launch(ctx, k_take_z, dim3((r + 127) / 128), dim3(128), (size_t)(0), z, ldz, r, ctx->d_w);
+    launches++;
+  }
   dim3 g0((N + EK_T - 1) / EK_T, (r + EK_T - 1) / EK_T);
   dim3 g1((r + EK_T - 1) / EK_T, (r + EK_T - 1) / EK_T);
+  dim3 g2((N + EK_T - 1) / EK_T, (N + EK_T - 1) / EK_T);
   if (one_shot) {
     const size_t sm01 = sizeof(double) * ((size_t)n * 33 + (size_t)32 * (n | 1));
     ovb_launch(ctx, k_ekf_gemm1, dim3(g0), dim3(256), sm01, 0, P, ld, H, ldHm, nullptr, 0, ctx->d_info, N, r, n, ctx->d_M, ld, 0.0, nullptr);
-    ovb_launch(ctx, k_ekf_gemm1, dim3(g1), dim3(256), sm01, 1, P, ld, H, ldHm, ctx->d_M, ld, ctx->d_info, r, r, n, ctx->d_S, ld, sigma2, Rdiag_dev);
+    ovb_launch(ctx, k_ekf_gemm1, dim3(g1), dim3(256), sm01, fused ? 2 : 1, P, ld, H, ldHm, ctx->d_M, ld, ctx->d_info, r, r, n, ctx->d_S, ld, sigma2, Rdiag_dev);
   } else {
     ovb_launch(ctx, k_ekf_gemm, dim3(g0), dim3(256), (size_t)(0), 0, P, ld, H, ldHm, nullptr, 0, ctx->d_info, N, r, n, ctx->d_M, ld, 0.0, nullptr);
     ovb_launch(ctx, k_ekf_gemm, dim3(g1), dim3(256), (size_t)(0), 1, P, ld, H, ldHm, ctx->d_M, ld, ctx->d_info, r, r, n, ctx->d_S, ld, sigma2, Rdiag_dev);
+  }
+  launches += 2;
+  const size_t smd = sizeof(double) * ((size_t)64 * (r | 1) + r);
+  if (fused) {
+    launch_chol_gain(ctx, ctx->d_S, r, z ? z : ctx->d_w, z ? ldz : 1, ctx->d_M, ld, N, ctx->d_w);
+    ovb_launch(ctx, k_ekf_downdate1, dim3(g2), dim3(256), smd, P, ld, (const double *)ctx->d_M, ld, N, r, ctx->d_w, ctx->d_dx, ctx->d_info);
+    return launches + 2;
   }
   size_t chol_bytes = sizeof(double) * (size_t)(r + 1) * (size_t)(r | 1);
   int use_smem = chol_bytes <= 200 * 1024;
@@ -406,17 +438,18 @@
   double *Lpk = nullptr;
   const bool dmma_chol = ctx->ekf_chol_dmma && launch_chol_ekf_dmma(ctx, ctx->d_S, ld, r, ctx->d_w, ctx->d_w, invdiag, &Lpk);
   const bool wide = !dmma_chol && ctx->ekf_chol_dmma && r < ld && launch_chol_solve_wide(ctx, ctx->d_S, ld, r, ctx->d_w, invdiag, ctx->d_M, ld, N, gate_only);
+  launches += 1;
   if (wide) {
     if (gate_only)
-      return;
+      return launches;
     dim3 g2w((N + EK_T - 1) / EK_T, (N + EK_T - 1) / EK_T);
     ovb_launch(ctx, k_ekf_downdate, dim3(g2w), dim3(256), (size_t)(0), P, ld, (const double *)ctx->d_M, ld, N, r, ctx->d_w, ctx->d_dx, ctx->d_info);
-    return;
+    return launches + 2;
   }
   if (!dmma_chol)
     ovb_launch(ctx, k_ekf_chol, dim3(1), dim3(EKC_THREADS), (size_t)(use_smem ? chol_bytes : 0), ctx->d_S, ld, r, ctx->d_w, ctx->d_w, invdiag, ctx->d_info, use_smem);
   if (gate_only)
-    return;
+    return launches;
   const double *Yd = ctx->d_Y;
   if (dmma_chol && Lpk != nullptr && launch_trsm_rows(ctx, ctx->d_M, ld, N, r, Lpk)) {
     Yd = ctx->d_M;
@@ -427,13 +460,12 @@
     ovb_launch(ctx, k_ekf_trsm, dim3((N + TR_ROWS - 1) / TR_ROWS), dim3(32 * TR_ROWS), (size_t)(L_in_smem ? trsm_full : trsm_small), ctx->d_M, ld, ctx->d_S, ld, invdiag, N,
                r, ctx->d_Y, ld, L_in_smem, ctx->d_info);
   }
-  dim3 g2((N + EK_T - 1) / EK_T, (N + EK_T - 1) / EK_T);
   if (one_shot) {
-    const size_t smd = sizeof(double) * ((size_t)64 * (r | 1) + r);
     ovb_launch(ctx, k_ekf_downdate1, dim3(g2), dim3(256), smd, P, ld, Yd, ld, N, r, ctx->d_w, ctx->d_dx, ctx->d_info);
   } else {
     ovb_launch(ctx, k_ekf_downdate, dim3(g2), dim3(256), (size_t)(0), P, ld, Yd, ld, N, r, ctx->d_w, ctx->d_dx, ctx->d_info);
   }
+  return launches + 2;
 }
 
 
diff --git a/open_vins_b200/csrc/ovb_api.cu b/open_vins_b200/csrc/ovb_api.cu
--- a/open_vins_b200/csrc/ovb_api.cu
+++ b/open_vins_b200/csrc/ovb_api.cu
@@ -99,6 +99,8 @@
     ctx->feat_classes = e3 ? atoi(e3) : 1;
     const char *e4 = getenv("OVB_EKF_CHOL_DMMA");
     ctx->ekf_chol_dmma = e4 ? atoi(e4) : 1;
+    const char *e6 = getenv("OVB_EKF_FUSED");
+    ctx->ekf_fused = e6 ? atoi(e6) : 1;
     const char *e5 = getenv("OVB_GRAM_CLUSTER");
     ctx->gram_cluster = e5 ? atoi(e5) : 0;
   }
@@ -1015,12 +1017,6 @@
   return OVB_OK;
 }
 
-__global__ void k_take_z(const double *R, int ldR, int rows, int col, double *w) {
-  OVB_PDL_ENTER();
-  int i = blockIdx.x * blockDim.x + threadIdx.x;
-  if (i < rows)
-    w[i] = R[(size_t)i * ldR + col];
-}
 __global__ void k_fill_zero_dx(double *dx, int N) {
   int i = blockIdx.x * blockDim.x + threadIdx.x;
   if (i < N)
@@ -1136,9 +1132,7 @@
   if (ev)
     cudaEventRecord(ev[4], ctx->stream);
   if (r > 0) {
-    ovb_launch(ctx, k_take_z, dim3((r + 127) / 128), dim3(128), (size_t)(0), Rfinal, ldR, r, n_all, ctx->d_w);
-    launch_ekf_update(ctx, Rfinal, ldR, r, n_all, false, slam ? 1.0 : ctx->h_opts->sigma_pix_sq, nullptr);
-    ctx->n_launch += 7;
+    ctx->n_launch += launch_ekf_update(ctx, Rfinal, ldR, r, n_all, false, slam ? 1.0 : ctx->h_opts->sigma_pix_sq, nullptr, Rfinal + n_all, ldR);
   } else {
     k_fill_zero_dx<<<(N + 127) / 128, 128, 0, ctx->stream>>>(ctx->d_dx, N);
     ctx->n_launch += 1;
@@ -1164,10 +1158,10 @@
     const int r = compress_system(ctx, ctx->h_opts->o.compress, ctx->d_Hs + (size_t)G.row0 * ldH, G.rows, n, ldH, ctx->d_R, ldH);
     ovb_launch(ctx, k_group_take_z, dim3((n + 127) / 128), dim3(128), (size_t)0, (const double *)ctx->d_R, ldH, r, n,
                (const int *)ctx->d_grp[g].col_state, (const double *)acc, ctx->d_w, ctx->d_info);
-    launch_ekf_update(ctx, ctx->d_R, ldH, r, n, false, 1.0, nullptr);
+    ctx->n_launch += launch_ekf_update(ctx, ctx->d_R, ldH, r, n, false, 1.0, nullptr);
     ovb_launch(ctx, k_group_accumulate, dim3((N + 255) / 256), dim3(256), (size_t)0, (const double *)ctx->d_dx, acc, N,
                (const DevUpdateInfo *)ctx->d_info, flags);
-    ctx->n_launch += 8;
+    ctx->n_launch += 2;
     r_total += r;
   }
   if (r_total > 0) {
@@ -1583,9 +1577,7 @@
     compress_system(ctx, ctx->h_opts->o.compress, stacked_dev, n_blocks * n_all, n_all, ld, ctx->d_R, ld);
     Rfinal = ctx->d_R;
   }
-  ovb_launch(ctx, k_take_z, dim3((n_all + 127) / 128), dim3(128), (size_t)(0), Rfinal, ld, n_all, n_all, ctx->d_w);
-  launch_ekf_update(ctx, Rfinal, ld, n_all, n_all, false, ctx->h_opts->sigma_pix_sq, nullptr);
-  ctx->n_launch += 7;
+  ctx->n_launch += launch_ekf_update(ctx, Rfinal, ld, n_all, n_all, false, ctx->h_opts->sigma_pix_sq, nullptr, Rfinal + n_all, ld);
   cudaEventRecord(ctx->ev[5], ctx->stream);
   OVB_CUDA_CHECK(ctx, cudaGetLastError());
   OVB_CUDA_CHECK(ctx, cudaMemcpyAsync(ctx->h_feat, ctx->d_feat, sizeof(DevFeat) * (size_t)F, cudaMemcpyDeviceToHost, ctx->stream));
@@ -1786,8 +1778,7 @@
     rr = compress_system(ctx, OVB_COMPRESS_CHOLQR2, ctx->d_Hs, r, n, ld, ctx->d_R, ld);
     Hdev = ctx->d_R;
   }
-  ovb_launch(ctx, k_take_z, dim3((rr + 127) / 128), dim3(128), (size_t)(0), Hdev, ld, rr, n, ctx->d_w);
-  launch_ekf_update(ctx, Hdev, ld, rr, n, false, s2, nullptr);
+  launch_ekf_update(ctx, Hdev, ld, rr, n, false, s2, nullptr, Hdev + n, ld);
   OVB_CUDA_CHECK(ctx, cudaGetLastError());
   OVB_CUDA_CHECK(ctx, cudaMemcpyAsync(ctx->h_info, ctx->d_info, sizeof(DevUpdateInfo), cudaMemcpyDeviceToHost, ctx->stream));
   OVB_CUDA_CHECK(ctx, cudaMemcpyAsync(ctx->h_dx, ctx->d_dx, sizeof(double) * (size_t)N, cudaMemcpyDeviceToHost, ctx->stream));
@@ -1907,10 +1898,10 @@
       Hdev = ctx->d_R;
       rr = n;
     }
-    ovb_launch(ctx, k_take_z, dim3((rr + 127) / 128), dim3(128), (size_t)(0), Hdev, ld, rr, n, ctx->d_w);
     std::vector<double> zh((size_t)rr), wh((size_t)rr);
-    OVB_CUDA_CHECK(ctx, cudaMemcpyAsync(zh.data(), ctx->d_w, sizeof(double) * (size_t)rr, cudaMemcpyDeviceToHost, ctx->stream));
-    launch_ekf_update(ctx, Hdev, ld, rr, n, true, sigma2, nullptr);
+    OVB_CUDA_CHECK(ctx, cudaMemcpy2DAsync(zh.data(), sizeof(double), Hdev + n, sizeof(double) * (size_t)ld, sizeof(double), (size_t)rr, cudaMemcpyDeviceToHost,
+                                          ctx->stream));
+    launch_ekf_update(ctx, Hdev, ld, rr, n, true, sigma2, nullptr, Hdev + n, ld);
     OVB_CUDA_CHECK(ctx, cudaGetLastError());
     OVB_CUDA_CHECK(ctx, cudaMemcpyAsync(wh.data(), ctx->d_w, sizeof(double) * (size_t)rr, cudaMemcpyDeviceToHost, ctx->stream));
     OVB_CUDA_CHECK(ctx, cudaMemcpyAsync(ctx->h_info, ctx->d_info, sizeof(DevUpdateInfo), cudaMemcpyDeviceToHost, ctx->stream));
@@ -1956,8 +1947,7 @@
   for (int i = 0; i < N + k; i++)
     dx[i] = 0.0;
   if (rup > 0) {
-    ovb_launch(ctx, k_take_z, dim3((rr + 127) / 128), dim3(128), (size_t)(0), Hdev, ld, rr, n, ctx->d_w);
-    launch_ekf_update(ctx, Hdev, ld, rr, n, false, sigma2, nullptr);
+    launch_ekf_update(ctx, Hdev, ld, rr, n, false, sigma2, nullptr, Hdev + n, ld);
     OVB_CUDA_CHECK(ctx, cudaGetLastError());
     OVB_CUDA_CHECK(ctx, cudaMemcpyAsync(ctx->h_info, ctx->d_info, sizeof(DevUpdateInfo), cudaMemcpyDeviceToHost, ctx->stream));
     OVB_CUDA_CHECK(ctx, cudaMemcpyAsync(ctx->h_dx, ctx->d_dx, sizeof(double) * (size_t)(N + k), cudaMemcpyDeviceToHost, ctx->stream));
diff --git a/open_vins_b200/csrc/ovb_internal.cuh b/open_vins_b200/csrc/ovb_internal.cuh
--- a/open_vins_b200/csrc/ovb_internal.cuh
+++ b/open_vins_b200/csrc/ovb_internal.cuh
@@ -149,6 +149,8 @@
   int tsqr_cluster;
   int gram_cluster;
   int ekf_chol_dmma;
+  int ekf_fused;
+  int gain_cluster_ok[8];
   mutable float stage_ms[6];
   mutable int stage_pending;
   double host_us[4];
@@ -191,11 +193,13 @@
 int launch_compress_gram(ovb_ctx *ctx, const double *A, int m, int n, int ldA, double *Rout, int ldR);
 int launch_compress_cholqr2(ovb_ctx *ctx, double *A, int m, int n, int ldA, double *Rout, int ldR);
 bool launch_chol_ekf_dmma(ovb_ctx *ctx, double *S, int ldS, int r, const double *res, double *w, double *invdiag, double **Lpk_out);
+bool chol_gain_fits(ovb_ctx *ctx, int r, int N, int ldM);
+void launch_chol_gain(ovb_ctx *ctx, const double *Spk, int r, const double *z, int ldz, double *M, int ldM, int N, double *w);
 bool launch_trsm_rows(ovb_ctx *ctx, double *A, int ldA, int m, int nt, const double *Lpk);
 bool launch_chol_solve_wide(ovb_ctx *ctx, double *S, int ldS, int r, double *w, double *invdiag, double *M, int ldM, int N, bool gate_only);
 void launch_reorder_R(ovb_ctx *ctx, const double *Rin, int n_all, int ldRin, double *Rout, int ldRout);
-void launch_ekf_update(ovb_ctx *ctx, const double *H, int ldHm, int r_max, int n_max, bool sizes_from_info, double sigma2,
-                       const double *Rdiag_dev);
+int launch_ekf_update(ovb_ctx *ctx, const double *H, int ldHm, int r, int n, bool gate_only, double sigma2, const double *Rdiag_dev,
+                      const double *z = nullptr, int ldz = 1);
 bool launch_cov_init_augment(ovb_ctx *ctx, int k, int n, const double *Hx_dev, const double *Hinv_dev, double sigma2);
 void launch_cov_clone(ovb_ctx *ctx, int old_off, int size, const double *dnc_dt_dev, int dt_off);
 void launch_cov_marginalize(ovb_ctx *ctx, int off, int size);
```

After: 2373 (median of 6 runs). 1.03x the previous value.
